# ShahzaibAhmad05/NextSearch-api

Hardware: AMD Instinct MI355X
Metric: queries/sec at k=10 over 1M-doc index; achieved HBM GB/s vs peak (higher is better)
Workload: dtype f32

## Files before the change

### include/nextsearch_hip.h

```cpp
#ifndef NEXTSEARCH_HIP_H
#define NEXTSEARCH_HIP_H

#include <stdint.h>

#ifdef __cplusplus
extern "C" {
#endif

#define NS_OK            0
#define NS_E_INVAL      -1
#define NS_E_NODEVICE   -2
#define NS_E_HIP        -3
#define NS_E_NOMEM      -4
#define NS_E_STATE      -5

#define NS_MAX_K        100u

#define NS_FLAG_OR      0u
#define NS_FLAG_AND     1u
#define NS_INFO_IMPACTS 0x100u
#define NS_INFO_PACKED  0x200u
#define NS_INFO_SHARED  0x800u
#define NS_INFO_PRUNED  0x400u

typedef struct ns_ctx   ns_ctx;
typedef struct ns_seg   ns_seg;
typedef struct ns_batch ns_batch;

typedef struct ns_term_ref {
    uint32_t seg_id;
    uint32_t count;
    uint64_t byte_off;
    float    idf;
    float    qweight;
} ns_term_ref;

typedef struct ns_query_desc {
    uint32_t term_begin;
    uint32_t term_count;
} ns_query_desc;

typedef struct ns_hit {
    float    score;
    uint32_t seg_id;
    uint32_t doc_id;
} ns_hit;

typedef struct ns_batch_info {
    uint64_t postings;
    uint64_t algo_bytes;
    uint32_t n_queries;
    uint32_t n_items;
    uint32_t n_term_refs;
    uint32_t tile_docs;
    uint32_t k;
    uint32_t flags;
    float    last_score_kernel_ms;
    float    last_total_ms;
    uint32_t timed_runs;
    uint32_t shared_lists;
    double   sum_score_kernel_ms;
    double   sum_total_ms;
    uint64_t shared_postings;
} ns_batch_info;

int  ns_ctx_create(int device, ns_ctx** out);
void ns_ctx_destroy(ns_ctx* ctx);
int  ns_ctx_set_stream(ns_ctx* ctx, void* hip_stream);
const char* ns_last_error(ns_ctx* ctx);
const char* ns_device_name(ns_ctx* ctx);

int ns_segment_upload(ns_ctx* ctx, uint32_t seg_id, uint32_t n_docs, float avgdl,
                      const uint32_t* doc_len, const void* postings, uint64_t nbytes, ns_seg** out);
int ns_segment_release(ns_ctx* ctx, ns_seg* seg);
int ns_segment_upload_begin(ns_ctx* ctx, uint32_t seg_id, uint32_t n_docs, float avgdl, const uint32_t* doc_len,
                            uint64_t total_nbytes, ns_seg** out);
int ns_segment_upload_append(ns_ctx* ctx, ns_seg* seg, const void* bytes, uint64_t nbytes);
int ns_segment_upload_end(ns_ctx* ctx, ns_seg* seg);

int ns_segment_build_impacts(ns_ctx* ctx, ns_seg* seg, const uint64_t* byte_off, const uint32_t* counts,
                             const float* idfs, uint32_t n_lists);
int ns_ctx_set_overlap(ns_ctx* ctx, int on);
int ns_ctx_set_host_threads(ns_ctx* ctx, uint32_t n);
int ns_segment_build_packed(ns_ctx* ctx, ns_seg* seg);
int ns_ctx_use_packed(ns_ctx* ctx, int mode);
int ns_ctx_use_impacts(ns_ctx* ctx, int on);
int ns_segment_build_skips(ns_ctx* ctx, ns_seg* seg, const uint64_t* byte_off, const uint32_t* counts, uint32_t n_lists);
int ns_segment_filter(ns_ctx* ctx, ns_seg* src, uint32_t new_seg_id, const uint32_t* keep_bits, const uint64_t* byte_off,
                      const uint32_t* counts, uint32_t n_lists, uint64_t* new_byte_off_out, uint32_t* new_counts_out,
                      void* postings_out, uint64_t* kept_postings_out, float* device_ms_out, ns_seg** out);
int ns_ctx_use_skips(ns_ctx* ctx, int on);
int ns_segment_build_blockmax(ns_ctx* ctx, ns_seg* seg, const uint64_t* byte_off, const uint32_t* counts,
                              const float* idfs, uint32_t n_lists);
int ns_ctx_use_pruning(ns_ctx* ctx, int on);
int ns_ctx_use_merge(ns_ctx* ctx, int on);
int ns_ctx_share_scores(ns_ctx* ctx, int mode);

int ns_search_batch(ns_ctx* ctx, const ns_query_desc* queries, const ns_term_ref* terms,
                    uint32_t n_queries, uint32_t k, ns_hit* hits_out, uint32_t* nhits_out,
                    uint64_t* found_out, uint32_t flags);

int  ns_batch_prepare(ns_ctx* ctx, const ns_query_desc* queries, const ns_term_ref* terms,
                      uint32_t n_queries, uint32_t k, uint32_t flags, ns_batch** out);
int  ns_batch_bind_outputs(ns_batch* b, void* d_hits, void* d_nhits, void* d_found);
#define NS_RUN_TIMED 1
#define NS_RUN_FETCH 2
int  ns_batch_run(ns_batch* b, int run_flags);
void* ns_batch_stream(ns_batch* b);
int  ns_batch_gap_ms(ns_batch* prev, ns_batch* next, float* ms);
int  ns_batch_sync(ns_batch* b);
int  ns_batch_fetch(ns_batch* b, ns_hit* hits_out, uint32_t* nhits_out, uint64_t* found_out);
int  ns_batch_get_info(ns_batch* b, ns_batch_info* info);
void ns_batch_destroy(ns_batch* b);

typedef struct ns_sem ns_sem;
int ns_sem_upload(ns_ctx* ctx, const float* vecs, uint32_t n_rows, uint32_t dim, ns_sem** out);
int ns_sem_release(ns_ctx* ctx, ns_sem* sem);
int ns_sem_topk(ns_ctx* ctx, ns_sem* sem, const float* qvecs, uint32_t n_q, uint32_t topk, float min_sim,
                const uint32_t* ban_off, const uint32_t* ban_rows, uint32_t* rows_out, float* sims_out,
                uint32_t* counts_out, float* device_ms_out);

typedef struct ns_ac ns_ac;
int ns_ac_upload(ns_ctx* ctx, const uint8_t* pool, const uint64_t* offsets, const uint32_t* scores, uint32_t n_terms, ns_ac** out);
int ns_ac_suggest(ns_ctx* ctx, ns_ac* ac, const uint8_t* prefix_bytes, const uint32_t* prefix_offsets, uint32_t n_q, uint32_t L,
                  uint32_t* idx_out, uint32_t* count_out, float* device_ms_out);
int ns_ac_release(ns_ctx* ctx, ns_ac* ac);

#define NS_FUZZY_MAX_LEN   64u
#define NS_FUZZY_MAX_EDITS 2u
int ns_ac_build_fuzzy(ns_ctx* ctx, ns_ac* ac, float* device_ms_out);
int ns_ac_fuzzy(ns_ctx* ctx, ns_ac* ac, const uint8_t* term_bytes, const uint32_t* term_offsets, uint32_t n_q,
                const uint8_t* max_edits, uint32_t prefix_len, uint32_t L, uint32_t* idx_out, uint8_t* dist_out,
                uint32_t* count_out, float* device_ms_out);

int ns_ac_fuzzy_prefix(ns_ctx* ctx, ns_ac* ac, const uint8_t* prefix_bytes, const uint32_t* prefix_offsets, uint32_t n_q,
                       const uint8_t* max_edits, uint32_t prefix_len, uint32_t L, uint32_t* idx_out, uint8_t* dist_out,
                       uint32_t* count_out, float* device_ms_out);

int ns_merge_rank_rows(ns_ctx* ctx, const void* d_hits, const void* d_nhits, const void* d_found, uint32_t n_ranks,
                       uint32_t n_queries, uint32_t k, const uint32_t* d_seg_map, uint32_t seg_map_stride,
                       void* d_out_hits, void* d_out_nhits, void* d_out_found);

int ns_invert_forward(ns_ctx* ctx, const uint32_t* doc_term_counts, uint32_t n_docs, const uint32_t* pairs,
                      uint64_t n_pairs, uint32_t n_terms, uint32_t* df_out, void* postings_out, uint64_t* kept_out,
                      float* device_ms_out);
int ns_segment_upload_inverted(ns_ctx* ctx, ns_seg* seg, const uint32_t* doc_term_counts, const uint32_t* pairs,
                               uint64_t n_pairs, uint32_t n_terms, uint32_t* df_out, void* postings_out,
                               uint64_t* kept_out, float* device_ms_out);

#define NS_E_ARG NS_E_INVAL
typedef struct ns_forward ns_forward;
typedef struct ns_forward_info {
    uint32_t struct_size;
    uint32_t kept_docs;
    uint32_t n_terms;
    uint32_t n_docs;
    uint64_t n_pairs;
    uint64_t term_bytes;
    uint64_t n_tokens;
    uint64_t kept_tokens;
    uint64_t device_bytes;
    float    device_ms;
    uint32_t pad;
} ns_forward_info;
int ns_forward_build(ns_ctx* ctx, const uint8_t* text, uint64_t text_bytes, const uint64_t* offsets, uint32_t n_docs,
                     ns_forward** out);
int ns_forward_get_info(const ns_forward* fwd, ns_forward_info* info);
int ns_forward_fetch(ns_forward* fwd, uint32_t* kept_docs_out, uint32_t* doc_len_out, uint32_t* counts_out,
                     uint32_t* pairs_out, uint8_t* term_bytes_out, uint64_t* term_offsets_out);
void ns_forward_destroy(ns_forward* fwd);

typedef struct ns_forward_src {
    uint32_t n_docs;  const uint32_t* doc_len;  const uint32_t* counts;
    uint64_t n_pairs; const uint32_t* pairs;
    uint32_t n_terms; const uint8_t* term_bytes; const uint64_t* term_offsets;
} ns_forward_src;
int ns_forward_merge(ns_ctx* ctx, const ns_forward_src* src, uint32_t n_src, ns_forward** out);
int ns_forward_invert(ns_forward* fwd, uint32_t* df_out, void* postings_out, uint64_t* kept_out, float* device_ms_out);
uint32_t ns_compact_doc_cut(void);
// ... 47 lines not shown
```

### nextsearch-api_amd/csrc/ns_api.hip

```cpp
#include <hip/hip_runtime.h>

#include <algorithm>
#include <cmath>
#include <cstdarg>
#include <cstdio>
#include <cstdlib>
#include <cstring>
#include <string>
#include <vector>

#include "../../include/nextsearch_hip.h"
#include "ns_internal.h"
#include "ns_plan.hpp"
#include "ns_kernels.hip"
#include "ns_wave_kernel.hip"
#include "ns_driver_kernel.hip"
#include "ns_prune_kernel.hip"
#include "ns_merge_kernel.hip"
#include "ns_tile_kernel.hip"
#include "ns_invert.hip"
#include "ns_ingest.hip"
#include "ns_compact.hip"
#include "ns_delete.hip"
#include "ns_filter.hip"
#include "ns_facet.hip"
#include "ns_similar.hip"
#include "ns_sorted.hip"
#include "ns_boolean.hip"
#include "ns_sem.hip"
#include "ns_suggest.hip"
#include "ns_fuzzy.hip"

using namespace ns;

static_assert(sizeof(ns_hit) == sizeof(Hit), "ns_hit layout");


struct ns_seg {
    ns_ctx* ctx = nullptr;
    uint32_t id = 0;
    uint32_t n_docs = 0;
    uint64_t n_postings = 0;
    uint2* d_postings = nullptr;
    float* d_norm = nullptr;
    float* d_pnorm = nullptr;
    bool norm_safe = false;
    float avgdl = 0.0f;
    bool pending = false;
    uint64_t filled = 0;
    uint32_t* d_len = nullptr;
    void* pin[2] = {nullptr, nullptr};
    hipEvent_t ev[2] = {nullptr, nullptr};
    int stage_k = 0;
    uint32_t* d_packed = nullptr;
    uint2* d_pk_hdr = nullptr;
    float* d_pk_scores = nullptr;
    uint16_t* d_nidx = nullptr;
    float* d_ntab = nullptr;
    uint32_t n_norms = 0;
    uint2* d_impacts = nullptr;
    uint32_t* d_skips = nullptr;
    std::vector<uint32_t*> skip_retired;
    uint64_t skip_cap = 0, skip_used = 0;
    uint32_t skip_entries() const { return (n_docs + kSkipDocs - 1) / kSkipDocs + 2; }
    float* d_blockmax = nullptr;
    std::vector<float*> bmx_retired;
    uint64_t bmx_cap = 0, bmx_used = 0;
    SegLists lists;
};

struct ns_ctx {
    struct Block { void* p; size_t n; };
    std::vector<Block> pool;
    size_t pool_bytes = 0;
    int device = 0;
    hipStream_t own_stream = nullptr;
    hipStream_t stream = nullptr;
    hipStream_t alt_stream = nullptr;
    hipStream_t pull_stream = nullptr;
    bool overlap = false, flip = false;
    std::string err;
    std::string devname;
    std::vector<ns_seg*> segs;
    std::vector<ns_seg*> pending_uploads;
    void* h_up = nullptr;
    size_t h_up_cap = 0;
    hipEvent_t up_done = nullptr;
    bool up_busy = false;
    void* h_down = nullptr;
    size_t h_down_cap = 0;
    struct ns_batch* down_owner = nullptr;
    struct DownSlot { void* p = nullptr; size_t cap = 0; bool busy = false; };
    std::vector<DownSlot> down_slots;
    PlanSettings cfg;
    ShareRegistry share;
    BatchPlan plan;
    std::vector<ns_ac*> acs;
    std::vector<ns_forward*> fwds;
    bool cp_inplace = true;
    std::vector<ns_docterms*> dts;
};

static thread_local std::string g_create_err;
static void ac_free_fwd(ns_ac* ac);
static void forward_orphan_fwd(ns_forward* f);
static void docterms_orphan_fwd(ns_docterms* h);
static void seg_free_device_fwd(ns_seg* s);
static void seg_free_staging_fwd(ns_seg* s);

static int fail(ns_ctx* ctx, int code, const char* fmt, ...) {
    va_list ap;
    va_start(ap, fmt);
    (ctx ? ctx->err : g_create_err) = vformat(fmt, ap);
    va_end(ap);
    return code;
}

#define HIPCHK(ctx, call)                                                                         \
    do {                                                                                          \
        hipError_t e_ = (call);                                                                   \
        if (e_ != hipSuccess)                                                                     \
            return fail((ctx), NS_E_HIP, "%s failed: %s (%s:%d)", #call, hipGetErrorString(e_), __FILE__, __LINE__); \
    } while (0)

template <int CB, int TMAX, bool IMP, int PK>
static void launch_uscore(bool and_mode, uint32_t n_items, hipStream_t st, const DevWItem* items, const DevTerm* terms,
                          const DevSeg* segs, Hit* hits, uint32_t* nhits, uint64_t* found, uint32_t K) {
    dim3 grid((n_items + kUscoreWavesPerBlock - 1) / kUscoreWavesPerBlock), block(64 * kUscoreWavesPerBlock);
    if (and_mode)
        hipLaunchKernelGGL((k_uscore<512, 192, true, CB, TMAX, IMP, PK>), grid, block, 0, st, items, n_items, terms, segs, hits, nhits, found, K);
    else
        hipLaunchKernelGGL((k_uscore<512, 192, false, CB, TMAX, IMP, PK>), grid, block, 0, st, items, n_items, terms, segs, hits, nhits, found, K);
}
template <int CB, int TMAX>
static void launch_uscore(bool and_mode, bool imp, int pk, uint32_t n_items, hipStream_t st, const DevWItem* items,
                          const DevTerm* terms, const DevSeg* segs, Hit* hits, uint32_t* nhits, uint64_t* found, uint32_t K) {
    if (imp && pk) launch_uscore<CB, TMAX, true, 1>(and_mode, n_items, st, items, terms, segs, hits, nhits, found, K);
    else if (imp) launch_uscore<CB, TMAX, true, 0>(and_mode, n_items, st, items, terms, segs, hits, nhits, found, K);
    else if (pk == 2) launch_uscore<CB, TMAX, false, 2>(and_mode, n_items, st, items, terms, segs, hits, nhits, found, K);
    else if (pk == 1) launch_uscore<CB, TMAX, false, 1>(and_mode, n_items, st, items, terms, segs, hits, nhits, found, K);
    else launch_uscore<CB, TMAX, false, 0>(and_mode, n_items, st, items, terms, segs, hits, nhits, found, K);
}

template <int HK, int FB>
static void launch_dscore(bool and_mode, uint32_t n_items, hipStream_t st, const DevWItem* items, const DevTerm* terms,
                          const DevSeg* segs, Hit* hits, uint32_t* nhits, uint64_t* found, uint32_t K) {
    dim3 grid((n_items + 3) / 4), block(256);
    if (and_mode)
        hipLaunchKernelGGL((k_dscore<HK, FB, true>), grid, block, 0, st, items, n_items, terms, segs, hits, nhits, found, K);
    else
        hipLaunchKernelGGL((k_dscore<HK, FB, false>), grid, block, 0, st, items, n_items, terms, segs, hits, nhits, found, K);
}

template <int TD>
static void launch_tscore(bool and_mode, uint32_t n_items, hipStream_t st, const DevWItem* items, const DevTerm* terms,
                          const DevSeg* segs, Hit* hits, uint32_t* nhits, uint64_t* found, uint32_t K) {
    dim3 grid((n_items + 3) / 4), block(256);
    if (and_mode)
        hipLaunchKernelGGL((k_tscore<TD, true>), grid, block, 0, st, items, n_items, terms, segs, hits, nhits, found, K);
    else
        hipLaunchKernelGGL((k_tscore<TD, false>), grid, block, 0, st, items, n_items, terms, segs, hits, nhits, found, K);
}

template <int NT, int SPT, int U>
static void launch_score(bool and_mode, uint32_t n_items, hipStream_t st, const DevItem* items, const DevTerm* terms,
                         const DevSeg* segs, const uint32_t* bounds, Hit* hits, uint32_t* nhits, uint64_t* found,
                         uint32_t K) {
    if (and_mode)
        hipLaunchKernelGGL((k_score<NT, SPT, U, true>), dim3(n_items), dim3(NT), 0, st, items, terms, segs, bounds, hits, nhits, found, K);
    else
        hipLaunchKernelGGL((k_score<NT, SPT, U, false>), dim3(n_items), dim3(NT), 0, st, items, terms, segs, bounds, hits, nhits, found, K);
}

extern "C" int ns_ctx_create(int device, ns_ctx** out) {
    if (!out) return fail(nullptr, NS_E_INVAL, "ns_ctx_create: out is NULL");
    *out = nullptr;
    int ndev = 0;
    hipError_t e = hipGetDeviceCount(&ndev);
    if (e != hipSuccess || ndev <= 0)
        return fail(nullptr, NS_E_NODEVICE, "no HIP device available (%s); this library has no CPU fallback",
                    e == hipSuccess ? "device count 0" : hipGetErrorString(e));
    if (device < 0 || device >= ndev) return fail(nullptr, NS_E_INVAL, "device %d out of range [0,%d)", device, ndev);
    e = hipSetDevice(device);
    if (e != hipSuccess) return fail(nullptr, NS_E_NODEVICE, "hipSetDevice(%d): %s", device, hipGetErrorString(e));
    hipDeviceProp_t prop;
    e = hipGetDeviceProperties(&prop, device);
    if (e != hipSuccess) return fail(nullptr, NS_E_NODEVICE, "hipGetDeviceProperties: %s", hipGetErrorString(e));
    ns_ctx* ctx = new ns_ctx();
    ctx->device = device;
    ctx->devname = std::string(prop.gcnArchName) + " " + prop.name;
    ctx->cfg.n_cus = prop.multiProcessorCount;
    e = hipStreamCreateWithFlags(&ctx->own_stream, hipStreamNonBlocking);
    if (e != hipSuccess) {
        int rc = fail(nullptr, NS_E_HIP, "hipStreamCreate: %s", hipGetErrorString(e));
        delete ctx;
        return rc;
    }
    ctx->stream = ctx->own_stream;
    if (const char* om = std::getenv("NS_ORDER_MODE")) ctx->cfg.order_mode = std::atoi(om);
    if (const char* kp = std::getenv("NS_KEY_PCT")) {
        unsigned a = 100, b = 100, c = 100, d = 100;
        if (std::sscanf(kp, "%u,%u,%u,%u", &a, &b, &c, &d) >= 1) { ctx->cfg.key_pct[0] = a; ctx->cfg.key_pct[1] = b; ctx->cfg.key_pct[2] = c; ctx->cfg.key_pct[3] = d; }
    }
    if (const char* td = std::getenv("NS_TILE_DENS64")) ctx->cfg.tile_dens64 = (uint32_t)std::max(1, std::atoi(td));
    if (const char* um = std::getenv("NS_MERGE")) ctx->cfg.use_merge = std::atoi(um) != 0;
    if (const char* mr = std::getenv("NS_MERGE_RATIO")) ctx->cfg.merge_ratio = (uint32_t)std::max(1, std::atoi(mr));
    if (const char* sm = std::getenv("NS_SHARE")) ctx->cfg.share_mode = std::max(0, std::min(2, std::atoi(sm)));
    if (const char* sr = std::getenv("NS_SHARE_RATIO")) ctx->cfg.share_ratio = (uint32_t)std::max(1, std::atoi(sr));
    if (const char* sp = std::getenv("NS_SHARE_MIN")) ctx->cfg.share_min_postings = (uint64_t)std::max(0ll, std::atoll(sp));
    if (const char* oc = std::getenv("NS_ORDER_COARSE")) { ctx->cfg.order_coarse = std::max(0, std::min(11, std::atoi(oc))); ctx->cfg.order_coarse_forced = true; }
    if (hipStreamCreateWithFlags(&ctx->alt_stream, hipStreamNonBlocking) != hipSuccess) { ctx->alt_stream = nullptr; (void)hipGetLastError(); }
    {
        int lo_pri = 0, hi_pri = 0;
        (void)hipDeviceGetStreamPriorityRange(&lo_pri, &hi_pri);
        if (hipStreamCreateWithPriority(&ctx->pull_stream, hipStreamNonBlocking, hi_pri) != hipSuccess) { ctx->pull_stream = nullptr; (void)hipGetLastError(); }
    }
    *out = ctx;
    return NS_OK;
}

extern "C" void ns_ctx_destroy(ns_ctx* ctx) {
    if (!ctx) return;
    (void)hipSetDevice(ctx->device);
    (void)hipStreamSynchronize(ctx->stream);
    if (ctx->alt_stream) (void)hipStreamSynchronize(ctx->alt_stream);
    if (ctx->pull_stream) (void)hipStreamSynchronize(ctx->pull_stream);
    for (ns_seg* s : ctx->segs) {
        if (!s) continue;
        seg_free_device_fwd(s);
        delete s;
    }
    for (ns_seg* s : ctx->pending_uploads) {
        seg_free_staging_fwd(s);
        seg_free_device_fwd(s);
        delete s;
    }
    for (ns_ac* ac : ctx->acs) ac_free_fwd(ac);
    for (ns_forward* f : ctx->fwds) forward_orphan_fwd(f);
    for (ns_docterms* h : ctx->dts) docterms_orphan_fwd(h);
    for (auto& blk : ctx->pool) (void)hipFree(blk.p);
    if (ctx->h_up) (void)hipHostFree(ctx->h_up);
    if (ctx->h_down) (void)hipHostFree(ctx->h_down);
    for (auto& ds : ctx->down_slots) if (ds.p) (void)hipHostFree(ds.p);
    if (ctx->up_done) (void)hipEventDestroy(ctx->up_done);
    if (ctx->own_stream) (void)hipStreamDestroy(ctx->own_stream);
    if (ctx->alt_stream) (void)hipStreamDestroy(ctx->alt_stream);
    if (ctx->pull_stream) (void)hipStreamDestroy(ctx->pull_stream);
    delete ctx;
}

extern "C" int ns_ctx_set_stream(ns_ctx* ctx, void* hip_stream) {
    if (!ctx) return fail(nullptr, NS_E_INVAL, "ns_ctx_set_stream: ctx is NULL");
    ctx->stream = hip_stream ? (hipStream_t)hip_stream : ctx->own_stream;
    return NS_OK;
}

extern "C" const char* ns_last_error(ns_ctx* ctx) { return ctx ? ctx->err.c_str() : g_create_err.c_str(); }
extern "C" const char* ns_device_name(ns_ctx* ctx) { return ctx ? ctx->devname.c_str() : ""; }

extern "C" int ns_set_tuning(ns_ctx* ctx, uint32_t variant, uint32_t min_items, uint32_t split_postings) {
    if (!ctx) return fail(nullptr, NS_E_INVAL, "ns_set_tuning: ctx is NULL");
    if (variant >= kNumVariants || kVariants[variant].nt == 0) return fail(ctx, NS_E_INVAL, "unknown kernel variant %u", variant);
#ifndef NS_VARIANTS
    if (variant != 0) return fail(ctx, NS_E_INVAL, "kernel variant %u exists only in the variants build (make -C nextsearch-api_amd variants)", variant);
#endif
    ctx->cfg.variant = variant;
    ctx->cfg.min_items = min_items;
    ctx->cfg.split_postings = split_postings;
    return NS_OK;
}

static constexpr size_t kPadPostings = 256;
static constexpr size_t kStageChunk = 32u << 20;

static void seg_free_staging(ns_seg* s) {
    for (int i = 0; i < 2; i++) {
        if (s->pin[i]) (void)hipHostFree(s->pin[i]);
        if (s->ev[i]) (void)hipEventDestroy(s->ev[i]);
        s->pin[i] = nullptr; s->ev[i] = nullptr;
    }
    if (s->d_len) (void)hipFree(s->d_len);
    s->d_len = nullptr;
}
static void seg_free_device(ns_seg* s);
static void seg_free_device_fwd(ns_seg* s) { seg_free_device(s); }
static void seg_free_staging_fwd(ns_seg* s) { seg_free_staging(s); }
static void seg_free_device(ns_seg* s) {
    (void)hipFree(s->d_postings);
    (void)hipFree(s->d_norm);
    (void)hipFree(s->d_pnorm);
    (void)hipFree(s->d_impacts);
    (void)hipFree(s->d_packed);
    (void)hipFree(s->d_pk_hdr);
    (void)hipFree(s->d_pk_scores);
    (void)hipFree(s->d_nidx);
    (void)hipFree(s->d_ntab);
    (void)hipFree(s->d_skips);
    for (uint32_t* p : s->skip_retired) (void)hipFree(p);
    s->skip_retired.clear();
    (void)hipFree(s->d_blockmax);
    for (float* p : s->bmx_retired) (void)hipFree(p);
    s->bmx_retired.clear();
    s->d_blockmax = nullptr; s->bmx_cap = s->bmx_used = 0; s->lists.bmx.clear();
    s->d_skips = nullptr; s->skip_cap = s->skip_used = 0; s->lists.skip.clear();
    s->d_postings = nullptr; s->d_norm = nullptr; s->d_pnorm = nullptr; s->d_impacts = nullptr; s->d_packed = nullptr;
    s->d_pk_hdr = nullptr; s->d_pk_scores = nullptr; s->d_nidx = nullptr; s->d_ntab = nullptr;
}
static hipError_t seg_stage(ns_ctx* ctx, ns_seg* s, void* dst, const void* src, size_t n) {
    size_t off = 0;
    while (off < n) {
        const size_t c = std::min(kStageChunk, n - off);
        const int k = s->stage_k;
        hipError_t r = hipEventSynchronize(s->ev[k]);
        if (r != hipSuccess) return r;
        std::memcpy(s->pin[k], (const char*)src + off, c);
        r = hipMemcpyAsync((char*)dst + off, s->pin[k], c, hipMemcpyHostToDevice, ctx->stream);
        if (r != hipSuccess) return r;
        r = hipEventRecord(s->ev[k], ctx->stream);
        if (r != hipSuccess) return r;
        off += c;
        s->stage_k ^= 1;
    }
    return hipSuccess;
}

extern "C" int ns_segment_upload_begin(ns_ctx* ctx, uint32_t seg_id, uint32_t n_docs, float avgdl, const uint32_t* doc_len,
                                       uint64_t nbytes, ns_seg** out) {
    if (!ctx) return fail(nullptr, NS_E_INVAL, "ns_segment_upload: ctx is NULL");
    if (!out) return fail(ctx, NS_E_INVAL, "ns_segment_upload_begin: out is NULL");
    *out = nullptr;
// ... 203 lines not shown
    if (int rc = check_lists(ctx, seg, byte_off, counts, n_lists)) return rc;
    struct L { uint32_t first, count; float idf; };
    std::vector<L> lists;
    lists.reserve(n_lists);
    for (uint32_t i = 0; i < n_lists; i++)
        if (counts[i]) lists.push_back({(uint32_t)(byte_off[i] / 8), counts[i], idfs[i]});
    std::sort(lists.begin(), lists.end(), [](const L& a, const L& b) { return a.first < b.first; });
    for (size_t i = 1; i < lists.size(); i++)
        if (lists[i - 1].first + (uint64_t)lists[i - 1].count > lists[i].first) return fail(ctx, NS_E_INVAL, "lists overlap at posting %u", lists[i].first);
    if (lists.empty()) return NS_OK;
    hipError_t e = hipSuccess;
    if (!seg->d_impacts) {
        e = hipMalloc((void**)&seg->d_impacts, (seg->n_postings + kPadPostings) * 8);
        if (e != hipSuccess) { seg->d_impacts = nullptr; return fail(ctx, NS_E_NOMEM, "hipMalloc impact stream (%llu B): %s", (unsigned long long)(seg->n_postings * 8), hipGetErrorString(e)); }
        e = hipMemsetAsync(seg->d_impacts, 0xFF, (seg->n_postings + kPadPostings) * 8, ctx->stream);
    }
    const size_t n = lists.size();
    std::vector<uint32_t> h_starts(n), h_counts(n);
    std::vector<float> h_idfs(n);
    for (size_t i = 0; i < n; i++) { h_starts[i] = lists[i].first; h_counts[i] = lists[i].count; h_idfs[i] = lists[i].idf; }
    uint32_t* d_tmp = nullptr;
    if (e == hipSuccess) e = hipMalloc((void**)&d_tmp, n * 12);
    if (e == hipSuccess) e = hipMemcpyAsync(d_tmp, h_starts.data(), n * 4, hipMemcpyHostToDevice, ctx->stream);
    if (e == hipSuccess) e = hipMemcpyAsync(d_tmp + n, h_counts.data(), n * 4, hipMemcpyHostToDevice, ctx->stream);
    if (e == hipSuccess) e = hipMemcpyAsync(d_tmp + 2 * n, h_idfs.data(), n * 4, hipMemcpyHostToDevice, ctx->stream);
    if (e == hipSuccess) {
        const uint32_t blocks = (uint32_t)std::min<uint64_t>((seg->n_postings + 255) / 256, 1u << 16);
        hipLaunchKernelGGL(k_build_impacts, dim3(blocks), dim3(256), 0, ctx->stream, seg->d_postings, seg->d_pnorm, seg->d_impacts,
                           d_tmp, d_tmp + n, (const float*)(d_tmp + 2 * n), (uint32_t)n, seg->n_postings);
        e = hipGetLastError();
    }
    if (e == hipSuccess) e = hipStreamSynchronize(ctx->stream);
    (void)hipFree(d_tmp);
    if (e == hipSuccess) e = seg_fill_pk_scores(ctx, seg);
    if (e != hipSuccess) return fail(ctx, NS_E_HIP, "ns_segment_build_impacts: %s", hipGetErrorString(e));
    for (const auto& l : lists) {
        uint32_t ib; std::memcpy(&ib, &l.idf, 4);
        seg->lists.imp.put(l.first, {l.count, ib});
    }
    return NS_OK;
}

__global__ void __launch_bounds__(256) k_share_scores(const DevShare* __restrict__ sh, uint32_t n_lists, const DevSeg* __restrict__ segs) {
    const uint32_t total = sh[n_lists].before;
    const uint32_t base = blockIdx.x * 1024u;
    if (base >= total) return;
    const uint32_t last = min(base + 1023u, total - 1u);
    __shared__ uint32_t s_lo, s_hi;
    if (threadIdx.x < 2) {
        const uint32_t want = threadIdx.x == 0 ? base : last;
        uint32_t lo = 0, hi = n_lists;
        while (hi - lo > 1) {
            const uint32_t mid = lo + ((hi - lo) >> 1);
            if (sh[mid].before <= want) lo = mid; else hi = mid;
        }
        if (threadIdx.x == 0) s_lo = lo; else s_hi = lo;
    }
    __syncthreads();
    const uint32_t l0 = s_lo, l1 = s_hi;
#pragma unroll
    for (int j = 0; j < 4; j++) {
        const uint32_t p = base + (uint32_t)j * 256u + threadIdx.x;
        if (p > last) continue;
        uint32_t lo = l0, hi = l1 + 1u;
        while (hi - lo > 1) {
            const uint32_t mid = lo + ((hi - lo) >> 1);
            if (sh[mid].before <= p) lo = mid; else hi = mid;
        }
        const DevShare L = sh[lo];
        const DevSeg& sg = segs[L.seg];
        const uint64_t at = (uint64_t)L.first + (p - L.before);
        const uint2 pv = sg.postings[at];
        const float tf = (float)pv.y;
        const float den = tf + sg.pnorm[at];
        const float num = L.idf * (tf * (1.2f + 1.0f));
        const_cast<uint2*>(sg.impacts)[at] = make_uint2(pv.x, __float_as_uint(num / den));
    }
}

extern "C" int ns_ctx_share_scores(ns_ctx* ctx, int mode) {
    if (!ctx) return fail(nullptr, NS_E_INVAL, "ns_ctx_share_scores: ctx is NULL");
    if (mode < 0 || mode > 2) return fail(ctx, NS_E_INVAL, "ns_ctx_share_scores: mode %d outside [0, 2]", mode);
    ctx->cfg.share_mode = mode;
    return NS_OK;
}

extern "C" int ns_segment_build_packed(ns_ctx* ctx, ns_seg* seg) {
    if (!ctx || !seg) return fail(ctx, NS_E_INVAL, "ns_segment_build_packed: null argument");
    if (seg->pending || seg->id >= ctx->segs.size() || ctx->segs[seg->id] != seg) return fail(ctx, NS_E_INVAL, "segment does not belong to this ctx");
    if (seg->d_packed || !seg->n_postings) return NS_OK;
    if (!seg->d_nidx) return fail(ctx, NS_E_INVAL, "ns_segment_build_packed: segment %u has more than 65536 distinct document lengths; its norms do not fit a 16-bit index", seg->id);
    HIPCHK(ctx, hipSetDevice(ctx->device));
    const uint64_t n_blocks = (seg->n_postings + kPkBlock - 1) / kPkBlock;
    hipError_t e = hipMalloc((void**)&seg->d_packed, (n_blocks + 2) * kPkStrideDwords * 4);
    if (e == hipSuccess) e = hipMalloc((void**)&seg->d_pk_hdr, (n_blocks + 2) * sizeof(uint2));
    if (e == hipSuccess) e = hipMemsetAsync(seg->d_packed + n_blocks * kPkStrideDwords, 0, 2 * kPkStrideDwords * 4, ctx->stream);
    if (e == hipSuccess) e = hipMemsetAsync(seg->d_pk_hdr + n_blocks, 0, 2 * sizeof(uint2), ctx->stream);
    if (e == hipSuccess) {
        hipLaunchKernelGGL(k_pack, dim3((uint32_t)n_blocks), dim3(64), 0, ctx->stream, seg->d_postings, seg->d_nidx, seg->d_packed, seg->d_pk_hdr,
                           seg->n_postings, seg->n_docs, (uint32_t)n_blocks);
        e = hipGetLastError();
    }
    if (e == hipSuccess) e = hipStreamSynchronize(ctx->stream);
    if (e == hipSuccess) e = seg_fill_pk_scores(ctx, seg);
    if (e != hipSuccess) {
        (void)hipFree(seg->d_packed); (void)hipFree(seg->d_pk_hdr);
        seg->d_packed = nullptr; seg->d_pk_hdr = nullptr;
        return fail(ctx, e == hipErrorOutOfMemory ? NS_E_NOMEM : NS_E_HIP, "ns_segment_build_packed: %s", hipGetErrorString(e));
    }
    return NS_OK;
}

__global__ void __launch_bounds__(256) k_skip_fill(uint32_t* __restrict__ sk, const uint32_t* __restrict__ starts, const uint32_t* __restrict__ counts,
                                                   uint32_t per_list) {
    const uint32_t l = blockIdx.y;
    const uint32_t endp = starts[l] + counts[l];
    for (uint32_t i = blockIdx.x * 256 + threadIdx.x; i < per_list; i += gridDim.x * 256) sk[(uint64_t)l * per_list + i] = endp;
}
__global__ void __launch_bounds__(256) k_skip_build(const uint2* __restrict__ postings, uint32_t* __restrict__ sk, const uint32_t* __restrict__ starts,
                                                    const uint32_t* __restrict__ counts, uint32_t per_list) {
    const uint32_t l = blockIdx.y;
    const uint32_t first = starts[l], n = counts[l];
    uint32_t* row = sk + (uint64_t)l * per_list;
    const uint32_t cells = per_list - 2;
    for (uint32_t i = blockIdx.x * 256 + threadIdx.x; i < n; i += gridDim.x * 256) {
        const uint32_t d = postings[first + i].x / kSkipDocs;
        uint32_t c0 = 0;
        if (i) {
            const uint32_t dp = postings[first + i - 1].x / kSkipDocs;
            c0 = dp + 1;
        }
        for (uint32_t c = c0; c <= d && c <= cells; c++) row[c] = first + i;
    }
}
__global__ void __launch_bounds__(256) k_skip_check(const uint2* __restrict__ postings, const uint32_t* __restrict__ sk, const uint32_t* __restrict__ starts,
                                                    const uint32_t* __restrict__ counts, uint32_t per_list, uint32_t* __restrict__ bad) {
    const uint32_t l = blockIdx.y;
    const uint32_t first = starts[l], endp = first + counts[l];
    const uint32_t* row = sk + (uint64_t)l * per_list;
    bool b = false;
    for (uint32_t i = blockIdx.x * 256 + threadIdx.x; i + 1 < per_list; i += gridDim.x * 256) {
        const uint32_t a = row[i], z = row[i + 1];
        if (a > z || a < first || z > endp) b = true;
        if (i == 0 && a != first) b = true;
        if (i + 2 == per_list && (z != endp || a != endp)) b = true;
        if (i + 2 < per_list && a < z) {
            if (postings[a].x / kSkipDocs != i || postings[z - 1].x / kSkipDocs != i) b = true;
        }
    }
    if (b) bad[l] = 1u;
}

extern "C" int ns_segment_build_skips(ns_ctx* ctx, ns_seg* seg, const uint64_t* byte_off, const uint32_t* counts, uint32_t n_lists) {
    if (!ctx || !seg) return fail(ctx, NS_E_INVAL, "ns_segment_build_skips: null argument");
    if (seg->pending || seg->id >= ctx->segs.size() || ctx->segs[seg->id] != seg) return fail(ctx, NS_E_INVAL, "segment does not belong to this ctx");
    if (n_lists && (!byte_off || !counts)) return fail(ctx, NS_E_INVAL, "null list arrays");
    if (!n_lists || !seg->n_postings || !seg->n_docs) return NS_OK;
    HIPCHK(ctx, hipSetDevice(ctx->device));
    if (int rc = check_lists(ctx, seg, byte_off, counts, n_lists)) return rc;
    struct L { uint32_t first, count; };
    std::vector<L> lists;
    lists.reserve(n_lists);
    for (uint32_t i = 0; i < n_lists; i++)
        if (counts[i] && !seg->lists.skip_of((uint32_t)(byte_off[i] / 8), counts[i])) lists.push_back({(uint32_t)(byte_off[i] / 8), counts[i]});
    std::sort(lists.begin(), lists.end(), [](const L& a, const L& b) { return a.first < b.first || (a.first == b.first && a.count < b.count); });
    lists.erase(std::unique(lists.begin(), lists.end(), [](const L& a, const L& b) { return a.first == b.first; }), lists.end());
// ... 96 lines not shown
    if (e == hipSuccess) e = hipMemcpyAsync(d_tmp, h.data(), n * 16, hipMemcpyHostToDevice, ctx->stream);
    if (e == hipSuccess) {
        for (size_t l0 = 0; l0 < n; l0 += 32768) {
            const uint32_t ny = (uint32_t)std::min<size_t>(32768, n - l0);
            hipLaunchKernelGGL(k_blockmax, dim3(std::min<uint32_t>(std::max<uint32_t>(bmax_blocks, 1u), 256u), ny), dim3(64), 0, ctx->stream,
                               seg->d_postings, seg->d_pnorm, seg->d_blockmax, d_tmp + l0, d_tmp + n + l0, (const float*)(d_tmp + 2 * n + l0), d_tmp + 3 * n + l0);
        }
        e = hipGetLastError();
    }
    if (e == hipSuccess) e = hipStreamSynchronize(ctx->stream);
    (void)hipFree(d_tmp);
    if (e != hipSuccess) return fail(ctx, NS_E_HIP, "ns_segment_build_blockmax: %s", hipGetErrorString(e));
    seg->bmx_used = need;
    for (const auto& l : lists) {
        uint32_t ib; std::memcpy(&ib, &l.idf, 4);
        seg->lists.bmx.put(l.first, {l.count, ib, l.entry});
    }
    return NS_OK;
}

extern "C" int ns_ctx_use_merge(ns_ctx* ctx, int on) {
    if (!ctx) return NS_E_INVAL;
    ctx->cfg.use_merge = on != 0;
    return NS_OK;
}

extern "C" int ns_ctx_use_pruning(ns_ctx* ctx, int on) {
    if (!ctx) return NS_E_INVAL;
    ctx->cfg.use_pruning = on != 0;
    return NS_OK;
}

extern "C" int ns_ctx_use_skips(ns_ctx* ctx, int on) {
    if (!ctx) return NS_E_INVAL;
    ctx->cfg.use_skips = on != 0;
    return NS_OK;
}

extern "C" int ns_ctx_use_packed(ns_ctx* ctx, int on) {
    if (!ctx) return NS_E_INVAL;
    if (on < 0 || on > 2) return fail(ctx, NS_E_INVAL, "ns_ctx_use_packed: mode %d (0, 1 or 2)", on);
    ctx->cfg.use_packed = on;
    return NS_OK;
}

extern "C" int ns_ctx_set_overlap(ns_ctx* ctx, int on) {
    if (!ctx) return NS_E_INVAL;
    if (on && !ctx->alt_stream) return fail(ctx, NS_E_HIP, "ns_ctx_set_overlap: the second stream could not be created");
    ctx->overlap = on != 0;
    return NS_OK;
}

extern "C" int ns_ctx_set_host_threads(ns_ctx* ctx, uint32_t n) {
    if (!ctx) return NS_E_INVAL;
    if (n > 64) return fail(ctx, NS_E_INVAL, "ns_ctx_set_host_threads: %u threads (at most 64)", n);
    ctx->cfg.prep_threads = n;
    return NS_OK;
}

extern "C" int ns_ctx_use_impacts(ns_ctx* ctx, int on) {
    if (!ctx) return NS_E_INVAL;
    ctx->cfg.use_impacts = on != 0;
    return NS_OK;
}

struct ns_batch {
    ns_ctx* ctx = nullptr;
    uint32_t Q = 0, K = 0, flags = 0;
    uint32_t variant = 0, tile_docs = 0, hb = 0;
    uint32_t n_items = 0;
    uint32_t n_witems = 0;
    uint32_t n_class[3] = {0, 0, 0};
    uint32_t n_bgroups = 0;
    uint32_t n_terms = 0, n_parts = 0;
    uint64_t postings = 0;
    bool direct = false;
    int pk = 0;
    bool pruned = false;
    bool imp = false;
    bool shared = false;
    uint32_t n_share = 0;
    uint64_t share_postings = 0;
    DevShare* d_share = nullptr;
    DevItem* d_items = nullptr;
    DevWItem* d_witems = nullptr;
    DevTerm* d_terms = nullptr;
    DevGroup* d_groups = nullptr;
    DevQuery* d_queries = nullptr;
    DevSeg* d_segs = nullptr;
    uint32_t* d_bounds = nullptr;
    Hit* d_part_hits = nullptr;
    uint32_t* d_part_nhits = nullptr;
    uint64_t* d_part_found = nullptr;
    uint32_t* d_heads = nullptr;
    Hit* d_hits = nullptr;
    uint32_t* d_nhits = nullptr;
    uint64_t* d_found = nullptr;
    Hit* o_hits = nullptr;
    uint32_t* o_nhits = nullptr;
    uint64_t* o_found = nullptr;
    std::vector<hipEvent_t> ev_pool;
    size_t ev_pending = 0;
    bool ran = false;
    float last_score_ms = -1.0f, last_total_ms = -1.0f;
    double sum_score_ms = 0.0, sum_total_ms = 0.0;
    uint32_t timed_runs = 0;
    uint32_t* d_wide_q = nullptr;
    uint32_t n_wide_q = 0;
    size_t out_span = 0, off_nhits = 0, off_found = 0;
    std::vector<std::pair<void*, size_t>> blocks;
    hipStream_t st = nullptr;
    hipEvent_t done = nullptr;
    bool done_recorded = false;
    bool fetch_enqueued = false;
    int down_slot = -1;
};

static constexpr size_t kPoolMaxBytes = 1ull << 30;
static constexpr size_t kStageMaxBytes = 256ull << 20;
static constexpr size_t kPullUploadBytes = 256 << 10;
static constexpr size_t kHostResultBytes = 64 << 10;

static size_t pool_quantise(size_t n) {
    if (n <= (64u << 10)) return 64u << 10;
    if (n <= (64u << 20)) { size_t q = 64u << 10; while (q < n) q <<= 1; return q; }
    return (n + (16u << 20) - 1) & ~(size_t)((16u << 20) - 1);
}
static hipError_t pool_alloc(ns_ctx* ctx, void** out, size_t n) {
    n = pool_quantise(n);
    size_t best = (size_t)-1;
    for (size_t i = 0; i < ctx->pool.size(); i++)
        if (ctx->pool[i].n >= n && ctx->pool[i].n <= 2 * n + 4096 && (best == (size_t)-1 || ctx->pool[i].n < ctx->pool[best].n)) best = i;
    if (best != (size_t)-1) {
        *out = ctx->pool[best].p;
        ctx->pool_bytes -= ctx->pool[best].n;
        ctx->pool[best] = ctx->pool.back();
        ctx->pool.pop_back();
        return hipSuccess;
    }
    hipError_t e = hipMalloc(out, n);
    if (e == hipErrorOutOfMemory && !ctx->pool.empty()) {
        for (auto& b : ctx->pool) (void)hipFree(b.p);
        ctx->pool.clear(); ctx->pool_bytes = 0;
        e = hipMalloc(out, n);
    }
    return e;
}
static void pool_free(ns_ctx* ctx, void* p, size_t n) {
    if (!p) return;
    n = pool_quantise(n);
    if (ctx->pool_bytes + n > kPoolMaxBytes || ctx->pool.size() >= 64) { (void)hipFree(p); return; }
    ctx->pool.push_back({p, n});
    ctx->pool_bytes += n;
}

__global__ void __launch_bounds__(256) k_pull(uint4* __restrict__ dst, const uint4* __restrict__ src, uint32_t n16) {
    const uint32_t i = blockIdx.x * 256 + threadIdx.x;
    if (i < n16) dst[i] = src[i];
}

extern "C" void ns_batch_destroy(ns_batch* b) {
    if (!b) return;
    (void)hipSetDevice(b->ctx->device);
    if (b->done_recorded) (void)hipEventSynchronize(b->done);
    else (void)hipStreamSynchronize(b->st);
    if (b->ctx->down_owner == b) b->ctx->down_owner = nullptr;
    if (b->down_slot >= 0) b->ctx->down_slots[(size_t)b->down_slot].busy = false;
    if (b->shared && b->ctx->share.live) b->ctx->share.live--;
    for (auto& blk : b->blocks) pool_free(b->ctx, blk.first, blk.second);
    for (auto& e : b->ev_pool) if (e) (void)hipEventDestroy(e);
    if (b->done) (void)hipEventDestroy(b->done);
    delete b;
}

static hipError_t batch_alloc(ns_batch* b, void** dptr, size_t n) {
    hipError_t e = pool_alloc(b->ctx, dptr, n);
    if (e == hipSuccess) b->blocks.push_back({*dptr, n});
    return e;
}
extern "C" int ns_batch_prepare(ns_ctx* ctx, const ns_query_desc* queries, const ns_term_ref* terms, uint32_t n_queries,
                                uint32_t k, uint32_t flags, ns_batch** out) {
    if (!ctx) return fail(nullptr, NS_E_INVAL, "ns_batch_prepare: ctx is NULL");
    if (!out) return fail(ctx, NS_E_INVAL, "ns_batch_prepare: out is NULL");
    *out = nullptr;
    if (k < 1 || k > NS_MAX_K) return fail(ctx, NS_E_INVAL, "k=%u outside [1,%u]", k, NS_MAX_K);
    if (n_queries && !queries) return fail(ctx, NS_E_INVAL, "queries is NULL");
    if (flags & ~NS_FLAG_AND) return fail(ctx, NS_E_INVAL, "unknown flags 0x%x", flags);
    HIPCHK(ctx, hipSetDevice(ctx->device));

    const VariantDesc vd = kVariants[ctx->cfg.variant];
    const uint32_t tile_docs = vd.nt * vd.spt;
    std::vector<SegView> views(ctx->segs.size());
    std::vector<DevSeg> segs(ctx->segs.size());
    for (size_t i = 0; i < ctx->segs.size(); i++) {
        DevSeg d{};
        if (ns_seg* s = ctx->segs[i]) {
            d.postings = s->d_postings;
            d.pnorm = s->d_pnorm;
            d.impacts = s->d_impacts;
            d.packed = s->d_packed;
            d.pk_hdr = s->d_pk_hdr;
            d.ntab = s->d_ntab;
            d.pk_scores = s->d_pk_scores;
            d.skips = s->d_skips;
            d.blockmax = s->d_blockmax;
            d.norm = s->d_norm;
            d.n_postings = s->n_postings;
            d.n_docs = s->n_docs;
            d.n_tiles = (s->n_docs + tile_docs - 1) / tile_docs;
            views[i] = SegView{s->n_docs, d.n_tiles, s->n_postings, s->norm_safe, s->d_packed != nullptr, &s->lists};
        }
        segs[i] = d;
    }

    BatchPlan& P = ctx->plan;
    int rc = P.group(ctx->cfg, views, ctx->share, queries, terms, n_queries, k, flags);
    if (rc != NS_OK) return fail(ctx, rc, "%s", P.err.c_str());
    for (size_t i = 0; P.shared && i < P.share_build.size(); i++) {
        ns_seg* sg = ctx->segs[P.share_build[i].seg];
        if (!sg->d_impacts) {
            const size_t nb = (size_t)(sg->n_postings + kPadPostings) * 8;
            hipError_t ea = hipMalloc((void**)&sg->d_impacts, nb);
            if (ea == hipSuccess) ea = hipMemsetAsync(sg->d_impacts, 0xFF, nb, ctx->stream);
            if (ea == hipSuccess) ea = hipStreamSynchronize(ctx->stream);
            if (ea != hipSuccess) {
                if (sg->d_impacts) (void)hipFree(sg->d_impacts);
                sg->d_impacts = nullptr; (void)hipGetLastError();
                P.shared = false;
            }
        }
        if (P.shared) segs[P.share_build[i].seg].impacts = sg->d_impacts;
    }
    rc = P.cut();
    if (rc != NS_OK) return fail(ctx, rc, "%s", P.err.c_str());

    ns_batch* b = new ns_batch();
    b->ctx = ctx;
    b->st = ctx->stream;
    if (ctx->overlap && ctx->stream == ctx->own_stream && ctx->alt_stream) {
        ctx->flip = !ctx->flip;
        if (ctx->flip) b->st = ctx->alt_stream;
    }
    b->Q = n_queries; b->K = k; b->flags = flags;
    b->variant = ctx->cfg.variant; b->tile_docs = tile_docs; b->hb = vd.hb;
    b->n_items = P.n_items; b->n_witems = P.n_witems;
    b->n_bgroups = P.n_bgroups; b->n_terms = P.n_dterms;
    for (int c = 0; c < 3; c++) b->n_class[c] = P.n_class[c];
    b->n_parts = P.direct ? 0 : P.n_rows;
    b->postings = P.postings_total;
    b->direct = P.direct;
    b->imp = P.all_imp && P.postings_total > 0;
    if (P.shared) {
        b->shared = true;
        b->n_share = (uint32_t)P.share_build.size();
        b->share_postings = P.share_postings;
        ctx->share.live++;
    }
    b->pk = (P.all_pk && P.postings_total > 0) ? ctx->cfg.use_packed : 0;
    b->pruned = P.pruned;
    b->n_wide_q = (uint32_t)P.wide_q.size();

    hipError_t e = hipSuccess;
    auto chk = [&](hipError_t r) { if (e == hipSuccess) e = r; };
    const BatchPlan::Layout& L = P.layout;
    const size_t up_bytes = L.bytes;
    size_t off = up_bytes;
    auto place = [&](size_t bytes) { return place_at(off, bytes); };
    const size_t Qn = std::max<uint32_t>(n_queries, 1), Pn = std::max<uint32_t>(b->n_parts, 1);
    const size_t o_bounds = place(P.bounds_total * 4);
    size_t o_phits = 0, o_pnhits = 0, o_pfound = 0, o_heads = 0;
    if (!P.direct) {
        o_phits = place(Pn * k * sizeof(Hit));
        o_pnhits = place(Pn * 4);
        o_pfound = place(Pn * 8);
        o_heads = place(Pn * 4);
    }
    const size_t o_hits = place(Qn * k * sizeof(Hit));
    const size_t o_nhits = place(Qn * 4);
    const size_t o_found = place(Qn * 8);
    char* base = nullptr;
    chk(batch_alloc(b, (void**)&base, off));
    if (e == hipSuccess) {
        b->d_items = (decltype(b->d_items))(base + L.items);
        b->d_witems = (decltype(b->d_witems))(base + L.witems);
        b->d_terms = (decltype(b->d_terms))(base + L.terms);
        b->d_groups = (decltype(b->d_groups))(base + L.groups);
        b->d_queries = (decltype(b->d_queries))(base + L.queries);
        b->d_segs = (decltype(b->d_segs))(base + L.segs);
        b->d_wide_q = (uint32_t*)(base + L.wideq);
        b->d_share = (DevShare*)(base + L.share);
        b->d_bounds = (uint32_t*)(base + o_bounds);
        if (!P.direct) {
            b->d_part_hits = (Hit*)(base + o_phits);
            b->d_part_nhits = (uint32_t*)(base + o_pnhits);
            b->d_part_found = (uint64_t*)(base + o_pfound);
            b->d_heads = (uint32_t*)(base + o_heads);
        }
        b->d_hits = (Hit*)(base + o_hits);
        b->d_nhits = (uint32_t*)(base + o_nhits);
        b->d_found = (uint64_t*)(base + o_found);
        b->out_span = o_found + Qn * 8 - o_hits;
        b->off_nhits = o_nhits - o_hits;
        b->off_found = o_found - o_hits;
        if (b->out_span <= kHostResultBytes && !ctx->down_owner) {
            if (ctx->h_down_cap < b->out_span) {
                if (ctx->h_down) (void)hipHostFree(ctx->h_down);
                ctx->h_down = nullptr; ctx->h_down_cap = 0;
                if (hipHostMalloc(&ctx->h_down, kHostResultBytes, hipHostMallocDefault) == hipSuccess) ctx->h_down_cap = kHostResultBytes;
                else { ctx->h_down = nullptr; (void)hipGetLastError(); }
            }
            if (ctx->h_down_cap >= b->out_span) {
                ctx->down_owner = b;
                b->d_hits = (Hit*)ctx->h_down;
                b->d_nhits = (uint32_t*)((char*)ctx->h_down + b->off_nhits);
                b->d_found = (uint64_t*)((char*)ctx->h_down + b->off_found);
            }
        }
    }
    if (e == hipSuccess && ctx->up_busy) {
        chk(hipEventSynchronize(ctx->up_done));
        ctx->up_busy = false;
    }
    if (e == hipSuccess && up_bytes <= kStageMaxBytes && ctx->h_up_cap < up_bytes) {
        if (ctx->h_up) (void)hipHostFree(ctx->h_up);
        ctx->h_up = nullptr; ctx->h_up_cap = 0;
        const size_t cap = std::max<size_t>(up_bytes + up_bytes / 2, 1 << 16);
        if (hipHostMalloc(&ctx->h_up, cap, hipHostMallocDefault) == hipSuccess) ctx->h_up_cap = cap;
        else { ctx->h_up = nullptr; (void)hipGetLastError(); }
    }
    if (e == hipSuccess && !ctx->up_done) chk(hipEventCreateWithFlags(&ctx->up_done, hipEventDisableTiming));
    if (e == hipSuccess) {
        const bool staged = ctx->h_up_cap >= up_bytes && ctx->up_done;
        std::vector<char> unstaged;
        if (!staged) unstaged.resize(up_bytes);
        char* hb = staged ? (char*)ctx->h_up : unstaged.data();
        P.write(hb);
        if (!segs.empty()) std::memcpy(hb + L.segs, segs.data(), segs.size() * sizeof(segs[0]));
        if (staged) {
            if (up_bytes > kPullUploadBytes && ctx->pull_stream) {
                hipLaunchKernelGGL(k_pull, dim3((uint32_t)((up_bytes / 16 + 255) / 256)), dim3(256), 0, ctx->pull_stream,
                                   (uint4*)base, (const uint4*)hb, (uint32_t)(up_bytes / 16));
                chk(hipEventRecord(ctx->up_done, ctx->pull_stream));
                chk(hipStreamWaitEvent(b->st, ctx->up_done, 0));
            } else {
                if (up_bytes <= kPullUploadBytes || ctx->overlap)
                    hipLaunchKernelGGL(k_pull, dim3((uint32_t)((up_bytes / 16 + 255) / 256)), dim3(256), 0, b->st,
                                       (uint4*)base, (const uint4*)hb, (uint32_t)(up_bytes / 16));
                else
                    chk(hipMemcpyAsync(base, hb, up_bytes, hipMemcpyHostToDevice, b->st));
                chk(hipEventRecord(ctx->up_done, b->st));
            }
            if (e == hipSuccess) ctx->up_busy = true;
        } else {
            chk(hipMemcpyAsync(base, hb, up_bytes, hipMemcpyHostToDevice, b->st));
            chk(hipStreamSynchronize(b->st));
        }
    }
    if (e != hipSuccess) {
        rc = fail(ctx, e == hipErrorOutOfMemory ? NS_E_NOMEM : NS_E_HIP, "ns_batch_prepare: %s", hipGetErrorString(e));
        ns_batch_destroy(b);
        return rc;
    }
    b->o_hits = b->d_hits; b->o_nhits = b->d_nhits; b->o_found = b->d_found;
    *out = b;
    return NS_OK;
}

extern "C" int ns_batch_bind_outputs(ns_batch* b, void* d_hits, void* d_nhits, void* d_found) {
    if (!b) return NS_E_INVAL;
    b->o_hits = d_hits ? (Hit*)d_hits : b->d_hits;
    b->o_nhits = d_nhits ? (uint32_t*)d_nhits : b->d_nhits;
    b->o_found = d_found ? (uint64_t*)d_found : b->d_found;
    return NS_OK;
}

extern "C" int ns_batch_run(ns_batch* b, int run_flags) {
    if (!b) return NS_E_INVAL;
    ns_ctx* ctx = b->ctx;
    const int timed = run_flags & NS_RUN_TIMED;
    if (run_flags & NS_RUN_FETCH) {
        const bool own_outputs = b->o_hits == b->d_hits && b->o_nhits == b->d_nhits && b->o_found == b->d_found;
        if (!own_outputs) return fail(ctx, NS_E_STATE, "NS_RUN_FETCH: the batch writes into caller-bound device buffers (ns_batch_bind_outputs); there is nothing to fetch");
    }
    b->done_recorded = false;
    HIPCHK(ctx, hipSetDevice(ctx->device));
    hipStream_t st = b->st;
    const bool and_mode = (b->flags & NS_FLAG_AND) != 0;
    hipEvent_t* ev = nullptr;
    if (timed) {
        while (b->ev_pool.size() < b->ev_pending + 4) {
            hipEvent_t e = nullptr;
            HIPCHK(ctx, hipEventCreate(&e));
            b->ev_pool.push_back(e);
        }
        ev = b->ev_pool.data() + b->ev_pending;
        b->ev_pending += 4;
    }
    if (timed) HIPCHK(ctx, hipEventRecord(ev[0], st));
    if (b->n_bgroups)
        hipLaunchKernelGGL(k_bounds, dim3(b->n_bgroups), dim3(128), 0, st, b->d_groups, b->d_terms, b->d_segs, b->d_bounds, b->tile_docs);
    if (timed) HIPCHK(ctx, hipEventRecord(ev[1], st));
    if (b->shared && b->n_share)
        hipLaunchKernelGGL(k_share_scores, dim3((uint32_t)((b->share_postings + 1023) / 1024)), dim3(256), 0, st, b->d_share, b->n_share, b->d_segs);
    Hit* sh = b->direct ? b->o_hits : b->d_part_hits;
    uint32_t* sn = b->direct ? b->o_nhits : b->d_part_nhits;
    uint64_t* sf = b->direct ? b->o_found : b->d_part_found;
    if (b->n_witems && b->variant == 0) {
        const uint32_t n_narrow = b->n_class[0], n_wide = b->n_witems - b->n_class[0];
        const DevWItem* wide = b->d_witems + n_narrow;
        if (b->K <= 32) {
            if (n_narrow) launch_uscore<128, 16>(and_mode, b->imp, b->pk, n_narrow, st, b->d_witems, b->d_terms, b->d_segs, sh, sn, sf, b->K);
            if (n_wide) launch_uscore<128, 64>(and_mode, b->imp, b->pk, n_wide, st, wide, b->d_terms, b->d_segs, sh, sn, sf, b->K);
        } else {
            if (n_narrow) launch_uscore<256, 16>(and_mode, b->imp, b->pk, n_narrow, st, b->d_witems, b->d_terms, b->d_segs, sh, sn, sf, b->K);
            if (n_wide) launch_uscore<256, 64>(and_mode, b->imp, b->pk, n_wide, st, wide, b->d_terms, b->d_segs, sh, sn, sf, b->K);
        }
    }
#ifdef NS_VARIANTS
    else if (b->n_witems) {
        const VariantDesc wv = kVariants[b->variant];
#define NS_D(HH, FF) launch_dscore<HH, FF>(and_mode, b->n_witems, st, b->d_witems, b->d_terms, b->d_segs, sh, sn, sf, b->K)
        if (wv.d == 1) {
            if (wv.hb == 512) launch_tscore<512>(and_mode, b->n_witems, st, b->d_witems, b->d_terms, b->d_segs, sh, sn, sf, b->K);
            else if (wv.hb == 2048) launch_tscore<2048>(and_mode, b->n_witems, st, b->d_witems, b->d_terms, b->d_segs, sh, sn, sf, b->K);
            else launch_tscore<1024>(and_mode, b->n_witems, st, b->d_witems, b->d_terms, b->d_segs, sh, sn, sf, b->K);
        } else if (wv.d == 0) {
            switch (b->variant) {
                case 13: NS_D(256, 64); break;
                case 14: NS_D(1024, 256); break;
                case 15: NS_D(512, 64); break;
                case 16: NS_D(512, 256); break;
                case 17: NS_D(1024, 128); break;
                default: NS_D(512, 128); break;
            }
        }
#undef NS_D
    }
#endif
    if (b->n_items) {
#ifdef NS_VARIANTS
        const VariantDesc vd = kVariants[b->variant];
        if (vd.nt == 1024) launch_score<1024, 12, 4>(and_mode, b->n_items, st, b->d_items, b->d_terms, b->d_segs, b->d_bounds, sh, sn, sf, b->K);
        else if (vd.nt == 256) launch_score<256, 16, 4>(and_mode, b->n_items, st, b->d_items, b->d_terms, b->d_segs, b->d_bounds, sh, sn, sf, b->K);
        else if (vd.spt == 16) launch_score<512, 16, 8>(and_mode, b->n_items, st, b->d_items, b->d_terms, b->d_segs, b->d_bounds, sh, sn, sf, b->K);
        else
#endif
        launch_score<512, 12, 4>(and_mode, b->n_items, st, b->d_items, b->d_terms, b->d_segs, b->d_bounds, sh, sn, sf, b->K);
    }
    if (timed) HIPCHK(ctx, hipEventRecord(ev[2], st));
    if (!b->direct && b->Q > b->n_wide_q)
        hipLaunchKernelGGL(k_merge, dim3((b->Q + 3) / 4), dim3(256), 0, st, b->d_queries, b->Q, b->d_part_hits, b->d_part_nhits,
                           b->d_part_found, b->o_hits, b->o_nhits, b->o_found, b->K, b->d_heads);
    if (!b->direct && b->n_wide_q)
        hipLaunchKernelGGL(k_merge_wide, dim3(b->n_wide_q), dim3(256), 0, st, b->d_queries, b->d_wide_q, b->d_part_hits, b->d_part_nhits,
                           b->d_part_found, b->o_hits, b->o_nhits, b->o_found, b->K, b->d_heads);
    if (timed) HIPCHK(ctx, hipEventRecord(ev[3], st));
    HIPCHK(ctx, hipGetLastError());
    b->ran = true;
    if (run_flags & NS_RUN_FETCH) {
        if (b->Q && ctx->down_owner != b) {
            if (b->down_slot < 0) {
                int slot = -1;
                for (size_t i = 0; i < ctx->down_slots.size(); i++)
                    if (!ctx->down_slots[i].busy && ctx->down_slots[i].cap >= b->out_span) { slot = (int)i; break; }
                if (slot < 0) {
                    for (size_t i = 0; i < ctx->down_slots.size() && slot < 0; i++)
                        if (!ctx->down_slots[i].busy) {
                            if (ctx->down_slots[i].p) (void)hipHostFree(ctx->down_slots[i].p);
                            ctx->down_slots[i] = ns_ctx::DownSlot{};
                            slot = (int)i;
                        }
                    if (slot < 0) {
                        if (ctx->down_slots.size() >= 8) return fail(ctx, NS_E_STATE, "NS_RUN_FETCH: more than 8 batches between run and fetch");
                        ctx->down_slots.emplace_back();
                        slot = (int)ctx->down_slots.size() - 1;
                    }
                    const size_t cap = std::max<size_t>(b->out_span + b->out_span / 4, 1 << 16);
                    if (hipHostMalloc(&ctx->down_slots[(size_t)slot].p, cap, hipHostMallocDefault) != hipSuccess) {
                        ctx->down_slots[(size_t)slot].p = nullptr;
                        (void)hipGetLastError();
                        return fail(ctx, NS_E_NOMEM, "NS_RUN_FETCH: pinned result buffer of %zu bytes", cap);
                    }
                    ctx->down_slots[(size_t)slot].cap = cap;
                }
                ctx->down_slots[(size_t)slot].busy = true;
                b->down_slot = slot;
            }
            HIPCHK(ctx, hipMemcpyAsync(ctx->down_slots[(size_t)b->down_slot].p, b->d_hits, b->out_span, hipMemcpyDeviceToHost, st));
        }
    }
    if (!b->done) HIPCHK(ctx, hipEventCreateWithFlags(&b->done, hipEventDisableTiming));
    HIPCHK(ctx, hipEventRecord(b->done, st));
    b->done_recorded = true;
    b->fetch_enqueued = (run_flags & NS_RUN_FETCH) != 0;
    return NS_OK;
}

extern "C" void* ns_batch_stream(ns_batch* b) { return b ? (void*)b->st : nullptr; }

extern "C" int ns_batch_gap_ms(ns_batch* prev, ns_batch* next, float* ms) {
    if (!prev || !next || !ms) return NS_E_INVAL;
    if (prev->ev_pool.size() < 4 || next->ev_pool.size() < 4) return fail(next->ctx, NS_E_STATE, "ns_batch_gap_ms: both batches need a timed run");
    const hipError_t e = hipEventElapsedTime(ms, prev->ev_pool[3], next->ev_pool[0]);
    if (e == hipErrorNotReady) { (void)hipGetLastError(); return NS_E_STATE; }
    if (e != hipSuccess) return fail(next->ctx, NS_E_HIP, "ns_batch_gap_ms: %s", hipGetErrorString(e));
    return NS_OK;
}


static int batch_collect_timings(ns_batch* b) {
    ns_ctx* ctx = b->ctx;
    for (size_t i = 0; i + 4 <= b->ev_pending; i += 4) {
        HIPCHK(ctx, hipEventElapsedTime(&b->last_score_ms, b->ev_pool[i + 1], b->ev_pool[i + 2]));
        HIPCHK(ctx, hipEventElapsedTime(&b->last_total_ms, b->ev_pool[i], b->ev_pool[i + 3]));
        b->sum_score_ms += b->last_score_ms;
        b->sum_total_ms += b->last_total_ms;
        b->timed_runs++;
    }
    b->ev_pending = 0;
    return NS_OK;
}

extern "C" int ns_batch_sync(ns_batch* b) {
    if (!b) return NS_E_INVAL;
    ns_ctx* ctx = b->ctx;
    HIPCHK(ctx, hipSetDevice(ctx->device));
    HIPCHK(ctx, hipStreamSynchronize(b->st));
    return batch_collect_timings(b);
}

extern "C" int ns_batch_fetch(ns_batch* b, ns_hit* hits_out, uint32_t* nhits_out, uint64_t* found_out) {
    if (!b) return NS_E_INVAL;
    ns_ctx* ctx = b->ctx;
    if (!b->ran) return fail(ctx, NS_E_STATE, "ns_batch_fetch before ns_batch_run");
    HIPCHK(ctx, hipSetDevice(ctx->device));
    hipStream_t st = b->st;
    const bool own_outputs = b->o_hits == b->d_hits && b->o_nhits == b->d_nhits && b->o_found == b->d_found;
    if (b->fetch_enqueued && b->done_recorded && own_outputs) {
        HIPCHK(ctx, hipEventSynchronize(b->done));
        int rc = batch_collect_timings(b);
        if (rc != NS_OK) return rc;
        if (b->Q) {
            const char* h = (ctx->down_owner == b) ? (const char*)ctx->h_down : (const char*)ctx->down_slots[(size_t)b->down_slot].p;
            if (hits_out) std::memcpy(hits_out, h, (size_t)b->Q * b->K * sizeof(Hit));
            if (nhits_out) std::memcpy(nhits_out, h + b->off_nhits, (size_t)b->Q * 4);
            if (found_out) std::memcpy(found_out, h + b->off_found, (size_t)b->Q * 8);
        }
        if (b->down_slot >= 0) { ctx->down_slots[(size_t)b->down_slot].busy = false; b->down_slot = -1; }
        b->fetch_enqueued = false;
        return NS_OK;
    }
    if (b->Q && own_outputs && ctx->down_owner == b) {
        int rc = ns_batch_sync(b);
        if (rc != NS_OK) return rc;
        const char* h = (const char*)ctx->h_down;
        if (hits_out) std::memcpy(hits_out, h, (size_t)b->Q * b->K * sizeof(Hit));
        if (nhits_out) std::memcpy(nhits_out, h + b->off_nhits, (size_t)b->Q * 4);
        if (found_out) std::memcpy(found_out, h + b->off_found, (size_t)b->Q * 8);
        return NS_OK;
    }
    if (b->Q && own_outputs && !ctx->down_owner && b->out_span <= kStageMaxBytes) {
        if (ctx->h_down_cap < b->out_span) {
            if (ctx->h_down) (void)hipHostFree(ctx->h_down);
            ctx->h_down = nullptr; ctx->h_down_cap = 0;
            const size_t cap = std::max<size_t>(b->out_span + b->out_span / 2, 1 << 16);
            if (hipHostMalloc(&ctx->h_down, cap, hipHostMallocDefault) == hipSuccess) ctx->h_down_cap = cap;
            else { ctx->h_down = nullptr; (void)hipGetLastError(); }
        }
        if (ctx->h_down_cap >= b->out_span) {
            HIPCHK(ctx, hipMemcpyAsync(ctx->h_down, b->d_hits, b->out_span, hipMemcpyDeviceToHost, st));
            int rc = ns_batch_sync(b);
            if (rc != NS_OK) return rc;
            const char* h = (const char*)ctx->h_down;
            if (hits_out) std::memcpy(hits_out, h, (size_t)b->Q * b->K * sizeof(Hit));
            if (nhits_out) std::memcpy(nhits_out, h + b->off_nhits, (size_t)b->Q * 4);
            if (found_out) std::memcpy(found_out, h + b->off_found, (size_t)b->Q * 8);
            return NS_OK;
        }
    }
    if (b->Q) {
        if (hits_out) HIPCHK(ctx, hipMemcpyAsync(hits_out, b->o_hits, (size_t)b->Q * b->K * sizeof(Hit), hipMemcpyDeviceToHost, st));
        if (nhits_out) HIPCHK(ctx, hipMemcpyAsync(nhits_out, b->o_nhits, (size_t)b->Q * 4, hipMemcpyDeviceToHost, st));
        if (found_out) HIPCHK(ctx, hipMemcpyAsync(found_out, b->o_found, (size_t)b->Q * 8, hipMemcpyDeviceToHost, st));
    }
    return ns_batch_sync(b);
}

extern "C" int ns_batch_get_info(ns_batch* b, ns_batch_info* info) {
    if (!b || !info) return NS_E_INVAL;
    info->postings = b->postings;
    info->algo_bytes = b->postings * 8;
    info->n_queries = b->Q;
    info->n_items = b->n_items + b->n_witems;
    info->n_term_refs = b->n_terms;
    info->tile_docs = b->tile_docs;
    info->k = b->K;
    info->flags = b->flags | (b->imp ? NS_INFO_IMPACTS : 0u) | (b->pk ? NS_INFO_PACKED : 0u) | (b->pruned ? NS_INFO_PRUNED : 0u) |
                  (b->shared ? NS_INFO_SHARED : 0u);
    info->shared_lists = b->n_share;
    info->shared_postings = b->share_postings;
    info->last_score_kernel_ms = b->last_score_ms;
    info->last_total_ms = b->last_total_ms;
    info->timed_runs = b->timed_runs;
    info->sum_score_kernel_ms = b->sum_score_ms;
    info->sum_total_ms = b->sum_total_ms;
    return NS_OK;
}

extern "C" int ns_search_batch(ns_ctx* ctx, const ns_query_desc* queries, const ns_term_ref* terms, uint32_t n_queries,
                               uint32_t k, ns_hit* hits_out, uint32_t* nhits_out, uint64_t* found_out, uint32_t flags) {
    ns_batch* b = nullptr;
    int rc = ns_batch_prepare(ctx, queries, terms, n_queries, k, flags, &b);
    if (rc != NS_OK) return rc;
    rc = ns_batch_run(b, 0);
    if (rc == NS_OK) rc = ns_batch_fetch(b, hits_out, nhits_out, found_out);
    ns_batch_destroy(b);
    return rc;
}


static int invert_run(ns_ctx* ctx, const uint32_t* doc_term_counts, uint32_t n_docs, const uint32_t* pairs,
                      uint64_t n_pairs, uint32_t n_terms, uint32_t* df_out, void* postings_out, uint64_t* kept_out,
                      float* device_ms_out, ns_seg* adopt, const uint2* dev_pairs = nullptr) {
    if (!ctx) return fail(nullptr, NS_E_INVAL, "ns_invert_forward: ctx is NULL");
    if ((n_docs && !doc_term_counts) || (n_pairs && !pairs && !dev_pairs) || (n_terms && !df_out) || !kept_out) return fail(ctx, NS_E_INVAL, "ns_invert_forward: null argument");
    if (n_pairs >= (1ull << 32) - kIvTile) return fail(ctx, NS_E_INVAL, "ns_invert_forward: %llu pairs; this build indexes pairs with 32 bits (split the segment)", (unsigned long long)n_pairs);
    if (n_terms == 0xFFFFFFFFu) return fail(ctx, NS_E_INVAL, "ns_invert_forward: n_terms too large");
    *kept_out = 0;
    if (device_ms_out) *device_ms_out = 0.0f;
    std::vector<uint64_t> prefix((size_t)n_docs + 1, 0);
    for (uint32_t d = 0; d < n_docs; d++) prefix[d + 1] = prefix[d] + doc_term_counts[d];
    if (prefix[n_docs] != n_pairs) return fail(ctx, NS_E_INVAL, "ns_invert_forward: the per-document counts sum to %llu, not to n_pairs = %llu", (unsigned long long)prefix[n_docs], (unsigned long long)n_pairs);
    if (n_terms) std::memset(df_out, 0, (size_t)n_terms * 4);
    if (!n_pairs) return NS_OK;
    if (!postings_out && !adopt) return fail(ctx, NS_E_INVAL, "ns_invert_forward: postings_out is NULL");
    HIPCHK(ctx, hipSetDevice(ctx->device));
    hipStream_t st = ctx->stream;
    const uint32_t n = (uint32_t)n_pairs;
    const uint32_t n_tiles = (n + kIvTile - 1) / kIvTile;
    int bits = 1;
    while (bits < 32 && n_terms > 1 && ((n_terms - 1) >> bits) != 0) bits++;
    const int passes = std::max(1, (bits + 10) / 11);
    int pbits[3] = {8, 8, 8};
    {
        int left = bits;
        for (int p = 0; p < passes; p++) {
            const int share = (left + (passes - p) - 1) / (passes - p);
            pbits[p] = std::min(11, std::max(8, share));
            left = std::max(0, left - pbits[p]);
        }
    }
    size_t m_max = 0;
    for (int p = 0; p < passes; p++) m_max = std::max(m_max, ((size_t)1 << pbits[p]) * n_tiles);
    const uint32_t scan_blocks_max = (uint32_t)((m_max + 1023) / 1024);

    uint2 *d_pairs = nullptr, *d_vals[2] = {nullptr, nullptr};
    uint32_t *d_keys[2] = {nullptr, nullptr}, *d_df = nullptr, *d_first = nullptr, *d_hist = nullptr, *d_sums = nullptr, *d_kept = nullptr;
    uint64_t* d_prefix = nullptr;
    uint2* d_tile_docs = nullptr;
    std::vector<uint32_t> tile_docs((size_t)n_tiles * 2);
    {
        uint32_t d = 0;
        auto doc_of = [&](uint64_t i) { while (d + 1 < n_docs && prefix[d + 1] <= i) d++; return d; };
        for (uint32_t t = 0; t < n_tiles; t++) {
            const uint64_t i0 = (uint64_t)t * kIvTile, i1 = std::min<uint64_t>(i0 + kIvTile, n) - 1;
            tile_docs[2 * (size_t)t] = doc_of(i0);
            tile_docs[2 * (size_t)t + 1] = doc_of(i1);
        }
    }
    hipEvent_t ev0 = nullptr, ev1 = nullptr;
    hipError_t e = hipSuccess;
    auto chk = [&](hipError_t r) { if (e == hipSuccess) e = r; };
    size_t off = 0;
    auto place = [&](size_t bytes) { const size_t o = off; off = (off + std::max<size_t>(bytes, 1) + 255) & ~(size_t)255; return o; };
    const size_t nt1 = (size_t)std::max<uint32_t>(n_terms, 1);
    const size_t o_pairs = place(dev_pairs ? 1 : (size_t)n * 8), o_v0 = place((size_t)n * 8), o_v1 = place(passes > 1 ? (size_t)n * 8 : 1);
    const size_t o_k0 = place((size_t)n * 4), o_k1 = place(passes > 1 ? (size_t)n * 4 : 1);
    const size_t o_df = place(nt1 * 4), o_first = place(nt1 * 4), o_hist = place(m_max * 4), o_sums = place((size_t)scan_blocks_max * 4), o_kept = place(4), o_prefix = place(prefix.size() * 8), o_tdocs = place((size_t)n_tiles * 8);
    const size_t block_bytes = off;
    char* blk = nullptr;
    chk(pool_alloc(ctx, (void**)&blk, block_bytes));
    if (e == hipSuccess) {
        d_pairs = dev_pairs ? const_cast<uint2*>(dev_pairs) : (uint2*)(blk + o_pairs); d_vals[0] = (uint2*)(blk + o_v0); d_vals[1] = (uint2*)(blk + o_v1);
        d_keys[0] = (uint32_t*)(blk + o_k0); d_keys[1] = (uint32_t*)(blk + o_k1);
        d_df = (uint32_t*)(blk + o_df); d_first = (uint32_t*)(blk + o_first); d_hist = (uint32_t*)(blk + o_hist); d_sums = (uint32_t*)(blk + o_sums);
        d_kept = (uint32_t*)(blk + o_kept);
        d_prefix = (uint64_t*)(blk + o_prefix);
        d_tile_docs = (uint2*)(blk + o_tdocs);
// ... 2043 lines not shown
```

### nextsearch-api_amd/csrc/ns_driver_kernel.hip

```cpp
#pragma once
#include <hip/hip_runtime.h>
#include <stdint.h>

#include "ns_internal.h"
#include "ns_wave_kernel.hip"

namespace ns {

#ifdef NS_COUNT
constexpr int kNsCnt = 32;
__device__ unsigned long long g_ns_cnt[kNsCnt];
#define NS_CNT(i, v) cnt_[(i)] += (unsigned long long)(v)
#else
#define NS_CNT(i, v)
#endif

template <bool IMP, int PKM>
__device__ __forceinline__ void pk_decode_round(const DevSeg& seg, const uint32_t blk, const int lane, uint32_t (&doc)[4], float (&tf)[4],
                                                float (&nr)[4], uint32_t (&sbits)[4]) {
    const gp_u32 pb = (gp_u32)seg.packed + (size_t)blk * kPkStrideDwords + (uint32_t)lane;
    const uint32_t d0 = pb[kPkDoc], d1 = pb[kPkDoc + 64];
    uint32_t t = 0, na = 0, nb = 0;
    if (IMP) {
        const gp_f32 sc = (gp_f32)seg.pk_scores + (size_t)blk * kPkBlock + (uint32_t)lane;
#pragma unroll
        for (int c = 0; c < 4; c++) { sbits[c] = __float_as_uint(sc[c * 64]); tf[c] = 0.0f; nr[c] = 0.0f; }
    } else {
        t = pb[kPkTf];
        if (PKM == 2) { na = pb[kPkNormA]; nb = pb[kPkNormB]; }
        else {
            const gp_f32 np = (gp_f32)seg.pnorm + (size_t)blk * kPkBlock + (uint32_t)lane;
#pragma unroll
            for (int c = 0; c < 4; c++) nr[c] = np[c * 64];
        }
    }
    typedef const __attribute__((address_space(4))) uint32_t* cp_u32;
    const cp_u32 hp = (cp_u32)(const void*)(seg.pk_hdr + blk);
    const uint32_t base = hp[0];
    const uint32_t code = hp[1];
    if (code == 0u) {
#pragma unroll
        for (int c = 0; c < 4; c++) doc[c] = base + ((d0 >> (8 * c)) & 255u);
    } else if (code == 1u) {
        doc[0] = base + (d0 & 0xFFFFu); doc[1] = base + (d0 >> 16);
        doc[2] = base + (d1 & 0xFFFFu); doc[3] = base + (d1 >> 16);
    } else {
        doc[0] = d0; doc[1] = d1;
        doc[2] = pb[kPkDoc + 128]; doc[3] = pb[kPkDoc + 192];
    }
    if (!IMP) {
        uint32_t tfi[4];
#pragma unroll
        for (int c = 0; c < 4; c++) tfi[c] = (t >> (8 * c)) & 255u;
        const uint32_t nt_ = ~t;
        if (wballot(((nt_ - 0x01010101u) & t & 0x80808080u) != 0u) != 0ull) {
            const gp_u2 raw = (gp_u2)seg.postings + (size_t)blk * kPkBlock + (uint32_t)lane;
#pragma unroll
            for (int c = 0; c < 4; c++)
                if (tfi[c] == 255u) { const nat_u2 pv = raw[c * 64]; tfi[c] = pv.y; }
        }
        if (PKM == 2) {
            const gp_f32 ntab = (gp_f32)seg.ntab;
            nr[0] = ntab[na & 0xFFFFu]; nr[1] = ntab[na >> 16];
            nr[2] = ntab[nb & 0xFFFFu]; nr[3] = ntab[nb >> 16];
        }
#pragma unroll
        for (int c = 0; c < 4; c++) { tf[c] = (float)tfi[c]; sbits[c] = 0u; }
    }
}

__device__ __forceinline__ uint64_t lane_span(uint32_t lo, uint32_t hi) {
    const uint64_t upto_hi = hi >= 64u ? ~0ull : ((1ull << hi) - 1ull);
    const uint64_t upto_lo = lo >= 64u ? ~0ull : ((1ull << lo) - 1ull);
    return upto_hi & ~upto_lo;
}

template <int NB, int FB, bool AND, int CB = 256, bool IMP = false, int PK = 0>
__device__ __forceinline__ void dscore_body(const DevWItem& it, const DevTerm* __restrict__ terms, const DevSeg* __restrict__ segs,
                                            uint32_t* ent, float* vals, uint8_t* mcnt, uint64_t* cand, uint4* tab, uint32_t* aux,
                                            Hit* __restrict__ out_hits, uint32_t* __restrict__ out_nhits,
                                            uint64_t* __restrict__ out_found, uint32_t K, const int lane) {
    constexpr int FE = FB / 64;
    constexpr int DE = 4;
    constexpr uint32_t EMPTY = 0u;
    constexpr int LOG2NB = (NB == 64) ? 6 : (NB == 128 ? 7 : 8);
    constexpr uint32_t MAXSPAN = (1u << (LOG2NB + 15)) - 1u;
#define NS_BUCKET(doc) ((uint32_t)__builtin_amdgcn_ubfe(__umul24((doc) - lo, bm), 16u, (uint32_t)LOG2NB))
#define NS_TAG(doc) (0x8000u | (((doc) - lo) & 0x7FFFu))
#define NS_IDENT(doc, bkt) ((NS_TAG(doc) << 16) | ((bkt) << 8))
    static_assert(NB == 64 || NB == 128 || NB == 256, "NB must be 64, 128 or 256");
    static_assert(FB % 64 == 0 && FB >= 64 && FB <= 256 && FB <= 2 * NB, "FB must be a multiple of 64, at most 256 and 2*NB");
    uint4* ent4 = reinterpret_cast<uint4*>(ent);

#ifdef NS_COUNT
    const unsigned long long cyc_t0_ = __builtin_readcyclecounter();
#endif
    const DevSeg seg = segs[it.seg];
    const uint32_t T = it.term_count;
    const bool fast_div = (__builtin_amdgcn_readfirstlane((int)it.whole) & 8) != 0;
    const bool signed_in = (__builtin_amdgcn_readfirstlane((int)it.whole) & 16) != 0;
    const gp_u2 postings = (gp_u2)seg.postings;
    const gp_f32 pnorm = (gp_f32)seg.pnorm;
    const gp_u2 stream = IMP ? (gp_u2)seg.impacts : postings;

    {
        const uint4 empty4 = make_uint4(EMPTY, EMPTY, EMPTY, EMPTY);
#pragma unroll
        for (int g = 0; g < NB / 64; g++) ent4[g * 64 + lane] = empty4;
#pragma unroll
        for (int g = 0; g < FB / 64; g++) {
            vals[g * 64 + lane] = 0.0f;
            if (AND) mcnt[g * 64 + lane] = 0;
        }
    }

    uint32_t base = 0, cur = 0, end = 0, idf_bits = 0, wq_bits = 0;
    if ((uint32_t)lane < T) {
        const DevTerm tm = terms[it.term_begin + lane];
        base = (uint32_t)tm.list_off;
        idf_bits = __float_as_uint(tm.idf);
        wq_bits = __float_as_uint(tm.weight);
        const uint2 r = item_list_range(it, seg, tm);
        cur = r.x + base;
        end = r.y + base;
        tab[lane] = make_uint4(idf_bits, wq_bits, 0u, 0u);
    }
    uint32_t dl;
    {
        const uint32_t remv = end - cur;
        const uint32_t mx = wave_max_dpp(remv);
        dl = (uint32_t)__builtin_ctzll(wballot(remv == mx && (uint32_t)lane < T) | (1ull << 63));
        if (dl >= T) dl = 0;
    }
    uint32_t d_cur = rdlane(cur, dl);
    const uint32_t d_end = rdlane(end, dl);
    const float d_idf = __uint_as_float(rdlane(idf_bits, dl));
    const float d_wq = __uint_as_float(rdlane(wq_bits, dl));
    uint32_t Rf = 0;
    {
        const uint32_t r32 = ((uint32_t)lane == dl) ? 0u : (end - cur);
        for (uint32_t t = 0; t < T; t++) {
            const uint32_t v = rdlane(r32, t);
            Rf = (Rf + v < Rf) ? 0xFFFFFFFFu : (Rf + v);
        }
    }
    if ((uint32_t)lane == dl) { cur = end; }

#ifdef NS_COUNT
    unsigned long long cnt_[kNsCnt] = {};
    cnt_[16] = __builtin_readcyclecounter() - cyc_t0_; cnt_[17] = 0;
    NS_CNT(0, 1);
    NS_CNT(10, T);
#endif
    uint32_t lo = it.doc_lo;
    const uint32_t last_doc = it.doc_hi - 1;
    WaveTopK<CB> top(cand, K, lane);
    uint32_t found_s = 0;

    constexpr uint32_t WSLACK = (FB == 64) ? kWinSlackThin : kWinSlackGen;
    uint32_t w_n = 0, e_n = 0xFFFFFFFFu;
#define NS_PLAN_FOREIGN()                                                                          \
    {                                                                                              \
        const uint32_t rem_ = end - cur;               \
        const uint32_t nact_ = (uint32_t)__popcll(wballot(rem_ > 0));                             \
        const uint32_t c_ = foreign_slack(WSLACK, (uint32_t)FB, nact_, Rf);            \
        const float scale_ = foreign_scale(c_, (uint32_t)FB, nact_, __builtin_amdgcn_rcpf((float)max(Rf, 1u))); \
        const uint32_t w_ = foreign_window(rem_, c_, scale_);                                      \
        const bool probe_ = w_ < rem_;                                                             \
        const uint32_t pi_ = probe_ ? (cur + w_ - 1u) : 0u;                                        \
        const nat_u2 pv_ = postings[pi_];      \
        w_n = (rem_ > 0) ? w_ : 0u;                                                                \
        e_n = probe_ ? pv_.x : 0xFFFFFFFFu;                                                        \
    }
    NS_PLAN_FOREIGN();
    wave_sync();
    for (;;) {
        top.begin_step();
        NS_CNT(1, 1);
        const uint32_t w = w_n;
        const uint32_t e = e_n;
        const uint32_t incl = wave_incl_scan_dpp(w);
        const uint32_t total = rdlane(incl, 63);
        uint32_t hi = wave_min_dpp(e);
        const uint32_t span_hi = (last_doc - lo > MAXSPAN) ? (lo + MAXSPAN) : last_doc;
        const bool span_clamped = hi > span_hi && span_hi != last_doc;
        hi = min(hi, span_hi);
        NS_CNT(27, span_clamped ? 1 : 0);
        uint32_t bm;
        {
            const uint32_t spn1 = (hi >= lo ? hi - lo : 0u) + 1u;
            bm = (uint32_t)((float)((uint32_t)NB << 16) * __builtin_amdgcn_rcpf((float)spn1));
            bm = (uint32_t)__builtin_amdgcn_readfirstlane((int)bm);
            while ((uint64_t)bm * spn1 > (uint64_t)((uint32_t)NB << 16)) bm--;
            while ((uint64_t)(bm + 1u) * spn1 <= (uint64_t)((uint32_t)NB << 16)) bm++;
            bm = min(bm, 0xFFFFFFu);
        }

        uint32_t ftj[FE];
        float fx[FE];
        bool fok[FE], fmine[FE];
        uint32_t fdoc[FE];
        uint32_t tb_min = 0, tb_max = 0;
#pragma unroll
        for (int j = 0; j < FE; j++) { ftj[j] = 0; fx[j] = 0.0f; fok[j] = false; fmine[j] = false; fdoc[j] = 0; }
        if (total > 0) {
            if ((uint32_t)lane < T) reinterpret_cast<uint2*>(tab + lane)[1] = make_uint2(cur - (incl - w), cur);
            if (T > 8 && (uint32_t)lane < T) aux[lane] = incl;
            wave_sync();
            NS_CNT(26, T > 8 ? 1 : 0);
            if (T <= 8) {
                for (uint32_t t = 0; t + 1 < T; t++) {
                    const uint32_t sp = rdlane(incl, t);
#pragma unroll
                    for (int j = 0; j < FE; j++) ftj[j] += ((uint32_t)(j * 64 + lane) >= sp) ? 1u : 0u;
                }
            } else {
#pragma unroll
                for (int j = 0; j < FE; j++) {
                    const uint32_t p = min((uint32_t)(j * 64 + lane), total - 1u);
                    uint32_t a = 0, b = T - 1;
                    while (a < b) {
                        const uint32_t m = (a + b) >> 1;
                        if (aux[m] > p) b = m; else a = m + 1;
                    }
                    ftj[j] = a;
                }
                wave_sync();
            }
            nat_u2 pst[FE];
            float nrm[FE];
            uint32_t pidx[FE];
#pragma unroll
            for (int j = 0; j < FE; j++) {
                const uint32_t p = (uint32_t)(j * 64 + lane);
                const bool inb = p < total;
                ftj[j] = inb ? ftj[j] : 0u;
                pidx[j] = tab[ftj[j]].z + (inb ? p : 0u);
                pst[j] = stream[pidx[j]];
                nrm[j] = IMP ? 0.0f : pnorm[pidx[j]];
                pst[j].x = inb ? pst[j].x : 0xFFFFFFFFu;
// ... 112 lines not shown
                            NS_CNT(15, (uint32_t)__popcll(wballot(isp && pos < 4u)));
                            NS_CNT(20, (uint32_t)__popcll(wballot(isp && pos >= 4u)));
                            NS_CNT(21, (wballot(isp && bkt == carry_b_in_ && (uint32_t)lane == hl) != 0ull) ? 1 : 0);
                        }
                    }
                }
                wave_sync();
            }
#pragma unroll
            for (int j = 0; j < FE; j++) {
                if ((uint32_t)(j * 64) >= total) continue;
                bool pending = fok[j] && !fmine[j];
                if (wballot(pending) == 0ull) continue;
                const uint32_t me = (uint32_t)(j * 64 + lane);
                uint32_t b = NS_BUCKET(fdoc[j]);
                const uint32_t mine = NS_IDENT(fdoc[j], b) | me;
                const bool todo = pending;
                uint32_t slot = 0, own = 0;
                bool scan = pending;
                uint32_t pos = 0;
                for (int round = 0; round < 8 * NB; round++) {
                    if (wballot(pending) == 0ull) break;
                    NS_CNT(6, 1);
                    if (wballot(scan) != 0ull) {
#ifdef NS_COUNT
                        bool owner_found_ = false;
#endif
                        if (scan) {
                            const uint4 q = ent4[b];
                            const uint32_t tmin = min(min(q.x ^ mine, q.y ^ mine), min(q.z ^ mine, q.w ^ mine));
                            pos = (q.x >> 31) + (q.y >> 31) + (q.z >> 31) + (q.w >> 31);
                            if (tmin < 256u) { own = tmin ^ me; pending = false; }
#ifdef NS_COUNT
                            owner_found_ = tmin < 256u;
#endif
                            scan = false;
                        }
                        NS_CNT(24, (uint32_t)__popcll(wballot(owner_found_)));
                    }
                    const bool try_store = pending && pos < 4;
                    if (try_store) ent[b * 4 + pos] = mine;
                    wave_sync();
                    if (try_store) {
                        const uint32_t back = ent[b * 4 + pos];
                        if ((back ^ mine) < 256u) { slot = b * 4 + pos; own = back & 255u; pending = false; }
                        else pos++;
                    } else if (pending) {
                        b = (b + 1) & (uint32_t)(NB - 1);
                        scan = true;
                    }
                    NS_CNT(22, (uint32_t)__popcll(wballot(pending && scan)));
                    NS_CNT(23, (uint32_t)__popcll(wballot(pending && scan && b == 0u)));
                    wave_sync();
                }
                if (todo) {
                    fmine[j] = own == me;
                    ftj[j] |= (own << 6) | (slot << 14);
                }
            }
        }

#define NS_FOREIGN_RMW(ta, tb)                                                                     \
        for (uint32_t tt = (ta); tt <= (tb); tt++) {                                               \
            if (tt == dl) continue;                                                                \
            NS_CNT(7, 1);                                                                          \
            float old_[FE];                                                                        \
             \
                                    \
            _Pragma("unroll") for (int j = 0; j < FE; j++) {                                       \
                const bool c_ = fok[j] && (ftj[j] & 63u) == tt;                                    \
                old_[j] = vals[c_ ? ((ftj[j] >> 6) & 255u) : (uint32_t)(j * 64 + lane)];           \
            }                                                                                      \
            _Pragma("unroll") for (int j = 0; j < FE; j++) {                                       \
                if (fok[j] && (ftj[j] & 63u) == tt) {                                              \
                    const uint32_t o_ = (ftj[j] >> 6) & 255u;                                      \
                    vals[o_] = old_[j] + fx[j];                                                    \
                    if (AND) mcnt[o_] = (uint8_t)(mcnt[o_] + 1);                                   \
                }                                                                                  \
            }                                                                                      \
            wave_sync();                                                                           \
        }
        if (total > 0 && tb_min < dl) { NS_FOREIGN_RMW(tb_min, min(tb_max, dl - 1)); }

        bool driver_progress = false;
        for (;;) {
            const uint32_t remd = d_end - d_cur;
            if (remd == 0) break;
            uint32_t n;
            nat_u2 ps[DE];
            float nr[DE];
            float tfv[DE];
            uint32_t sbits[DE];
            uint32_t cnt = 0, r_hits = 0;
            NS_CNT(8, 1);
            float dx[DE];
            uint64_t dokm[DE];
            uint32_t first_pos, last_pos;
            if (PK) {
                static_assert(DE == 4, "a packed round is one block of 4 chunks");
                const uint32_t blk = d_cur >> 8;
                const uint32_t a = d_cur & 255u;
                const uint32_t e = min(256u, d_end - (blk << 8));
                n = e - a;
                first_pos = a; last_pos = e - 1u;
                uint32_t docs_[4];
                pk_decode_round<IMP, PK>(seg, blk, lane, docs_, tfv, nr, sbits);
#pragma unroll
                for (int j = 0; j < DE; j++) { ps[j].x = docs_[j]; ps[j].y = sbits[j]; }
                if (n == (uint32_t)(DE * 64)) {
#pragma unroll
                    for (int j = 0; j < DE; j++) {
                        dokm[j] = wballot(ps[j].x <= hi);
                        cnt += (uint32_t)__popcll(dokm[j]);
                    }
                } else {
#pragma unroll
                    for (int j = 0; j < DE; j++) {
                        const uint32_t c0 = (uint32_t)(j * 64);
                        const uint64_t vm = lane_span(a > c0 ? a - c0 : 0u, e > c0 ? min(e - c0, 64u) : 0u);
                        dokm[j] = wballot(ps[j].x <= hi) & vm;
                        cnt += (uint32_t)__popcll(dokm[j]);
                    }
                }
            } else {
                n = min(remd, (uint32_t)(DE * 64));
                first_pos = 0u; last_pos = n - 1u;
                const gp_u2 sp = stream + d_cur;
                const gp_f32 np = pnorm + d_cur;
#pragma unroll
                for (int j = 0; j < DE; j++) {
                    ps[j] = sp[j * 64 + lane];
                    nr[j] = IMP ? 0.0f : np[j * 64 + lane];
                    tfv[j] = (float)ps[j].y;
                }
                if (n == (uint32_t)(DE * 64)) {
#pragma unroll
                    for (int j = 0; j < DE; j++) {
                        dokm[j] = wballot(ps[j].x <= hi);
                        cnt += (uint32_t)__popcll(dokm[j]);
                    }
                } else {
#pragma unroll
                    for (int j = 0; j < DE; j++) {
                        const uint32_t left = (n > (uint32_t)(j * 64)) ? (n - (uint32_t)(j * 64)) : 0u;
                        const uint64_t nmask = (left >= 64u) ? ~0ull : ((1ull << left) - 1ull);
                        dokm[j] = wballot(ps[j].x <= hi) & nmask;
                        cnt += (uint32_t)__popcll(dokm[j]);
                    }
                }
            }
            NS_CNT(12, (n + 63) / 64);
            {
                float num[DE], den[DE];
#pragma unroll
                for (int j = 0; j < DE; j++) {
                    const float tf = tfv[j];
                    den[j] = tf + nr[j];
                    num[j] = d_idf * (tf * (1.2f + 1.0f));
                }
                if (IMP) {
#pragma unroll
                    for (int j = 0; j < DE; j++) dx[j] = __uint_as_float(ps[j].y);
                } else {
                    ns_div_n<DE>(dx, num, den, fast_div);
                }
#pragma unroll
                for (int j = 0; j < DE; j++) dx[j] = d_wq * dx[j];
                if (signed_in) {
// ... 19 lines not shown
#pragma unroll
                for (int j = 0; j < FE; j++) here = here || (fok[j] && fdoc[j] >= rfirst && fdoc[j] <= rlast);
                any_foreign_here = wballot(here) != 0ull;
            }
            if (any_foreign_here) {
#pragma unroll
                for (int j = 0; j < DE; j++) {
                    if (dokm[j] == 0ull) continue;
                    const uint32_t tag = NS_TAG(ps[j].x);
                    const uint32_t hb = NS_BUCKET(ps[j].x);
                    uint32_t b = hb;
                    uint4 q = ent4[b];
                    const uint64_t cm = wballot((q.x >> 16) == tag) | wballot((q.y >> 16) == tag) |
                                        wballot((q.z >> 16) == tag) | wballot((q.w >> 16) == tag);
                    const uint64_t go = dokm[j] & (cm | wballot(q.w != EMPTY));
                    if (go != 0ull) {
                        const uint32_t ident = NS_IDENT(ps[j].x, hb);
                        uint32_t m = 0;
                        bool more = __builtin_amdgcn_inverse_ballot_w64(go);
                        while (wballot(more) != 0ull) {
                            if (more) {
                                m = ((q.x ^ ident) < 256u) ? q.x : m;
                                m = ((q.y ^ ident) < 256u) ? q.y : m;
                                m = ((q.z ^ ident) < 256u) ? q.z : m;
                                m = ((q.w ^ ident) < 256u) ? q.w : m;
                                more = m == 0 && q.w != EMPTY;
                                if (more) { b = (b + 1) & (uint32_t)(NB - 1); q = ent4[b]; }
                            }
                        }
                        const uint64_t hitm = wballot(m != 0);
                        if (hitm != 0ull) {
                            if (m != 0) {
                                const uint32_t o = m & 255u;
                                vals[o] = vals[o] + dx[j];
                                if (AND) mcnt[o] = (uint8_t)(mcnt[o] + 1);
                            }
                            dokm[j] &= ~hitm;
                            r_hits += (uint32_t)__popcll(hitm);
                        }
                    }
                }
            }
            if (!AND || T == 1) {
                found_s += cnt - r_hits;
#pragma unroll
                for (int j = 0; j < DE; j++) {
                    top.offer_mask_stream(dokm[j], dx[j], ps[j].x);
                }
            }
            NS_CNT(9, cnt);
            NS_CNT(13, any_foreign_here ? (n + 63) / 64 : 0);
            NS_CNT(14, r_hits);
            d_cur += cnt;
            driver_progress = driver_progress || (cnt > 0);
            if (cnt < n) break;
        }

        if (total > 0) {
            if (tb_max > dl) { NS_FOREIGN_RMW(max(tb_min, dl + 1), tb_max); }
            float fin[FE];
            bool scored[FE];
#pragma unroll
            for (int j = 0; j < FE; j++) {
                fin[j] = vals[j * 64 + lane];
                scored[j] = fmine[j];
                if (AND && fmine[j]) scored[j] = (mcnt[j * 64 + lane] == (uint8_t)T);
            }
            wave_sync();
#pragma unroll
            for (int j = 0; j < FE; j++) {
                vals[j * 64 + lane] = 0.0f;
                if (fmine[j]) {
                    ent[ftj[j] >> 14] = EMPTY;
                    if (AND) mcnt[j * 64 + lane] = 0;
                }
                found_s += (uint32_t)__popcll(wballot(scored[j]));
                top.offer(scored[j], fin[j], fdoc[j]);
            }
            wave_sync();
        }
        top.keep_room();

        if (hi >= last_doc) break;
        if (Rf == 0 && d_cur >= d_end) break;
        if (total == 0 && !driver_progress) break;
        lo = hi + 1;
    }
#undef NS_FOREIGN_RMW
#undef NS_PLAN_FOREIGN
#undef NS_TAG
#undef NS_IDENT
#undef NS_BUCKET

#ifdef NS_COUNT
    const unsigned long long cyc_t1_ = __builtin_readcyclecounter();
#endif
    top.write_out(it.seg, it.out_slot, found_s, out_hits, out_nhits, out_found);
#ifdef NS_COUNT
    cnt_[17] = __builtin_readcyclecounter() - cyc_t0_;
    cnt_[18] = __builtin_readcyclecounter() - cyc_t1_;
    if (lane == 0)
        for (int i = 0; i < kNsCnt; i++) if (cnt_[i]) atomicAdd(&g_ns_cnt[i], cnt_[i]);
#endif
}

template <int HK, int FB, bool AND>
__global__ void __launch_bounds__(256) k_dscore(const DevWItem* __restrict__ items, uint32_t n_items,
                                                const DevTerm* __restrict__ terms, const DevSeg* __restrict__ segs,
                                                Hit* __restrict__ out_hits, uint32_t* __restrict__ out_nhits,
                                                uint64_t* __restrict__ out_found, uint32_t K) {
    constexpr int WPB = 4;
    __shared__ __attribute__((aligned(16))) uint32_t s_ent[WPB][HK];
    __shared__ __attribute__((aligned(16))) float s_vals[WPB][FB];
    __shared__ __attribute__((aligned(16))) uint8_t s_mcnt[WPB][AND ? FB : 16];
    __shared__ uint64_t s_cand[WPB][256];
    __shared__ __attribute__((aligned(16))) uint4 s_tab[WPB][64];
    __shared__ uint32_t s_aux[WPB][64];
    const int wave = __builtin_amdgcn_readfirstlane((int)(threadIdx.x >> 6));
    const int lane = threadIdx.x & 63;
    const uint32_t item_idx = blockIdx.x * WPB + wave;
    if (item_idx >= n_items) return;
    const DevWItem it = items[item_idx];
    dscore_body<HK / 4, FB, AND>(it, terms, segs, s_ent[wave], s_vals[wave], s_mcnt[wave], s_cand[wave], s_tab[wave], s_aux[wave],
                                 out_hits, out_nhits, out_found, K, lane);
}

}
```

### nextsearch-api_amd/csrc/ns_internal.h

```cpp
#pragma once
#include <stdint.h>

namespace ns {

static constexpr uint32_t kTileEmptyBits = 0xFFFFFFFFu;
static constexpr uint32_t kPkBlock = 256;
static constexpr uint32_t kPkStrideDwords = 512;
static constexpr uint32_t kPkTf = 0, kPkNormA = 64, kPkNormB = 128, kPkDoc = 192;
static constexpr uint32_t kSkipDocs = 1024;
static constexpr uint32_t kBmxBlock = 256;

struct DevSeg {
    const uint2* postings;
    const float* pnorm;
    const float* norm;
    const uint2* impacts;
    const uint32_t* packed;
    const uint2* pk_hdr;
    const float* ntab;
    const float* pk_scores;
    const uint32_t* skips;
    const float* blockmax;
    uint64_t     n_postings;
    uint32_t     n_docs;
    uint32_t     n_tiles;
};

struct DevTerm {
    uint64_t list_off;
    uint32_t count;
    float    idf;
    float    weight;
    uint32_t seg;
    uint32_t skip;
    uint32_t bmx;
};

struct DevShare {
    uint32_t first;
    uint32_t count;
    float    idf;
    uint32_t seg;
    uint32_t before;
};

struct DevItem {
    uint64_t bounds_off;
    uint32_t query;
    uint32_t seg;
    uint32_t term_begin;
    uint32_t term_count;
    uint32_t tile_begin;
    uint32_t tile_end;
    uint32_t out_slot;
    uint32_t pad;
};

struct DevWItem {
    uint32_t query;
    uint32_t seg;
    uint32_t term_begin;
    uint32_t term_count;
    uint32_t doc_lo;
    uint32_t doc_hi;
    uint32_t out_slot;
    uint32_t whole;
};

struct DevGroup {
    uint64_t bounds_off;
    uint32_t term_begin;
    uint32_t term_count;
    uint32_t seg;
    uint32_t pad;
};

struct DevQuery {
    uint32_t part_begin;
    uint32_t part_count;
};
constexpr bool merge_is_wide(uint32_t part_count, uint32_t K) { return part_count > 64 && part_count >= K; }

#ifndef NS_WIN_SLACK_THIN
#define NS_WIN_SLACK_THIN 1
#endif
#ifndef NS_WIN_SLACK_GEN
#define NS_WIN_SLACK_GEN 3
#endif
static constexpr uint32_t kWinSlackThin = NS_WIN_SLACK_THIN, kWinSlackGen = NS_WIN_SLACK_GEN;
#if defined(__HIPCC__) || defined(__CUDACC__)
#define NS_HD __host__ __device__
#else
#define NS_HD
#endif
NS_HD inline uint32_t foreign_slack(uint32_t c, uint32_t FB, uint32_t nact, uint32_t Rf) {
    if (Rf <= FB - nact) return 1u;
    if (2u * c * nact > FB) return 1u;
    return c;
}
NS_HD inline float foreign_scale(uint32_t c_eff, uint32_t FB, uint32_t nact, float rcp_Rf) {
    return (float)((int)FB - (int)(c_eff * nact)) * rcp_Rf;
}
NS_HD inline uint32_t foreign_window(uint32_t rem, uint32_t c_eff, float scale) {
    const uint32_t w = c_eff + (uint32_t)((float)rem * scale);
    return (w < rem) ? w : rem;
}

struct Hit {
    float    score;
    uint32_t seg;
    uint32_t doc;
};

}
```

### nextsearch-api_amd/csrc/ns_plan.hpp

```cpp
#pragma once
#include <algorithm>
#include <cmath>
#include <cstdarg>
#include <cstdio>
#include <cstring>
#include <functional>
#include <map>
#include <memory>
#include <string>
#include <thread>
#include <vector>

#include "../../include/nextsearch_hip.h"
#include "ns_forkjoin.hpp"
#include "ns_internal.h"

namespace ns {

struct VariantDesc { uint32_t hb; uint32_t nt, spt, u; uint32_t d; };
static const VariantDesc kVariants[] = {
    {512, 512, 12, 4, 0},
    {0, 1024, 12, 4, 0},
    {0, 512, 12, 4, 0},
    {0, 256, 16, 4, 0},
    {0, 512, 16, 8, 0},
    {0, 0, 0, 0, 0},
    {0, 0, 0, 0, 0}, {0, 0, 0, 0, 0}, {0, 0, 0, 0, 0}, {0, 0, 0, 0, 0}, {0, 0, 0, 0, 0}, {0, 0, 0, 0, 0},
    {512, 512, 12, 4, 0},
    {256, 512, 12, 4, 0},
    {1024, 512, 12, 4, 0},
    {512, 512, 12, 4, 0},
    {512, 512, 12, 4, 0},
    {1024, 512, 12, 4, 0},
    {512, 512, 12, 4, 1},
    {1024, 512, 12, 4, 1},
    {2048, 512, 12, 4, 1},
};
static constexpr uint32_t kNumVariants = sizeof(kVariants) / sizeof(kVariants[0]);
static constexpr uint32_t kWaveMaxTerms = 64;
static constexpr uint32_t kDefaultSplitPostings = 32768;
static constexpr uint32_t kSplitWorkSmallK = 98304, kSplitWorkLargeK = 131072;
static constexpr uint64_t kWorkForeign = 8, kWorkTile = 2, kWorkMerge = 4;
static constexpr uint32_t kSkipMinCount = 64;
static constexpr uint64_t kItemTermGeneral = 4000, kItemTermThin = 3000, kItemTermTile = 8000;

inline std::string vformat(const char* fmt, va_list ap) {
    char buf[512];
    std::vsnprintf(buf, sizeof(buf), fmt, ap);
    return buf;
}

template <class V>
class ListTable {
public:
    bool empty() const { return n_ == 0; }
    size_t slot_of(uint64_t key) const { return (size_t)((key * 0x9E3779B97F4A7C15ull) >> 20) & (slots_.size() - 1); }
    void prefetch(uint64_t key) const { if (!slots_.empty()) __builtin_prefetch(&slots_[slot_of(key)]); }
    const V* find(uint64_t key) const {
        if (slots_.empty()) return nullptr;
        for (size_t h = slot_of(key);; h = (h + 1) & (slots_.size() - 1)) {
            if (slots_[h].key == key) return &slots_[h].v;
            if (slots_[h].key == kFree) return nullptr;
        }
    }
    V& insert(uint64_t key, bool* fresh) {
        if (2 * n_ >= slots_.size()) rebuild(std::max<size_t>(16, slots_.size() * 2));
        for (size_t h = slot_of(key);; h = (h + 1) & (slots_.size() - 1)) {
            Slot& s = slots_[h];
            if (s.key == key) { *fresh = false; return s.v; }
            if (s.key == kFree) { s.key = key; n_++; *fresh = true; return s.v; }
        }
    }
    void put(uint64_t key, const V& v) { bool fresh; insert(key, &fresh) = v; }
    template <class F> void for_each(F fn) { for (Slot& s : slots_) if (s.key != kFree) fn(s.key, s.v); }
    template <class F> void erase_if(F pred) { refill(slots_.size(), pred); }
    void clear() { slots_.clear(); n_ = 0; }

private:
    static constexpr uint64_t kFree = ~0ull;
    struct Slot { uint64_t key = kFree; V v{}; };
    void rebuild(size_t cap) { refill(cap, [](uint64_t, const V&) { return false; }); }
    template <class F> void refill(size_t cap, F drop) {
        std::vector<Slot> old(cap);
        old.swap(slots_);
        n_ = 0;
        for (const Slot& s : old) if (s.key != kFree && !drop(s.key, s.v)) put(s.key, s.v);
    }
    std::vector<Slot> slots_;
    size_t n_ = 0;
};

struct SegLists {
    struct Imp { uint32_t count, idf_bits; };
    struct Skip { uint32_t count, entry; };
    struct Bmx { uint32_t count, idf_bits, entry; };
    ListTable<Imp> imp;
    ListTable<Skip> skip;
    ListTable<Bmx> bmx;
    std::map<uint32_t, uint32_t> share_lists;
    bool share_admit(uint32_t first, uint32_t count) {
        auto it = share_lists.lower_bound(first);
        if (it != share_lists.end() && (it->first == first ? it->second != count : (uint64_t)first + count > it->first)) return false;
        if (it != share_lists.begin() && (it == share_lists.end() || it->first != first)) {
            auto pv = std::prev(it);
            if ((uint64_t)pv->first + pv->second > first) return false;
        }
        share_lists.emplace(first, count);
        return true;
    }
    bool imp_has(uint32_t first, uint32_t count, uint32_t idf_bits) const {
        const Imp* e = imp.find(first);
        return e && e->count == count && e->idf_bits == idf_bits;
    }
    uint32_t skip_of(uint32_t first, uint32_t count) const {
        const Skip* e = skip.find(first);
        return e && e->count == count ? e->entry + 1u : 0u;
    }
    uint32_t bmx_of(uint32_t first, uint32_t count, uint32_t idf_bits) const {
        const Bmx* e = bmx.find(first);
        return e && e->count == count && e->idf_bits == idf_bits ? e->entry + 1u : 0u;
    }
};

struct SegView {
    uint32_t n_docs = 0, n_tiles = 0;
    uint64_t n_postings = 0;
    bool norm_safe = false;
    bool packed = false;
    SegLists* lists = nullptr;
};

struct ShareRegistry {
    struct Ent { uint32_t count, idf_bits, epoch; bool bad; };
    ListTable<Ent> tab;
    uint32_t epoch = 0;
    uint32_t live = 0;
};

struct PlanSettings {
    uint32_t variant = 0;
    uint32_t min_items = 0;
    uint32_t split_postings = 0;
    int n_cus = 0;
    bool use_impacts = true;
    int use_packed = 1;
    bool use_skips = true;
    bool use_merge = true;
    uint32_t merge_ratio = 8;
    bool use_pruning = false;
    int share_mode = 1;
    uint32_t share_ratio = 48;
    uint64_t share_min_postings = 4u << 20;
    unsigned prep_threads = 0;
    int order_mode = 1, order_coarse = 3;
    bool order_coarse_forced = false;
    uint32_t key_pct[4] = {100, 100, 100, 100};
    uint32_t tile_dens64 = 16;
};

inline size_t place_at(size_t& off, size_t bytes) {
    const size_t o = off;
    off = (off + std::max<size_t>(bytes, 1) + 255) & ~(size_t)255;
    return o;
}


struct HostGroup { DevGroup g; uint32_t query; uint64_t cost; uint64_t cmax; uint64_t work; bool wave; uint8_t cls; bool fast_div; bool signed_in; bool grid; bool merge2; };

constexpr uint32_t kOrderBuckets = 2048;
inline uint32_t order_bucket(uint64_t c) {
    if (c < 32) return kOrderBuckets - 1 - (uint32_t)c;
    const int b = 63 - __builtin_clzll(c);
    const uint32_t key = (uint32_t)b * 32u + (uint32_t)((c >> (b - 5)) & 31u);
    return kOrderBuckets - 1 - std::min(key, kOrderBuckets - 1);
}

struct PrepSlice {
    uint32_t q0 = 0, q1 = 0;
    std::vector<DevTerm> dterms;
    std::vector<HostGroup> groups;
    std::vector<uint32_t> qgroup_begin;
    std::vector<uint32_t> seg_ids;
    uint64_t bounds_total = 0, postings_total = 0, total_work = 0;
    bool all_imp = true, all_pk = true, any_pruned = false;
    int err_code = NS_OK;
    uint32_t err_query = 0xFFFFFFFFu;
    std::string err_msg;
    std::vector<DevWItem> witems;
    std::vector<uint16_t> wbucket;
    std::vector<uint32_t> wshare;
    std::vector<DevItem> items;
    std::vector<uint64_t> item_cost;
    std::vector<DevGroup> bgroups;
    uint32_t n_rows = 0;
    bool direct = true;
    std::vector<uint32_t> hist;
    uint32_t term_off = 0, row_off = 0, bgroup_off = 0;
    uint64_t bounds_off = 0;
    std::vector<uint32_t> start;
    void reset(uint32_t a, uint32_t b) {
        q0 = a; q1 = b;
        dterms.clear(); groups.clear(); qgroup_begin.clear(); seg_ids.clear();
        bounds_total = postings_total = total_work = 0; all_imp = true; all_pk = true; any_pruned = false;
        err_code = NS_OK; err_query = 0xFFFFFFFFu; err_msg.clear();
        witems.clear(); wbucket.clear(); wshare.clear(); items.clear(); item_cost.clear(); bgroups.clear();
        n_rows = 0; direct = true;
        hist.assign(2 * kOrderBuckets, 0u);
        start.assign(2 * kOrderBuckets, 0u);
        term_off = row_off = bgroup_off = 0; bounds_off = 0;
    }
    void fail_at(uint32_t q, int code, const char* fmt, ...) {
        if (err_code != NS_OK) return;
        va_list ap;
        va_start(ap, fmt);
        err_msg = vformat(fmt, ap);
        va_end(ap);
        err_code = code; err_query = q;
    }
};

struct BatchPlan {
    std::string err;
    uint32_t n_dterms = 0, n_rows = 0, n_witems = 0, n_items = 0, n_bgroups = 0;
    uint32_t n_class[3] = {0, 0, 0};
    uint64_t bounds_total = 0, postings_total = 0;
    bool direct = false;
    bool all_imp = false, all_pk = false, pruned = false;
    bool shared = false;
    std::vector<DevShare> share_build;
    uint64_t share_postings = 0;
    std::vector<uint32_t> wide_q;
    struct Layout { size_t items, witems, terms, groups, queries, segs, wideq, share, bytes; } layout{};
    bool deal = false;
    uint32_t deal_shift = 0;
    std::vector<uint32_t> bucket_pos;

    const PlanSettings* cfg = nullptr;
    const std::vector<SegView>* segs = nullptr;
    const ns_query_desc* queries = nullptr;
    const ns_term_ref* terms = nullptr;
    uint32_t n_queries = 0, k = 0, flags = 0;
    bool auto_mode = false, want_imp = false;
    unsigned width = 1;
    uint32_t G = 0;
    uint64_t total_work = 0;
    std::vector<PrepSlice> slices;
    std::vector<DevQuery> dq;
    std::vector<DevItem> sorted_items;
    std::vector<uint32_t> share_at;
    std::vector<std::vector<DevWItem>> deal_tmp;
    std::vector<std::vector<uint64_t>> deal_key, deal_alt;
    std::vector<std::vector<uint32_t>> deal_bins;
    std::unique_ptr<ForkJoin> pool;

    int failed(int code, const char* fmt, ...) {
        va_list ap;
        va_start(ap, fmt);
        err = vformat(fmt, ap);
        va_end(ap);
        return code;
    }
    void fork(const std::function<void(unsigned)>& fn) {
        if (width == 1) fn(0); else pool->run(width, fn);
    }

    int group(const PlanSettings& C, const std::vector<SegView>& SV, ShareRegistry& reg, const ns_query_desc* queries_,
              const ns_term_ref* terms_, uint32_t n_queries_, uint32_t k_, uint32_t flags_) {
        cfg = &C; segs = &SV; queries = queries_; terms = terms_; n_queries = n_queries_; k = k_; flags = flags_;
        const bool wave_path = kVariants[C.variant].hb != 0;
        auto_mode = C.variant == 0;

        width = 1;
        if (n_queries >= 3000 && C.prep_threads != 1) {
            unsigned want = C.prep_threads ? C.prep_threads : std::min<unsigned>(std::max(1u, std::thread::hardware_concurrency()), 8u);
            uint64_t n_refs = 0;
            for (uint32_t q = 0; q < n_queries; q++) n_refs += queries[q].term_count;
            width = std::max(1u, std::min<unsigned>(want, std::max<unsigned>(n_queries / 1500, (unsigned)std::min<uint64_t>(n_refs / 6000, 64))));
        }
        if (width > 1 && (!pool || pool->width() < width)) pool.reset(new ForkJoin(width));
        if (slices.size() < width) slices.resize(width);
        for (unsigned s = 0; s < width; s++) slices[s].reset((uint32_t)((uint64_t)n_queries * s / width), (uint32_t)((uint64_t)n_queries * (s + 1) / width));
        want_imp = C.use_impacts && auto_mode;

        fork([&](unsigned si) {
            PrepSlice& S = slices[si];
            S.all_imp = want_imp;
            S.qgroup_begin.reserve(S.q1 - S.q0 + 1);
            for (uint32_t q = S.q0; q < S.q1; q++) {
                S.qgroup_begin.push_back((uint32_t)S.groups.size());
                const ns_query_desc qd = queries[q];
                if (qd.term_count && !terms) { S.fail_at(q, NS_E_INVAL, "terms is NULL"); break; }
                S.seg_ids.clear();
                bool bad = false;
                for (uint32_t i = 0; i < qd.term_count && !bad; i++) {
                    const ns_term_ref& r = terms[qd.term_begin + i];
                    if (r.seg_id >= SV.size() || !SV[r.seg_id].lists) { S.fail_at(q, NS_E_INVAL, "query %u term %u: unknown segment %u", q, i, r.seg_id); bad = true; break; }
                    const SegView& s = SV[r.seg_id];
                    if (r.byte_off % 8 != 0) { S.fail_at(q, NS_E_INVAL, "query %u term %u: byte_off %llu not a multiple of 8", q, i, (unsigned long long)r.byte_off); bad = true; break; }
                    if (r.byte_off / 8 + r.count > s.n_postings) { S.fail_at(q, NS_E_INVAL, "query %u term %u: list [%llu,+%u) outside segment %u (%llu postings)", q, i, (unsigned long long)(r.byte_off / 8), r.count, r.seg_id, (unsigned long long)s.n_postings); bad = true; break; }
                    if (std::find(S.seg_ids.begin(), S.seg_ids.end(), r.seg_id) == S.seg_ids.end()) S.seg_ids.push_back(r.seg_id);
                }
                if (bad) break;
                std::sort(S.seg_ids.begin(), S.seg_ids.end());
                for (uint32_t sid : S.seg_ids) {
                    const SegView& sv = SV[sid];
                    HostGroup hg{};
                    hg.fast_div = sv.norm_safe;
                    if (!sv.packed) S.all_pk = false;
                    hg.g.term_begin = (uint32_t)S.dterms.size();
                    hg.g.seg = sid;
                    hg.query = q;
                    for (uint32_t i = 0; i < qd.term_count; i++) {
                        const ns_term_ref& r = terms[qd.term_begin + i];
                        if (r.seg_id != sid) continue;
                        DevTerm t{};
                        t.list_off = r.byte_off / 8;
                        t.count = r.count;
                        t.idf = r.idf;
                        t.weight = r.qweight;
                        t.seg = sid;
                        S.dterms.push_back(t);
                        hg.cost += r.count;
                        hg.cmax = std::max<uint64_t>(hg.cmax, r.count);
                        if (S.all_imp) {
                            uint32_t ib; std::memcpy(&ib, &r.idf, 4);
                            S.all_imp = sv.lists->imp_has((uint32_t)(r.byte_off / 8), r.count, ib);
                        }
                        if (!(r.idf >= 9.313225746154785e-10f && r.idf <= 1073741824.0f)) hg.fast_div = false;
                        if (std::signbit(r.idf) || std::signbit(r.qweight)) hg.signed_in = true;
                    }
                    hg.g.term_count = (uint32_t)S.dterms.size() - hg.g.term_begin;
                    if ((flags & NS_FLAG_AND) && hg.g.term_count > 255) { S.fail_at(q, NS_E_INVAL, "AND mode supports at most 255 term refs per (query, segment)"); bad = true; break; }
                    hg.wave = wave_path && hg.g.term_count <= kWaveMaxTerms;
                    {
                        const uint64_t rest = hg.cost - hg.cmax;
                        const uint32_t nd = std::max<uint32_t>(sv.n_docs, 1);
                        if (rest * 32 <= hg.cmax) hg.cls = 1;
                        else if (hg.g.term_count >= 2 && hg.cost * 64 >= (uint64_t)nd * C.tile_dens64) hg.cls = 2;
                        else hg.cls = 0;
                        hg.work = !auto_mode ? hg.cost : (hg.cls == 2 ? hg.cost * kWorkTile : hg.cmax + rest * kWorkForeign);
                        hg.merge2 = auto_mode && C.use_merge && hg.cls == 0 && hg.g.term_count == 2 && rest * C.merge_ratio >= hg.cmax;
                        if (hg.merge2) hg.work = hg.cmax + rest * kWorkMerge;
                    }
                    if (!hg.wave) {
                        hg.g.bounds_off = S.bounds_total;
                        S.bounds_total += (uint64_t)(sv.n_tiles + 1) * hg.g.term_count;
                    }
                    S.postings_total += hg.cost;
                    S.total_work += hg.work;
                    S.groups.push_back(hg);
                }
                if (bad) break;
            }
            S.qgroup_begin.resize(S.q1 - S.q0 + 1, (uint32_t)S.groups.size());
        });
        {
            const PrepSlice* first = nullptr;
            for (unsigned s = 0; s < width; s++)
                if (slices[s].err_code != NS_OK && (!first || slices[s].err_query < first->err_query)) first = &slices[s];
            if (first) return failed(first->err_code, "%s", first->err_msg.c_str());
        }
        bounds_total = postings_total = total_work = 0;
        n_dterms = G = 0;
        all_imp = want_imp; all_pk = C.use_packed != 0 && auto_mode;
        for (unsigned s = 0; s < width; s++) {
            PrepSlice& S = slices[s];
            S.term_off = n_dterms; S.bounds_off = bounds_total;
            n_dterms += (uint32_t)S.dterms.size(); G += (uint32_t)S.groups.size();
            bounds_total += S.bounds_total; postings_total += S.postings_total; total_work += S.total_work;
            all_imp = all_imp && S.all_imp;
            all_pk = all_pk && S.all_pk;
        }
        if (bounds_total >= (1ull << 32)) return failed(NS_E_INVAL, "batch too large: %llu boundary entries; split the batch", (unsigned long long)bounds_total);

        share_build.clear();
        share_postings = 0;
        shared = false;
        if (!all_imp && want_imp && C.share_mode != 0 && !all_pk && postings_total > 0 &&
            (C.share_mode == 2 || postings_total >= C.share_min_postings)) {
            shared = true;
            if (++reg.epoch == 0) {
                reg.tab.for_each([](uint64_t, ShareRegistry::Ent& en) { en.epoch = 0; });
                reg.epoch = 1;
            }
            const uint32_t epoch = reg.epoch;
            for (unsigned sl = 0; sl < width && shared; sl++) {
                const std::vector<DevTerm>& dts = slices[sl].dterms;
                for (size_t ti = 0; ti < dts.size(); ti++) {
                    if (ti + 8 < dts.size()) reg.tab.prefetch(((uint64_t)dts[ti + 8].seg << 32) | (uint32_t)dts[ti + 8].list_off);
                    const DevTerm& t = dts[ti];
                    if (!t.count) continue;
                    SegLists* sg = SV[t.seg].lists;
                    uint32_t ib; std::memcpy(&ib, &t.idf, 4);
                    const uint32_t first = (uint32_t)t.list_off;
                    if (!sg->imp.empty()) {
                        if (sg->imp_has(first, t.count, ib)) continue;
                        shared = false; break;
                    }
                    bool fresh = false;
                    ShareRegistry::Ent& en = reg.tab.insert(((uint64_t)t.seg << 32) | first, &fresh);
                    if (fresh) { en.count = t.count; en.idf_bits = ib; en.epoch = 0; en.bad = !sg->share_admit(first, t.count); }
                    if (en.bad || en.count != t.count) { shared = false; break; }
                    if (en.idf_bits != ib) {
                        if (reg.live || en.epoch == epoch) { shared = false; break; }
                        en.idf_bits = ib;
                    }
                    if (en.epoch != epoch) {
                        en.epoch = epoch;
                        if (share_postings + t.count >= (1ull << 32)) { shared = false; break; }
                        share_build.push_back(DevShare{first, t.count, t.idf, t.seg, (uint32_t)share_postings});
                        share_postings += t.count;
                        if (C.share_mode == 1 && share_postings * C.share_ratio > postings_total) { shared = false; break; }
                    }
                }
            }
            if (shared && C.share_mode == 1 && postings_total < (uint64_t)C.share_ratio * share_postings) shared = false;
        }
        return NS_OK;
    }

    int cut() {
        const PlanSettings& C = *cfg;
        const std::vector<SegView>& SV = *segs;
        if (shared) all_imp = true;
        else { share_build.clear(); share_postings = 0; }

        const uint32_t min_items = C.min_items ? C.min_items : (uint32_t)std::max(C.n_cus, 1) * 24u;
        int small_mode = 0;
        uint64_t split_postings = C.split_postings ? C.split_postings
                                  : (!auto_mode ? kDefaultSplitPostings : (k <= 32 ? kSplitWorkSmallK : kSplitWorkLargeK));
        bool fine_cut = false;
        if (!C.split_postings && auto_mode) {
            const uint64_t fine = total_work / ((uint64_t)std::max(C.n_cus, 1) * 96u);
            fine_cut = fine < split_postings;
            split_postings = std::min<uint64_t>(split_postings, std::max<uint64_t>(fine, 16384));
            const uint64_t per_slot = total_work / ((uint64_t)std::max(C.n_cus, 1) * 24u);
            small_mode = per_slot >= 2 * split_postings ? 0 : (per_slot >= split_postings ? 1 : 2);
        }
        uint32_t chunks_per_group = 1;
        if (G > 0 && G < min_items) chunks_per_group = std::min<uint32_t>((min_items + G - 1) / G, 1024u);
        dq.assign(n_queries, DevQuery{});

        fork([&](unsigned si) {
            PrepSlice& S = slices[si];
            for (uint32_t q = S.q0; q < S.q1; q++) {
                dq[q].part_begin = S.n_rows;
                for (uint32_t gi = S.qgroup_begin[q - S.q0]; gi < S.qgroup_begin[q - S.q0 + 1]; gi++) {
                    HostGroup& hg = S.groups[gi];
                    hg.g.term_begin += S.term_off;
                    const SegView& sg = SV[hg.g.seg];
                    if (sg.n_docs == 0) continue;
                    if (hg.wave) {
                        DevTerm* dt = S.dterms.data() + (hg.g.term_begin - S.term_off);
                        uint64_t sp_ = (auto_mode && hg.cls != 0) ? split_postings * 2 : split_postings;
                        if (auto_mode && hg.cls != 0 && small_mode) sp_ = small_mode == 2 ? split_postings / 2 : split_postings;
                        const uint64_t want = std::max<uint64_t>((hg.work + sp_ - 1) / sp_, chunks_per_group);
                        uint32_t ns = (uint32_t)std::min<uint64_t>(std::max<uint64_t>(want, 1), std::min<uint32_t>(sg.n_docs, 4096));
                        if (auto_mode && ns > 1) {
                            uint32_t p2 = 1;
                            while (p2 < ns) p2 <<= 1;
                            if (!small_mode && (uint64_t)ns * ns * 2 < (uint64_t)p2 * p2) p2 >>= 1;
                            if (k > 32 && p2 < 8) p2 = 8;
                            ns = std::min<uint32_t>(p2, std::min<uint32_t>(sg.n_docs, 4096));
                        }
                        if (auto_mode && C.use_skips && (hg.cls == 2 || ns > 1) && !sg.lists->skip.empty()) {
                            for (uint32_t ti = 0; ti < hg.g.term_count; ti++) {
                                if (dt[ti].count < kSkipMinCount) continue;
                                dt[ti].skip = sg.lists->skip_of((uint32_t)dt[ti].list_off, dt[ti].count);
                                if (dt[ti].skip) hg.grid = true;
                            }
                        }
                        bool pruned_ = false;
                        if (auto_mode && C.use_pruning && hg.g.term_count == 1 && !sg.lists->bmx.empty()) {
                            uint32_t ib; std::memcpy(&ib, &dt[0].idf, 4);
                            if (dt[0].idf > 0.0f && std::isfinite(dt[0].idf) && dt[0].weight > 0.0f && std::isfinite(dt[0].weight)) {
                                dt[0].bmx = sg.lists->bmx_of((uint32_t)dt[0].list_off, dt[0].count, ib);
                                pruned_ = dt[0].bmx != 0;
                            }
                            if (pruned_) S.any_pruned = true;
                        }
                        const uint64_t per_term = hg.cls == 2 ? kItemTermTile : (hg.cls == 1 ? kItemTermThin : kItemTermGeneral);
                        uint64_t key = hg.work / ns + 1 + (auto_mode ? per_term * hg.g.term_count : 0);
                        if (fine_cut && hg.cls == 0) key = key * 5 / 8;
                        else if (auto_mode && k > 32 && hg.cls == 0) key = key * 3 / 4;
                        if (auto_mode) key = key * C.key_pct[hg.merge2 ? 3 : hg.cls] / 100;
                        const bool wide = auto_mode && hg.g.term_count > 16;
                        const uint32_t bucket = order_bucket(key);
                        uint64_t big_off = 0;
                        for (uint32_t ti = 0, cm = 0; ti < hg.g.term_count; ti++)
                            if (dt[ti].count >= cm) { cm = dt[ti].count; big_off = dt[ti].list_off; }
                        for (uint32_t i = 0; i < ns; i++) {
                            DevWItem it{};
                            it.query = q;
                            it.seg = hg.g.seg;
                            it.term_begin = hg.g.term_begin;
                            it.term_count = hg.g.term_count;
                            it.doc_lo = (uint32_t)((uint64_t)sg.n_docs * i / ns);
                            it.doc_hi = (uint32_t)((uint64_t)sg.n_docs * (i + 1) / ns);
                            if (hg.grid) {
                                it.doc_lo -= it.doc_lo % kSkipDocs;
                                if (i + 1 < ns) it.doc_hi -= it.doc_hi % kSkipDocs;
                            }
                            if (it.doc_hi <= it.doc_lo) continue;
                            it.out_slot = S.n_rows++;
                            it.whole = (ns == 1 ? 1u : 0u) | (hg.fast_div ? 8u : 0u) | (hg.signed_in ? 16u : 0u) | (hg.grid ? (hg.cls == 2 ? 32u : 64u) : 0u);
                            if (auto_mode) it.whole |= (hg.cls == 2 ? 2u : 0u) | (hg.cls == 1 ? 4u : 0u) | (pruned_ ? 128u : 0u) | (hg.merge2 && hg.wave ? 256u : 0u);
                            S.witems.push_back(it);
                            S.wbucket.push_back((uint16_t)(bucket | (wide ? 0x8000u : 0u)));
                            {
                                uint64_t h = big_off * 0x9E3779B97F4A7C15ull;
                                h ^= h >> 29;
                                const uint32_t r12 = (uint32_t)(((uint64_t)it.doc_lo << 12) / std::max<uint32_t>(sg.n_docs, 1u)) & 4095u;
                                S.wshare.push_back(((it.seg & 63u) << 26) | (r12 << 14) | (uint32_t)((h >> 40) & 0x3FFFu));
                            }
                            S.hist[(wide ? kOrderBuckets : 0) + bucket]++;
                        }
                    } else {
                        DevGroup g = hg.g;
                        g.bounds_off += S.bounds_off;
                        S.bgroups.push_back(g);
                        const uint32_t nt = sg.n_tiles;
                        const uint32_t chunks = std::min(chunks_per_group, nt);
                        const uint32_t per = (nt + chunks - 1) / chunks;
                        for (uint32_t tb = 0; tb < nt; tb += per) {
                            DevItem it{};
                            it.bounds_off = g.bounds_off;
                            it.query = q;
                            it.seg = g.seg;
                            it.term_begin = g.term_begin;
                            it.term_count = g.term_count;
                            it.tile_begin = tb;
                            it.tile_end = std::min(nt, tb + per);
                            it.out_slot = S.n_rows++;
                            S.item_cost.push_back(hg.cost * (it.tile_end - it.tile_begin) / nt + 1);
                            S.items.push_back(it);
                        }
                    }
                }
                dq[q].part_count = S.n_rows - dq[q].part_begin;
                if (dq[q].part_count != 1) S.direct = false;
            }
        });
        n_rows = n_witems = n_items = n_bgroups = 0;
        direct = n_queries > 0;
        pruned = false;
        for (unsigned s = 0; s < width; s++) {
            PrepSlice& S = slices[s];
            S.row_off = n_rows; S.bgroup_off = n_bgroups;
            n_rows += S.n_rows; n_witems += (uint32_t)S.witems.size(); n_items += (uint32_t)S.items.size(); n_bgroups += (uint32_t)S.bgroups.size();
            direct = direct && S.direct;
            pruned = pruned || S.any_pruned;
        }
        n_class[0] = n_class[1] = n_class[2] = 0;
        {
            uint32_t pos = 0;
            bucket_pos.assign(kOrderBuckets + 1, 0u);
            for (uint32_t half = 0; half < 2; half++) {
                for (uint32_t bkt = 0; bkt < kOrderBuckets; bkt++) {
                    if (half == 0) bucket_pos[bkt] = pos;
                    for (unsigned s = 0; s < width; s++) {
                        slices[s].start[half * kOrderBuckets + bkt] = pos;
                        pos += slices[s].hist[half * kOrderBuckets + bkt];
                    }
                }
                if (half == 0) { n_class[0] = pos; bucket_pos[kOrderBuckets] = pos; }
            }
            n_class[1] = pos - n_class[0];
            if (pos != n_witems) return failed(NS_E_STATE, "internal: launch order holds %u of %u work items", pos, n_witems);
            if (!auto_mode) { n_class[0] = n_class[1] = 0; }
        }
        sorted_items.clear();
        if (n_items) {
            struct Cost { uint64_t c; uint32_t slice, idx; };
            std::vector<Cost> ic;
            ic.reserve(n_items);
            for (unsigned s = 0; s < width; s++)
                for (uint32_t i = 0; i < slices[s].items.size(); i++) ic.push_back({slices[s].item_cost[i], s, i});
            std::stable_sort(ic.begin(), ic.end(), [](const Cost& a, const Cost& b) { return a.c > b.c; });
            sorted_items.resize(n_items);
            for (uint32_t i = 0; i < n_items; i++) {
                DevItem it = slices[ic[i].slice].items[ic[i].idx];
                it.out_slot = direct ? it.query : it.out_slot + slices[ic[i].slice].row_off;
                sorted_items[i] = it;
            }
        }
        wide_q.clear();
        if (!direct)
            for (uint32_t q = 0; q < n_queries; q++)
                if (merge_is_wide(dq[q].part_count, k)) wide_q.push_back(q);

        size_t off = 0;
        layout.items = place_at(off, (size_t)n_items * sizeof(DevItem));
        layout.witems = place_at(off, (size_t)n_witems * sizeof(DevWItem));
        layout.terms = place_at(off, (size_t)n_dterms * sizeof(DevTerm));
        layout.groups = place_at(off, (size_t)n_bgroups * sizeof(DevGroup));
        layout.queries = place_at(off, dq.size() * sizeof(DevQuery));
        layout.segs = place_at(off, SV.size() * sizeof(DevSeg));
        layout.wideq = place_at(off, wide_q.size() * 4);
        layout.share = place_at(off, shared ? (share_build.size() + 1) * sizeof(DevShare) : 0);
        layout.bytes = off;

        uint64_t resident_bytes = 0;
        for (const SegView& sv : SV) resident_bytes += sv.n_postings * 12ull;
        deal = C.order_mode >= 1 && auto_mode && n_class[0] >= 64 && (width >= 4 || resident_bytes > (256ull << 20) || C.order_mode >= 2);
        deal_shift = C.order_coarse_forced ? (uint32_t)C.order_coarse : (resident_bytes > (256ull << 20) ? 4u : 3u);
        return NS_OK;
    }

    void write(char* hb) {
        if (deal && share_at.size() < n_witems) share_at.resize(n_witems);
        fork([&](unsigned si) {
            PrepSlice& S = slices[si];
            DevWItem* wdst = (DevWItem*)(hb + layout.witems);
            for (size_t i = 0; i < S.witems.size(); i++) {
                DevWItem it = S.witems[i];
                it.out_slot = direct ? it.query : it.out_slot + S.row_off;
                const uint32_t bk = S.wbucket[i];
                const uint32_t at = S.start[((bk & 0x8000u) ? kOrderBuckets : 0) + (bk & 0x7FFFu)]++;
                wdst[at] = it;
                if (deal) share_at[at] = S.wshare[i];
            }
            if (!S.dterms.empty()) std::memcpy(hb + layout.terms + (size_t)S.term_off * sizeof(DevTerm), S.dterms.data(), S.dterms.size() * sizeof(DevTerm));
            if (!S.bgroups.empty()) std::memcpy(hb + layout.groups + (size_t)S.bgroup_off * sizeof(DevGroup), S.bgroups.data(), S.bgroups.size() * sizeof(DevGroup));
            for (uint32_t q = S.q0; q < S.q1; q++) dq[q].part_begin += S.row_off;
            if (S.q1 > S.q0) std::memcpy(hb + layout.queries + (size_t)S.q0 * sizeof(DevQuery), dq.data() + S.q0, (size_t)(S.q1 - S.q0) * sizeof(DevQuery));
        });
        if (deal) {
            DevWItem* wd = (DevWItem*)(hb + layout.witems);
            const uint32_t shift = deal_shift, n_cls = kOrderBuckets >> shift;
            if (deal_tmp.size() < width) { deal_tmp.resize(width); deal_key.resize(width); deal_alt.resize(width); deal_bins.resize(width); }
            fork([&](unsigned si) {
                std::vector<DevWItem>& tmp = deal_tmp[si];
                std::vector<uint64_t>& ord = deal_key[si];
                for (uint32_t c = si; c < n_cls; c += width) {
                    const uint32_t p0 = bucket_pos[c << shift], p1 = bucket_pos[(c + 1) << shift];
                    const uint32_t n = p1 - p0;
                    if (n < 16) continue;
                    ord.resize(n);
                    for (uint32_t i = 0; i < n; i++) ord[i] = ((uint64_t)share_at[p0 + i] << 32) | i;
                    if (n <= 4096) {
                        std::sort(ord.begin(), ord.end());
                    } else {
                        std::vector<uint64_t>& alt = deal_alt[si];
                        std::vector<uint32_t>& bins = deal_bins[si];
                        alt.resize(n);
                        bins.resize(65537);
                        for (int pass = 0; pass < 2; pass++) {
                            const int sh = 32 + 16 * pass;
                            std::fill(bins.begin(), bins.end(), 0u);
                            const uint64_t* src = pass ? alt.data() : ord.data();
                            uint64_t* dst = pass ? ord.data() : alt.data();
                            for (uint32_t i = 0; i < n; i++) bins[((src[i] >> sh) & 0xFFFFu) + 1u]++;
                            for (uint32_t b2 = 0; b2 < 65536; b2++) bins[b2 + 1] += bins[b2];
                            for (uint32_t i = 0; i < n; i++) dst[bins[(src[i] >> sh) & 0xFFFFu]++] = src[i];
                        }
                    }
                    tmp.assign(wd + p0, wd + p1);
                    uint32_t cur[8], end[8];
                    for (uint32_t x = 0; x < 8; x++) { cur[x] = (uint32_t)((uint64_t)n * x / 8); end[x] = (uint32_t)((uint64_t)n * (x + 1) / 8); }
                    for (uint32_t p = 0; p < n; p++) {
                        uint32_t x = (p0 + p) & 7u;
                        for (uint32_t tr = 0; tr < 8 && cur[x] >= end[x]; tr++) x = (x + 1) & 7u;
                        wd[p0 + p] = tmp[(uint32_t)ord[cur[x]++]];
                    }
                }
            });
        }
        if (n_items) std::memcpy(hb + layout.items, sorted_items.data(), (size_t)n_items * sizeof(DevItem));
        if (!wide_q.empty()) std::memcpy(hb + layout.wideq, wide_q.data(), wide_q.size() * 4);
        if (shared) {
            std::memcpy(hb + layout.share, share_build.data(), share_build.size() * sizeof(DevShare));
            const DevShare sentinel{0u, 0u, 0.0f, 0u, (uint32_t)share_postings};
            std::memcpy(hb + layout.share + share_build.size() * sizeof(DevShare), &sentinel, sizeof(DevShare));
        }
    }
};

}
```

### nextsearch-api_amd/nsbind.py

```python
import ctypes as C
import os

import numpy as np

HERE = os.path.dirname(os.path.abspath(__file__))
HIP_LIB_PATH = os.environ.get("NS_HIP_LIB") or os.path.join(HERE, "libnextsearch_hip.so")
HOST_LIB_PATH = os.path.join(HERE, "libnextsearch_host.so")

NS_OK = 0
NS_FLAG_OR = 0
NS_FLAG_AND = 1
NS_SORT_DESC, NS_SORT_ASC = 0, 0x1000
NS_ROLE_SHOULD, NS_ROLE_MUST, NS_ROLE_NOT = 0, 1, 2
NS_INFO_IMPACTS = 0x100
NS_INFO_PACKED = 0x200
NS_INFO_PRUNED = 0x400
NS_INFO_SHARED = 0x800
NS_MAX_K = 100


class NsTermRef(C.Structure):
    _fields_ = [("seg_id", C.c_uint32), ("count", C.c_uint32), ("byte_off", C.c_uint64),
                ("idf", C.c_float), ("qweight", C.c_float)]


class NsQueryDesc(C.Structure):
    _fields_ = [("term_begin", C.c_uint32), ("term_count", C.c_uint32)]


class NsHit(C.Structure):
    _fields_ = [("score", C.c_float), ("seg_id", C.c_uint32), ("doc_id", C.c_uint32)]


class NsBatchInfo(C.Structure):
    _fields_ = [("postings", C.c_uint64), ("algo_bytes", C.c_uint64), ("n_queries", C.c_uint32),
                ("n_items", C.c_uint32), ("n_term_refs", C.c_uint32), ("tile_docs", C.c_uint32),
                ("k", C.c_uint32), ("flags", C.c_uint32), ("last_score_kernel_ms", C.c_float),
                ("last_total_ms", C.c_float), ("timed_runs", C.c_uint32), ("shared_lists", C.c_uint32),
                ("sum_score_kernel_ms", C.c_double), ("sum_total_ms", C.c_double), ("shared_postings", C.c_uint64)]


HIT_DTYPE = np.dtype([("score", "<f4"), ("seg", "<u4"), ("doc", "<u4")])
TERM_DTYPE = np.dtype([("seg_id", "<u4"), ("count", "<u4"), ("byte_off", "<u8"), ("idf", "<f4"), ("qweight", "<f4")])
QDESC_DTYPE = np.dtype([("term_begin", "<u4"), ("term_count", "<u4")])
assert HIT_DTYPE.itemsize == C.sizeof(NsHit) == 12
assert TERM_DTYPE.itemsize == C.sizeof(NsTermRef) == 24
assert QDESC_DTYPE.itemsize == C.sizeof(NsQueryDesc) == 8

HIP_SYMBOLS = [
    "ns_facet_upload", "ns_facet_release", "ns_facet_count", "ns_facet_tile_docs",
    "ns_dockeys_upload", "ns_dockeys_release", "ns_search_sorted", "ns_sorted_kernel_ms",
    "ns_search_boolean", "ns_boolean_kernel_ms",
    "ns_segment_filter",
    "ns_ctx_create", "ns_ctx_destroy", "ns_ctx_set_stream", "ns_last_error", "ns_device_name",
    "ns_segment_upload", "ns_segment_release", "ns_segment_upload_begin", "ns_segment_upload_append", "ns_segment_upload_end", "ns_search_batch", "ns_batch_prepare",
    "ns_batch_bind_outputs", "ns_batch_run", "ns_batch_stream", "ns_batch_gap_ms", "ns_batch_sync", "ns_batch_fetch", "ns_batch_get_info",
    "ns_batch_destroy", "ns_set_tuning", "ns_segment_build_impacts", "ns_ctx_use_impacts", "ns_ctx_set_host_threads", "ns_ctx_set_overlap", "ns_segment_build_packed", "ns_ctx_use_packed", "ns_segment_build_skips", "ns_ctx_use_skips", "ns_segment_build_blockmax", "ns_ctx_use_pruning", "ns_ctx_use_merge", "ns_ctx_share_scores",
    "ns_invert_forward", "ns_segment_upload_inverted", "ns_merge_rank_rows", "ns_sem_upload", "ns_sem_release", "ns_sem_topk",
    "ns_ac_upload", "ns_ac_suggest", "ns_ac_release", "ns_ac_build_fuzzy", "ns_ac_fuzzy", "ns_ac_fuzzy_prefix",
    "ns_forward_build", "ns_forward_get_info", "ns_forward_fetch", "ns_forward_destroy",
    "ns_forward_merge", "ns_forward_invert", "ns_compact_doc_cut", "ns_ctx_use_docsort",
    "ns_forward_merge_keep",
    "ns_docterms_upload", "ns_docterms_select", "ns_docterms_destroy", "ns_docterms_doc_cut",
]
HOST_SYMBOLS = [
    "nsh_parse_boolean", "nsh_engine_search_boolean_batch", "nsh_engine_search_boolean_json",
    "nsh_engine_sort_keys", "nsh_engine_search_sorted_batch", "nsh_engine_search_sorted_json", "nsh_engine_release_sorted", "nsh_engine_sort_tables_on_device",
    "nsh_engine_facet_buckets", "nsh_engine_facet_batch", "nsh_engine_search_faceted_json", "nsh_engine_release_facets", "nsh_engine_facet_tables_on_device",
    "nsh_date_key", "nsh_engine_filter_bits", "nsh_engine_open_filter", "nsh_engine_open_filter_bits", "nsh_engine_close_filter", "nsh_engine_open_filters",
    "nsh_engine_search_filtered_batch", "nsh_engine_search_filtered_json",
    "nsh_gen_index", "nsh_engine_open", "nsh_engine_open_multi", "nsh_engine_num_devices", "nsh_shard_bounds", "nsh_engine_close", "nsh_engine_reload", "nsh_engine_error", "nsh_engine_ctx",
    "nsh_engine_num_segments", "nsh_engine_segment_name", "nsh_engine_segment_info",
    "nsh_engine_segment_doc_len", "nsh_engine_segment_postings", "nsh_engine_lookup", "nsh_bm25_idf",
    "nsh_base_terms", "nsh_engine_build_refs", "nsh_engine_search_json", "nsh_free",
    "nsh_engine_search_batch", "nsh_engine_prepare", "nsh_engine_doc_metadata", "nsh_engine_hits_to_json", "nsh_engine_search_batch_json",
    "nsh_engine_build_impacts", "nsh_engine_use_impacts", "nsh_engine_build_packed", "nsh_engine_use_packed", "nsh_engine_build_blockmax", "nsh_engine_use_pruning", "nsh_engine_use_merge", "nsh_engine_share_scores", "nsh_engine_use_skips", "nsh_invert_segment", "nsh_invert_error",
    "nsh_engine_semantic_info", "nsh_engine_expand", "nsh_engine_semantic_row", "nsh_engine_set_cache", "nsh_engine_cache_size",
    "nsh_engine_suggest_json", "nsh_engine_suggest_batch", "nsh_engine_suggest_table", "nsh_suggest_split", "nsh_suggest_clamp_limit",
    "nsh_engine_correct_batch", "nsh_engine_did_you_mean_json", "nsh_correct_auto_edits", "nsh_engine_correct_build_ms",
    "nsh_engine_complete_batch", "nsh_engine_complete_json",
    "nsh_index_documents", "nsh_index_error", "nsh_engine_open_noload", "nsh_engine_add_documents",
    "nsh_merge_segments", "nsh_compact_error", "nsh_engine_compact",
    "nsh_engine_find_documents", "nsh_engine_delete_documents", "nsh_engine_delete_by_id",
    "nsh_similar_select_host", "nsh_similar_clamp_terms", "nsh_similar_clamp_k", "nsh_similar_qweight", "nsh_similar_defaults",
    "nsh_engine_similar_term_stats", "nsh_engine_similar_batch", "nsh_engine_more_like_this_json", "nsh_engine_release_similar",
    "nsh_engine_similar_segments_on_device",
]

class NsForwardInfo(C.Structure):
    _fields_ = [("struct_size", C.c_uint32), ("kept_docs", C.c_uint32), ("n_terms", C.c_uint32), ("n_docs", C.c_uint32),
                ("n_pairs", C.c_uint64), ("term_bytes", C.c_uint64), ("n_tokens", C.c_uint64), ("kept_tokens", C.c_uint64),
                ("device_bytes", C.c_uint64), ("device_ms", C.c_float), ("pad", C.c_uint32)]


class NshIndexStats(C.Structure):
    _fields_ = [("struct_size", C.c_uint32), ("n_docs_in", C.c_uint32), ("n_docs", C.c_uint32), ("n_terms", C.c_uint32),
                ("text_bytes", C.c_uint64), ("tokens", C.c_uint64), ("kept_tokens", C.c_uint64), ("pairs", C.c_uint64),
                ("device_bytes", C.c_uint64), ("avgdl", C.c_float), ("device_ms", C.c_float), ("call_s", C.c_double), ("total_s", C.c_double)]

    def as_dict(self):
        return {k: getattr(self, k) for k, _ in self._fields_ if k != "struct_size"}


class NsForwardSrc(C.Structure):
    _fields_ = [("n_docs", C.c_uint32), ("doc_len", C.c_void_p), ("counts", C.c_void_p), ("n_pairs", C.c_uint64), ("pairs", C.c_void_p),
                ("n_terms", C.c_uint32), ("term_bytes", C.c_void_p), ("term_offsets", C.c_void_p)]


class NshCompactStats(C.Structure):
    _fields_ = [("struct_size", C.c_uint32), ("sources", C.c_uint32), ("n_docs", C.c_uint32), ("n_terms", C.c_uint32),
                ("terms_in", C.c_uint64), ("pairs", C.c_uint64), ("device_bytes", C.c_uint64),
                ("merge_ms", C.c_float), ("invert_ms", C.c_float), ("call_s", C.c_double), ("total_s", C.c_double)]

    def as_dict(self):
        return {k: getattr(self, k) for k, _ in self._fields_ if k != "struct_size"}


class NshDeleteStats(C.Structure):
    _fields_ = [("struct_size", C.c_uint32), ("segments_rewritten", C.c_uint32), ("segments_dropped", C.c_uint32), ("docs_deleted", C.c_uint32),
                ("uids_not_found", C.c_uint32), ("terms_dropped", C.c_uint32),
                ("pairs_in", C.c_uint64), ("pairs_out", C.c_uint64), ("device_bytes", C.c_uint64),
                ("merge_ms", C.c_float), ("invert_ms", C.c_float), ("call_s", C.c_double), ("total_s", C.c_double)]

    def as_dict(self):
        return {k: getattr(self, k) for k, _ in self._fields_ if k != "struct_size"}


class NshFacetSpec(C.Structure):
    _fields_ = [("kind", C.c_uint32), ("n_custom_labels", C.c_uint32), ("custom_buckets", C.c_void_p), ("n_custom", C.c_uint64),
                ("custom_labels", C.POINTER(C.c_char_p))]


FACET_KINDS = {"year": 0, "month": 1, "custom": 2}


class NshSortSpec(C.Structure):
    _fields_ = [("kind", C.c_uint32), ("ascending", C.c_uint32), ("custom_keys", C.c_void_p), ("n_custom", C.c_uint64)]


SORT_ORDERS = {"newest": (0, 0), "oldest": (0, 1)}

_hip = None
_host = None


def hip_lib():
    global _hip
    if _hip is None:
        if not os.path.exists(HIP_LIB_PATH):
            raise RuntimeError(f"{HIP_LIB_PATH} is missing: build it with `make -C nextsearch-api_amd` "
                               "(there is no fallback path)")
        L = C.CDLL(HIP_LIB_PATH, mode=C.RTLD_GLOBAL)
        vp, u32, u64, i32 = C.c_void_p, C.c_uint32, C.c_uint64, C.c_int
        L.ns_ctx_create.argtypes = [i32, C.POINTER(vp)]
        L.ns_ctx_destroy.argtypes = [vp]
        L.ns_ctx_destroy.restype = None
        L.ns_ctx_set_stream.argtypes = [vp, vp]
        L.ns_ac_upload.argtypes = [vp, vp, vp, vp, u32, C.POINTER(vp)]
        L.ns_ac_suggest.argtypes = [vp, vp, vp, vp, u32, u32, vp, vp, C.POINTER(C.c_float)]
        L.ns_ac_release.argtypes = [vp, vp]
        L.ns_ac_build_fuzzy.argtypes = [vp, vp, C.POINTER(C.c_float)]
        L.ns_ac_fuzzy.argtypes = [vp, vp, vp, vp, u32, vp, u32, u32, vp, vp, vp, C.POINTER(C.c_float)]
        L.ns_ac_fuzzy_prefix.argtypes = [vp, vp, vp, vp, u32, vp, u32, u32, vp, vp, vp, C.POINTER(C.c_float)]
        L.ns_last_error.argtypes = [vp]
        L.ns_last_error.restype = C.c_char_p
        L.ns_device_name.argtypes = [vp]
        L.ns_device_name.restype = C.c_char_p
        L.ns_segment_upload.argtypes = [vp, u32, u32, C.c_float, vp, vp, u64, C.POINTER(vp)]
        L.ns_segment_release.argtypes = [vp, vp]
        L.ns_segment_upload_begin.argtypes = [vp, u32, u32, C.c_float, vp, u64, C.POINTER(vp)]
        L.ns_segment_upload_append.argtypes = [vp, vp, vp, u64]
        L.ns_segment_upload_end.argtypes = [vp, vp]
        L.ns_segment_build_impacts.argtypes = [vp, vp, vp, vp, vp, u32]
        L.ns_ctx_use_impacts.argtypes = [vp, i32]
        L.ns_segment_build_skips.argtypes = [vp, vp, vp, vp, u32]
        L.ns_ctx_use_skips.argtypes = [vp, i32]
        L.ns_segment_filter.argtypes = [vp, vp, u32, vp, vp, vp, u32, vp, vp, vp, C.POINTER(u64), C.POINTER(C.c_float), C.POINTER(vp)]
        L.ns_ctx_set_host_threads.argtypes = [vp, u32]
        L.ns_ctx_set_overlap.argtypes = [vp, i32]
        L.ns_segment_build_packed.argtypes = [vp, vp]
        L.ns_ctx_use_packed.argtypes = [vp, i32]
        L.ns_segment_build_blockmax.argtypes = [vp, vp, vp, vp, vp, u32]
        L.ns_ctx_use_pruning.argtypes = [vp, i32]
        L.ns_ctx_use_merge.argtypes = [vp, i32]
        L.ns_ctx_share_scores.argtypes = [vp, i32]
        L.ns_sem_upload.argtypes = [vp, vp, u32, u32, C.POINTER(vp)]
        L.ns_sem_release.argtypes = [vp, vp]
        L.ns_sem_topk.argtypes = [vp, vp, vp, u32, u32, C.c_float, vp, vp, vp, vp, vp, vp]
        L.ns_merge_rank_rows.argtypes = [vp, vp, vp, vp, u32, u32, u32, vp, u32, vp, vp, vp]
        L.ns_invert_forward.argtypes = [vp, vp, u32, vp, u64, u32, vp, vp, C.POINTER(u64), vp]
        L.ns_segment_upload_inverted.argtypes = [vp, vp, vp, vp, u64, u32, vp, vp, C.POINTER(u64), vp]
        L.ns_search_batch.argtypes = [vp, vp, vp, u32, u32, vp, vp, vp, u32]
        L.ns_batch_prepare.argtypes = [vp, vp, vp, u32, u32, u32, C.POINTER(vp)]
        L.ns_batch_bind_outputs.argtypes = [vp, vp, vp, vp]
        L.ns_batch_run.argtypes = [vp, i32]
        L.ns_batch_gap_ms.argtypes = [vp, vp, C.POINTER(C.c_float)]
        L.ns_batch_stream.argtypes = [vp]
        L.ns_batch_stream.restype = vp
        L.ns_batch_sync.argtypes = [vp]
        L.ns_batch_fetch.argtypes = [vp, vp, vp, vp]
        L.ns_batch_get_info.argtypes = [vp, C.POINTER(NsBatchInfo)]
        L.ns_batch_destroy.argtypes = [vp]
        L.ns_batch_destroy.restype = None
        L.ns_set_tuning.argtypes = [vp, u32, u32, u32]
        L.ns_forward_build.argtypes = [vp, vp, u64, vp, u32, C.POINTER(vp)]
        L.ns_forward_get_info.argtypes = [vp, C.POINTER(NsForwardInfo)]
        L.ns_forward_fetch.argtypes = [vp, vp, vp, vp, vp, vp, vp]
        L.ns_forward_destroy.argtypes = [vp]
        L.ns_forward_destroy.restype = None
        L.ns_forward_merge.argtypes = [vp, vp, u32, C.POINTER(vp)]
        L.ns_forward_invert.argtypes = [vp, vp, vp, C.POINTER(u64), vp]
        L.ns_compact_doc_cut.argtypes = []
        L.ns_compact_doc_cut.restype = u32
        L.ns_ctx_use_docsort.argtypes = [vp, i32]
        L.ns_forward_merge_keep.argtypes = [vp, vp, vp, u32, C.POINTER(vp)]
        L.ns_docterms_upload.argtypes = [vp, vp, vp, vp, C.POINTER(vp)]
        L.ns_docterms_select.argtypes = [vp, vp, u32, u32, u32, u32, u32, vp, vp, vp, C.POINTER(C.c_float)]
        L.ns_docterms_destroy.argtypes = [vp]
        L.ns_docterms_destroy.restype = None
        L.ns_docterms_doc_cut.argtypes = []
        L.ns_docterms_doc_cut.restype = u32
        L.ns_facet_upload.argtypes = [vp, u32, vp, u32, C.POINTER(vp)]
        L.ns_facet_release.argtypes = [vp, vp]
        L.ns_facet_count.argtypes = [vp, vp, u32, vp, u32, u32, vp, vp, vp, u32, vp, vp, C.POINTER(C.c_float)]
        L.ns_facet_tile_docs.argtypes = []
        L.ns_facet_tile_docs.restype = u32
        L.ns_dockeys_upload.argtypes = [vp, u32, vp, C.POINTER(vp)]
        L.ns_dockeys_release.argtypes = [vp, vp]
        L.ns_search_sorted.argtypes = [vp, vp, u32, vp, u32, u32, u32, vp, vp, vp, u32, vp, vp, vp, vp, C.POINTER(C.c_float)]
        L.ns_sorted_kernel_ms.argtypes = [C.POINTER(C.c_float), i32]
        L.ns_search_boolean.argtypes = [vp, vp, u32, vp, vp, u32, u32, vp, vp, u32, vp, vp, vp, C.POINTER(C.c_float)]
        L.ns_boolean_kernel_ms.argtypes = [C.POINTER(C.c_float), i32]
        for name in DEBUG_COUNTERS:
            if hasattr(L, name):
                getattr(L, name).argtypes = [C.POINTER(u64), i32]
        _hip = L
    return _hip


DEBUG_COUNTERS = {"ns_debug_counters": 32, "ns_debug_tile_counters": 12, "ns_debug_merge_counters": 16, "ns_debug_topk_counters": 4,
                  "ns_debug_join_counters": 16, "ns_debug_facet_counters": 8, "ns_debug_sorted_counters": 9,
                  "ns_debug_boolean_counters": 8}


def debug_counters(reset=False):
    L = hip_lib()
    out = {}
    for name, n in DEBUG_COUNTERS.items():
        if hasattr(L, name):
            buf = (C.c_uint64 * n)()
            if getattr(L, name)(buf, int(bool(reset))) != 0:
                raise RuntimeError(name + " failed")
            out[name] = [int(v) for v in buf]
    return out


def host_lib():
    global _host
    if _host is None:
        hip_lib()
        if not os.path.exists(HOST_LIB_PATH):
            raise RuntimeError(f"{HOST_LIB_PATH} is missing: build it with `make -C nextsearch-api_amd`")
        L = C.CDLL(HOST_LIB_PATH, mode=C.RTLD_GLOBAL)
        vp, u32, u64, i32 = C.c_void_p, C.c_uint32, C.c_uint64, C.c_int
        L.nsh_gen_index.argtypes = [C.c_char_p, u32, u32, u32, u64, i32, C.POINTER(u64)]
        L.nsh_engine_open.argtypes = [C.c_char_p, i32, C.POINTER(vp)]
        L.nsh_engine_open_multi.argtypes = [C.c_char_p, C.POINTER(i32), u32, C.POINTER(vp)]
        L.nsh_engine_num_devices.argtypes = [vp]
# ... 118 lines not shown
        L.nsh_engine_release_facets.argtypes = [vp]
        L.nsh_engine_release_facets.restype = None
        L.nsh_engine_facet_tables_on_device.argtypes = [vp]
        L.nsh_engine_facet_tables_on_device.restype = u64
        L.nsh_engine_sort_keys.argtypes = [vp, C.POINTER(NshSortSpec), vp, u64]
        L.nsh_engine_sort_keys.restype = C.c_int64
        L.nsh_engine_search_sorted_batch.argtypes = [vp, C.POINTER(NshSortSpec), u32, C.POINTER(C.c_char_p), u32, i32, u32, vp, vp, vp, vp, vp, C.POINTER(C.c_float)]
        L.nsh_engine_search_sorted_json.argtypes = [vp, C.c_char_p, i32, C.POINTER(NshSortSpec), i32, C.c_char_p, C.c_char_p, i32, C.POINTER(vp)]
        L.nsh_engine_release_sorted.argtypes = [vp]
        L.nsh_engine_release_sorted.restype = None
        L.nsh_engine_sort_tables_on_device.argtypes = [vp]
        L.nsh_engine_sort_tables_on_device.restype = u64
        L.nsh_parse_boolean.argtypes = [C.c_char_p, C.c_char_p, u32, vp, u32]
        L.nsh_parse_boolean.restype = u32
        L.nsh_engine_search_boolean_batch.argtypes = [vp, u32, C.POINTER(C.c_char_p), u32, i32, vp, vp, vp, vp, C.POINTER(C.c_float)]
        L.nsh_engine_search_boolean_json.argtypes = [vp, C.c_char_p, i32, i32, C.c_char_p, C.c_char_p, i32, C.POINTER(vp)]
        _host = L
    return _host


def _cstr_array(strings):
    arr = (C.c_char_p * len(strings))()
    arr[:] = [s.encode("utf-8") if isinstance(s, str) else s for s in strings]
    return arr


def clamp_k(k):
    return max(1, min(int(k), NS_MAX_K))


def gen_index(index_dir, n_segments, docs_per_segment, vocab=65536, seed=1337, legacy=False):
    total = C.c_uint64(0)
    rc = host_lib().nsh_gen_index(index_dir.encode(), n_segments, docs_per_segment, vocab, seed, int(legacy), C.byref(total))
    if rc != 0:
        raise RuntimeError(f"nsh_gen_index({index_dir}) failed")
    return total.value


class Batch:

    def __init__(self, handle, n_queries, k):
        self.h = handle
        self.Q = n_queries
        self.K = k

    def bind_outputs(self, d_hits, d_nhits, d_found):
        rc = hip_lib().ns_batch_bind_outputs(self.h, d_hits, d_nhits, d_found)
        if rc != NS_OK:
            raise RuntimeError("ns_batch_bind_outputs failed")

    def run(self, timed=False, fetch=False):
        rc = hip_lib().ns_batch_run(self.h, int(bool(timed)) | (2 if fetch else 0))
        if rc != NS_OK:
            raise RuntimeError(f"ns_batch_run failed rc={rc}")

    @property
    def stream(self):
        return hip_lib().ns_batch_stream(self.h)

    def sync(self):
        rc = hip_lib().ns_batch_sync(self.h)
        if rc != NS_OK:
            raise RuntimeError(f"ns_batch_sync failed rc={rc}")

    def fetch(self):
        hits = np.empty((self.Q, self.K), dtype=HIT_DTYPE)
        nhits = np.empty(self.Q, dtype=np.uint32)
        found = np.empty(self.Q, dtype=np.uint64)
        rc = hip_lib().ns_batch_fetch(self.h, hits.ctypes.data, nhits.ctypes.data, found.ctypes.data)
        if rc != NS_OK:
            raise RuntimeError(f"ns_batch_fetch failed rc={rc}")
        return hits, nhits, found

    def fetch_into(self, hits, nhits, found):
        rc = hip_lib().ns_batch_fetch(self.h, hits.ctypes.data, nhits.ctypes.data, found.ctypes.data)
        if rc != NS_OK:
            raise RuntimeError(f"ns_batch_fetch failed rc={rc}")

    def info(self):
        inf = NsBatchInfo()
        hip_lib().ns_batch_get_info(self.h, C.byref(inf))
        return inf

    def close(self):
        if self.h:
            hip_lib().ns_batch_destroy(self.h)
            self.h = None

    def __del__(self):
        self.close()


class Engine:

    def __init__(self, index_dir, device=0):
        self._L = host_lib()
        h = C.c_void_p()
        if isinstance(device, (list, tuple)):
            arr = (C.c_int32 * len(device))(*device)
            rc = self._L.nsh_engine_open_multi(index_dir.encode(), arr, len(device), C.byref(h))
        else:
            rc = self._L.nsh_engine_open(index_dir.encode(), device, C.byref(h))
        self.h = h
        if rc != 0:
            msg = self._L.nsh_engine_error(h).decode()
            self._L.nsh_engine_close(h)
            self.h = None
            raise RuntimeError(f"Engine.reload failed: {msg}")
        self.device = device

    @classmethod
    def create(cls, index_dir, device=0):
        self = cls.__new__(cls)
        self._L = host_lib()
        h = C.c_void_p()
        if self._L.nsh_engine_open_noload(str(index_dir).encode(), device, C.byref(h)) != 0:
            raise RuntimeError("nsh_engine_open_noload failed")
        self.h = h
        self.device = device
        return self

    def add_documents(self, docs):
        blob, offs = pack_documents(docs)
        st = NshIndexStats(struct_size=C.sizeof(NshIndexStats))
        old_ctx = self.ctx
        rc = self._L.nsh_engine_add_documents(self.h, blob, offs.ctypes.data, (len(offs) - 1) // 4, C.byref(st))
        if _ctx_key(self.ctx) != _ctx_key(old_ctx):
            _LIVE_BATCHES.pop(_ctx_key(old_ctx), None)
        if rc != 0:
            raise RuntimeError(f"Engine.add_documents failed: {self.error()}")
        return st.as_dict()

    def compact(self, first=0, count=None, remove_sources=True):
        st = NshCompactStats(struct_size=C.sizeof(NshCompactStats))
        old_ctx = self.ctx
        rc = self._L.nsh_engine_compact(self.h, int(first), 0xFFFFFFFFFFFFFFFF if count is None else int(count), 1 if remove_sources else 0, C.byref(st))
        if _ctx_key(self.ctx) != _ctx_key(old_ctx):
            _LIVE_BATCHES.pop(_ctx_key(old_ctx), None)
        if rc != 0:
            raise RuntimeError(f"Engine.compact failed: {self.error()}")
        return st.as_dict()

    def find_documents(self, uids):
        blob, offs = _flat_bytes(uids)
        cap = 64
        while True:
            out = np.zeros((cap, 2), dtype=np.uint32)
            n = self._L.nsh_engine_find_documents(self.h, blob, offs.ctypes.data, len(offs) - 1, out.ctypes.data, cap)
            if n < 0:
                raise RuntimeError(f"Engine.find_documents failed: {self.error()}")
            if n <= cap:
                return [(int(s), int(d)) for s, d in out[:n]]
            cap = int(n)

    def _deleted(self, rc, st, old_ctx, what):
        if _ctx_key(self.ctx) != _ctx_key(old_ctx):
            _LIVE_BATCHES.pop(_ctx_key(old_ctx), None)
        if rc != 0:
            raise RuntimeError(f"Engine.{what} failed: {self.error()}")
        return st.as_dict()

    def delete_documents(self, uids):
        blob, offs = _flat_bytes(uids)
        st = NshDeleteStats(struct_size=C.sizeof(NshDeleteStats))
        old_ctx = self.ctx
        rc = self._L.nsh_engine_delete_documents(self.h, blob, offs.ctypes.data, len(offs) - 1, C.byref(st))
# ... 1077 lines not shown
```

Measured before the change: 8.143 million.

## Share precomputed top rows of common driver terms across queries via row consumers

Adds a row-sharing mode, on by default. Producer items score a common driver term once into a top-kRowLen row. Consumer items then merge that shared row with their other terms instead of streaming the driver term's postings, finding matches through skip-table binary search. If the shared row turns out insufficient, the consumer falls back to the full scoring body. Producer and consumer kernels run on a forked stream so they overlap with the regular wide-item kernels. The cost is extra planning complexity, extra kernels and events, and a full recompute whenever the fallback triggers.

```diff
diff --git a/include/nextsearch_hip.h b/include/nextsearch_hip.h
--- a/include/nextsearch_hip.h
+++ b/include/nextsearch_hip.h
@@ -95,6 +95,9 @@
 int ns_ctx_use_pruning(ns_ctx* ctx, int on);
 int ns_ctx_use_merge(ns_ctx* ctx, int on);
 int ns_ctx_share_scores(ns_ctx* ctx, int mode);
+
+int ns_ctx_share_rows(ns_ctx* ctx, int mode);
+int ns_batch_row_stats(ns_batch* b, uint32_t out[4]);
 
 int ns_search_batch(ns_ctx* ctx, const ns_query_desc* queries, const ns_term_ref* terms,
                     uint32_t n_queries, uint32_t k, ns_hit* hits_out, uint32_t* nhits_out,
diff --git a/nextsearch-api_amd/csrc/ns_api.hip b/nextsearch-api_amd/csrc/ns_api.hip
--- a/nextsearch-api_amd/csrc/ns_api.hip
+++ b/nextsearch-api_amd/csrc/ns_api.hip
@@ -18,6 +18,7 @@
 #include "ns_prune_kernel.hip"
 #include "ns_merge_kernel.hip"
 #include "ns_tile_kernel.hip"
+#include "ns_row_kernel.hip"
 #include "ns_invert.hip"
 #include "ns_ingest.hip"
 #include "ns_compact.hip"
@@ -79,6 +80,7 @@
     hipStream_t alt_stream = nullptr;
     hipStream_t pull_stream = nullptr;
     bool overlap = false, flip = false;
+    hipStream_t row_stream = nullptr;
     std::string err;
     std::string devname;
     std::vector<ns_seg*> segs;
@@ -208,6 +210,14 @@
     if (const char* sm = std::getenv("NS_SHARE")) ctx->cfg.share_mode = std::max(0, std::min(2, std::atoi(sm)));
     if (const char* sr = std::getenv("NS_SHARE_RATIO")) ctx->cfg.share_ratio = (uint32_t)std::max(1, std::atoi(sr));
     if (const char* sp = std::getenv("NS_SHARE_MIN")) ctx->cfg.share_min_postings = (uint64_t)std::max(0ll, std::atoll(sp));
+    ctx->cfg.row_mode = 1;
+    if (const char* rm = std::getenv("NS_SHARE_ROWS")) ctx->cfg.row_mode = std::max(0, std::min(2, std::atoi(rm)));
+    if (const char* ru = std::getenv("NS_ROW_MIN_USERS")) ctx->cfg.row_min_users = (uint32_t)std::max(1, std::atoi(ru));
+    if (const char* rc = std::getenv("NS_ROW_CELL")) ctx->cfg.row_cell_postings = (uint32_t)std::max(1, std::atoi(rc));
+    {
+        const char* rf = std::getenv("NS_ROW_FORK");
+        if ((!rf || std::atoi(rf) != 0) && hipStreamCreateWithFlags(&ctx->row_stream, hipStreamNonBlocking) != hipSuccess) { ctx->row_stream = nullptr; (void)hipGetLastError(); }
+    }
     if (const char* oc = std::getenv("NS_ORDER_COARSE")) { ctx->cfg.order_coarse = std::max(0, std::min(11, std::atoi(oc))); ctx->cfg.order_coarse_forced = true; }
     if (hipStreamCreateWithFlags(&ctx->alt_stream, hipStreamNonBlocking) != hipSuccess) { ctx->alt_stream = nullptr; (void)hipGetLastError(); }
     {
@@ -225,6 +235,7 @@
     (void)hipStreamSynchronize(ctx->stream);
     if (ctx->alt_stream) (void)hipStreamSynchronize(ctx->alt_stream);
     if (ctx->pull_stream) (void)hipStreamSynchronize(ctx->pull_stream);
+    if (ctx->row_stream) (void)hipStreamSynchronize(ctx->row_stream);
     for (ns_seg* s : ctx->segs) {
         if (!s) continue;
         seg_free_device_fwd(s);
@@ -246,6 +257,7 @@
     if (ctx->own_stream) (void)hipStreamDestroy(ctx->own_stream);
     if (ctx->alt_stream) (void)hipStreamDestroy(ctx->alt_stream);
     if (ctx->pull_stream) (void)hipStreamDestroy(ctx->pull_stream);
+    if (ctx->row_stream) (void)hipStreamDestroy(ctx->row_stream);
     delete ctx;
 }
 
@@ -615,6 +627,13 @@
     if (!ctx) return fail(nullptr, NS_E_INVAL, "ns_ctx_share_scores: ctx is NULL");
     if (mode < 0 || mode > 2) return fail(ctx, NS_E_INVAL, "ns_ctx_share_scores: mode %d outside [0, 2]", mode);
     ctx->cfg.share_mode = mode;
+    return NS_OK;
+}
+
+extern "C" int ns_ctx_share_rows(ns_ctx* ctx, int mode) {
+    if (!ctx) return fail(nullptr, NS_E_INVAL, "ns_ctx_share_rows: ctx is NULL");
+    if (mode < 0 || mode > 2) return fail(ctx, NS_E_INVAL, "ns_ctx_share_rows: mode %d outside [0, 2]", mode);
+    ctx->cfg.row_mode = mode;
     return NS_OK;
 }
 
@@ -877,6 +896,14 @@
     uint32_t n_share = 0;
     uint64_t share_postings = 0;
     DevShare* d_share = nullptr;
+    uint32_t n_pitems = 0, n_ritems = 0;
+    DevWItem* d_pitems = nullptr;
+    DevRItem* d_ritems = nullptr;
+    Hit* d_row_hits = nullptr;
+    uint32_t* d_row_nhits = nullptr;
+    uint64_t* d_row_found = nullptr;
+    uint32_t* d_row_stats = nullptr;
+    hipEvent_t row_fork = nullptr, row_join = nullptr;
     DevItem* d_items = nullptr;
     DevWItem* d_witems = nullptr;
     DevTerm* d_terms = nullptr;
@@ -965,6 +992,8 @@
     for (auto& blk : b->blocks) pool_free(b->ctx, blk.first, blk.second);
     for (auto& e : b->ev_pool) if (e) (void)hipEventDestroy(e);
     if (b->done) (void)hipEventDestroy(b->done);
+    if (b->row_fork) (void)hipEventDestroy(b->row_fork);
+    if (b->row_join) (void)hipEventDestroy(b->row_join);
     delete b;
 }
 
@@ -1054,6 +1083,7 @@
     b->pk = (P.all_pk && P.postings_total > 0) ? ctx->cfg.use_packed : 0;
     b->pruned = P.pruned;
     b->n_wide_q = (uint32_t)P.wide_q.size();
+    b->n_pitems = P.n_pitems; b->n_ritems = P.n_ritems;
 
     hipError_t e = hipSuccess;
     auto chk = [&](hipError_t r) { if (e == hipSuccess) e = r; };
@@ -1069,6 +1099,12 @@
         o_pnhits = place(Pn * 4);
         o_pfound = place(Pn * 8);
         o_heads = place(Pn * 4);
+    }
+    size_t o_rhits = 0, o_rnhits = 0, o_rfound = 0;
+    if (b->n_pitems) {
+        o_rhits = place((size_t)b->n_pitems * kRowLen * sizeof(Hit));
+        o_rnhits = place((size_t)b->n_pitems * 4);
+        o_rfound = place((size_t)b->n_pitems * 8);
     }
     const size_t o_hits = place(Qn * k * sizeof(Hit));
     const size_t o_nhits = place(Qn * 4);
@@ -1085,6 +1121,14 @@
         b->d_wide_q = (uint32_t*)(base + L.wideq);
         b->d_share = (DevShare*)(base + L.share);
         b->d_bounds = (uint32_t*)(base + o_bounds);
+        if (b->n_pitems) {
+            b->d_pitems = (DevWItem*)(base + L.pitems);
+            b->d_ritems = (DevRItem*)(base + L.ritems);
+            b->d_row_hits = (Hit*)(base + o_rhits);
+            b->d_row_nhits = (uint32_t*)(base + o_rnhits);
+            b->d_row_found = (uint64_t*)(base + o_rfound);
+            b->d_row_stats = (uint32_t*)(base + L.rstats);
+        }
         if (!P.direct) {
             b->d_part_hits = (Hit*)(base + o_phits);
             b->d_part_nhits = (uint32_t*)(base + o_pnhits);
@@ -1200,6 +1244,25 @@
     Hit* sh = b->direct ? b->o_hits : b->d_part_hits;
     uint32_t* sn = b->direct ? b->o_nhits : b->d_part_nhits;
     uint64_t* sf = b->direct ? b->o_found : b->d_part_found;
+    const bool rows = b->n_pitems && b->n_ritems && b->variant == 0;
+    bool row_forked = false;
+    if (rows) {
+        hipStream_t ps = st;
+        if (ctx->row_stream) {
+            if (!b->row_fork) HIPCHK(ctx, hipEventCreateWithFlags(&b->row_fork, hipEventDisableTiming));
+            if (!b->row_join) HIPCHK(ctx, hipEventCreateWithFlags(&b->row_join, hipEventDisableTiming));
+            HIPCHK(ctx, hipEventRecord(b->row_fork, st));
+            HIPCHK(ctx, hipStreamWaitEvent(ctx->row_stream, b->row_fork, 0));
+            ps = ctx->row_stream;
+            row_forked = true;
+        }
+        launch_uscore<128, 16>(false, true, 0, b->n_pitems, ps, b->d_pitems, b->d_terms, b->d_segs, b->d_row_hits, b->d_row_nhits, b->d_row_found, kRowLen);
+        if (row_forked) {
+            hipLaunchKernelGGL((k_rscore<512, 128, 16>), dim3(b->n_ritems), dim3(64), 0, ps, b->d_ritems, b->n_ritems, b->d_terms, b->d_segs,
+                               b->d_row_hits, b->d_row_nhits, sh, sn, sf, b->K, b->d_row_stats);
+            HIPCHK(ctx, hipEventRecord(b->row_join, ps));
+        }
+    }
     if (b->n_witems && b->variant == 0) {
         const uint32_t n_narrow = b->n_class[0], n_wide = b->n_witems - b->n_class[0];
         const DevWItem* wide = b->d_witems + n_narrow;
@@ -1232,6 +1295,11 @@
 #undef NS_D
     }
 #endif
+    if (rows) {
+        if (row_forked) HIPCHK(ctx, hipStreamWaitEvent(st, b->row_join, 0));
+        else hipLaunchKernelGGL((k_rscore<512, 128, 16>), dim3(b->n_ritems), dim3(64), 0, st, b->d_ritems, b->n_ritems, b->d_terms, b->d_segs,
+                                b->d_row_hits, b->d_row_nhits, sh, sn, sf, b->K, b->d_row_stats);
+    }
     if (b->n_items) {
 #ifdef NS_VARIANTS
         const VariantDesc vd = kVariants[b->variant];
@@ -1386,7 +1454,7 @@
     info->postings = b->postings;
     info->algo_bytes = b->postings * 8;
     info->n_queries = b->Q;
-    info->n_items = b->n_items + b->n_witems;
+    info->n_items = b->n_items + b->n_witems + b->n_ritems + b->n_pitems;
     info->n_term_refs = b->n_terms;
     info->tile_docs = b->tile_docs;
     info->k = b->K;
@@ -1399,6 +1467,19 @@
     info->timed_runs = b->timed_runs;
     info->sum_score_kernel_ms = b->sum_score_ms;
     info->sum_total_ms = b->sum_total_ms;
+    return NS_OK;
+}
+
+extern "C" int ns_batch_row_stats(ns_batch* b, uint32_t out[4]) {
+    if (!b || !out) return NS_E_INVAL;
+    ns_ctx* ctx = b->ctx;
+    const bool rows = b->n_pitems && b->n_ritems && b->variant == 0;
+    out[0] = rows ? b->n_pitems : 0u; out[1] = rows ? b->n_ritems : 0u; out[2] = 0u; out[3] = 0u;
+    if (rows && b->ran) {
+        HIPCHK(ctx, hipSetDevice(ctx->device));
+        HIPCHK(ctx, hipMemcpyAsync(out + 2, b->d_row_stats, 8, hipMemcpyDeviceToHost, b->st));
+        HIPCHK(ctx, hipStreamSynchronize(b->st));
+    }
     return NS_OK;
 }
 
diff --git a/nextsearch-api_amd/csrc/ns_driver_kernel.hip b/nextsearch-api_amd/csrc/ns_driver_kernel.hip
--- a/nextsearch-api_amd/csrc/ns_driver_kernel.hip
+++ b/nextsearch-api_amd/csrc/ns_driver_kernel.hip
@@ -75,11 +75,14 @@
     return upto_hi & ~upto_lo;
 }
 
-template <int NB, int FB, bool AND, int CB = 256, bool IMP = false, int PK = 0>
-__device__ __forceinline__ void dscore_body(const DevWItem& it, const DevTerm* __restrict__ terms, const DevSeg* __restrict__ segs,
+struct RowArgs { const Hit* hits; uint32_t nhits; uint32_t dterm; uint32_t* stats; };
+
+template <int NB, int FB, bool AND, int CB = 256, bool IMP = false, int PK = 0, bool ROW = false>
+__device__ __forceinline__ bool dscore_body(const DevWItem& it, const DevTerm* __restrict__ terms, const DevSeg* __restrict__ segs,
                                             uint32_t* ent, float* vals, uint8_t* mcnt, uint64_t* cand, uint4* tab, uint32_t* aux,
                                             Hit* __restrict__ out_hits, uint32_t* __restrict__ out_nhits,
-                                            uint64_t* __restrict__ out_found, uint32_t K, const int lane) {
+                                            uint64_t* __restrict__ out_found, uint32_t K, const int lane, const RowArgs ra = RowArgs{}) {
+    static_assert(!ROW || (FB == 64 && !AND && IMP && PK == 0), "the row consumer is the thin OR body over shared term scores");
     constexpr int FE = FB / 64;
     constexpr int DE = 4;
     constexpr uint32_t EMPTY = 0u;
@@ -132,6 +135,7 @@
         dl = (uint32_t)__builtin_ctzll(wballot(remv == mx && (uint32_t)lane < T) | (1ull << 63));
         if (dl >= T) dl = 0;
     }
+    if constexpr (ROW) dl = ra.dterm;
     uint32_t d_cur = rdlane(cur, dl);
     const uint32_t d_end = rdlane(end, dl);
     const float d_idf = __uint_as_float(rdlane(idf_bits, dl));
@@ -156,6 +160,21 @@
     const uint32_t last_doc = it.doc_hi - 1;
     WaveTopK<CB> top(cand, K, lane);
     uint32_t found_s = 0;
+    float r_sc = 0.0f;
+    uint32_t r_doc = 0xFFFFFFFFu, row_hits = 0;
+    uint64_t r_left = 0ull;
+    bool row_complete = false;
+    gp_u32 d_skips = nullptr;
+    if constexpr (ROW) {
+        const uint32_t nrow = min(ra.nhits, kRowLen);
+        const Hit rh = ra.hits[lane];
+        r_sc = rh.score; r_doc = rh.doc;
+        r_left = lane_span(0u, nrow);
+        found_s = d_end - d_cur;
+        row_complete = nrow == d_end - d_cur;
+        d_skips = (gp_u32)seg.skips + (terms[it.term_begin + dl].skip - 1u);
+        NS_CNT(19, 1);
+    }
 
     constexpr uint32_t WSLACK = (FB == 64) ? kWinSlackThin : kWinSlackGen;
     uint32_t w_n = 0, e_n = 0xFFFFFFFFu;
@@ -434,8 +453,84 @@
         }
         if (total > 0 && tb_min < dl) { NS_FOREIGN_RMW(tb_min, min(tb_max, dl - 1)); }
 
+        if constexpr (ROW) {
+            if (total > 0) {
+                static_assert(FE == 1, "one foreign posting per lane");
+                const bool own = fmine[0];
+                const uint32_t doc = own ? fdoc[0] : lo;
+                const uint32_t cell = doc / kSkipDocs;
+                uint32_t a = d_skips[cell];
+                uint32_t n = d_skips[cell + 1u] - a;
+                bool hit = false;
+                uint32_t hbits = 0u;
+#pragma unroll
+                for (int step = 0; step < 4; step++) {
+                    const uint32_t s8 = (n + 7u) >> 3;
+                    nat_u2 pv[7];
+#pragma unroll
+                    for (int i = 0; i < 7; i++) {
+                        const uint32_t e = (uint32_t)(i + 1) * s8;
+                        pv[i] = stream[a + ((e <= n && e != 0u) ? e - 1u : 0u)];
+                    }
+                    uint32_t c = 0u;
+#pragma unroll
+                    for (int i = 0; i < 7; i++) {
+                        const uint32_t e = (uint32_t)(i + 1) * s8;
+                        const bool valid = e <= n && e != 0u;
+                        c += (valid && pv[i].x < doc) ? 1u : 0u;
+                        if (valid && pv[i].x == doc) { hit = true; hbits = pv[i].y; }
+                    }
+                    const bool closed = c < 7u && (c + 1u) * s8 <= n;
+                    a += c * s8;
+                    n = (n == 0u) ? 0u : (closed ? s8 - 1u : n - c * s8);
+                }
+                hit = hit && own;
+                if (hit) vals[lane] = vals[lane] + d_wq * __uint_as_float(hbits);
+                found_s -= (uint32_t)__popcll(wballot(hit));
+                NS_CNT(28, (uint32_t)__popcll(wballot(own)));
+                NS_CNT(29, (uint32_t)__popcll(wballot(hit)));
+                wave_sync();
+            }
+            const uint64_t inr = r_left & wballot(r_doc <= hi);
+            if (inr != 0ull) {
+                uint64_t offm = inr;
+                if (total > 0) {
+                    const uint32_t tag = NS_TAG(r_doc);
+                    const uint32_t hb = NS_BUCKET(r_doc);
+                    uint32_t b = hb;
+                    uint4 q = ent4[b];
+                    const uint64_t cm = wballot((q.x >> 16) == tag) | wballot((q.y >> 16) == tag) |
+                                        wballot((q.z >> 16) == tag) | wballot((q.w >> 16) == tag);
+                    const uint64_t go = inr & (cm | wballot(q.w != EMPTY));
+                    NS_CNT(30, (uint32_t)__popcll(inr));
+                    if (go != 0ull) {
+                        const uint32_t ident = NS_IDENT(r_doc, hb);
+                        uint32_t m = 0;
+                        bool more = __builtin_amdgcn_inverse_ballot_w64(go);
+                        for (int round = 0; round < NB; round++) {
+                            if (wballot(more) == 0ull) break;
+                            if (more) {
+                                m = ((q.x ^ ident) < 256u) ? q.x : m;
+                                m = ((q.y ^ ident) < 256u) ? q.y : m;
+                                m = ((q.z ^ ident) < 256u) ? q.z : m;
+                                m = ((q.w ^ ident) < 256u) ? q.w : m;
+                                more = m == 0 && q.w != EMPTY;
+                                if (more) { b = (b + 1) & (uint32_t)(NB - 1); q = ent4[b]; }
+                            }
+                        }
+                        const uint64_t hitm = wballot(m != 0) & go;
+                        offm &= ~hitm;
+                        row_hits += (uint32_t)__popcll(hitm);
+                        NS_CNT(31, (uint32_t)__popcll(hitm));
+                    }
+                }
+                top.offer_mask_stream(offm, r_sc, r_doc);
+                r_left &= ~inr;
+            }
+        }
+
         bool driver_progress = false;
-        for (;;) {
+        if constexpr (!ROW) for (;;) {
             const uint32_t remd = d_end - d_cur;
             if (remd == 0) break;
             uint32_t n;
@@ -621,8 +716,10 @@
         top.keep_room();
 
         if (hi >= last_doc) break;
-        if (Rf == 0 && d_cur >= d_end) break;
-        if (total == 0 && !driver_progress) break;
+        if constexpr (!ROW) {
+            if (Rf == 0 && d_cur >= d_end) break;
+            if (total == 0 && !driver_progress) break;
+        }
         lo = hi + 1;
     }
 #undef NS_FOREIGN_RMW
@@ -634,6 +731,16 @@
 #ifdef NS_COUNT
     const unsigned long long cyc_t1_ = __builtin_readcyclecounter();
 #endif
+    if constexpr (ROW) {
+        if (lane == 0 && row_hits != 0u) atomicAdd(ra.stats + 1, row_hits);
+        if (!row_complete && row_hits > kRowLen - K) {
+#ifdef NS_COUNT
+            if (lane == 0)
+                for (int i = 0; i < kNsCnt; i++) if (cnt_[i]) atomicAdd(&g_ns_cnt[i], cnt_[i]);
+#endif
+            return false;
+        }
+    }
     top.write_out(it.seg, it.out_slot, found_s, out_hits, out_nhits, out_found);
 #ifdef NS_COUNT
     cnt_[17] = __builtin_readcyclecounter() - cyc_t0_;
@@ -641,6 +748,7 @@
     if (lane == 0)
         for (int i = 0; i < kNsCnt; i++) if (cnt_[i]) atomicAdd(&g_ns_cnt[i], cnt_[i]);
 #endif
+    return true;
 }
 
 template <int HK, int FB, bool AND>
diff --git a/nextsearch-api_amd/csrc/ns_internal.h b/nextsearch-api_amd/csrc/ns_internal.h
--- a/nextsearch-api_amd/csrc/ns_internal.h
+++ b/nextsearch-api_amd/csrc/ns_internal.h
@@ -67,6 +67,13 @@
     uint32_t whole;
 };
 
+struct DevRItem {
+    DevWItem it;
+    uint32_t row;
+    uint32_t dterm;
+};
+static constexpr uint32_t kRowLen = 64;
+
 struct DevGroup {
     uint64_t bounds_off;
     uint32_t term_begin;
diff --git a/nextsearch-api_amd/csrc/ns_plan.hpp b/nextsearch-api_amd/csrc/ns_plan.hpp
--- a/nextsearch-api_amd/csrc/ns_plan.hpp
+++ b/nextsearch-api_amd/csrc/ns_plan.hpp
@@ -9,6 +9,7 @@
 #include <memory>
 #include <string>
 #include <thread>
+#include <unordered_map>
 #include <vector>
 
 #include "../../include/nextsearch_hip.h"
@@ -43,6 +44,8 @@
 static constexpr uint64_t kWorkForeign = 8, kWorkTile = 2, kWorkMerge = 4;
 static constexpr uint32_t kSkipMinCount = 64;
 static constexpr uint64_t kItemTermGeneral = 4000, kItemTermThin = 3000, kItemTermTile = 8000;
+static constexpr uint32_t kRowMinUsers = 4, kRowCellPostings = 65536;
+static constexpr uint32_t kRowMaxTerms = 16;
 
 inline std::string vformat(const char* fmt, va_list ap) {
     char buf[512];
@@ -156,6 +159,9 @@
     bool order_coarse_forced = false;
     uint32_t key_pct[4] = {100, 100, 100, 100};
     uint32_t tile_dens64 = 16;
+    int row_mode = 0;
+    uint32_t row_min_users = kRowMinUsers;
+    uint32_t row_cell_postings = kRowCellPostings;
 };
 
 inline size_t place_at(size_t& off, size_t bytes) {
@@ -165,7 +171,22 @@
 }
 
 
-struct HostGroup { DevGroup g; uint32_t query; uint64_t cost; uint64_t cmax; uint64_t work; bool wave; uint8_t cls; bool fast_div; bool signed_in; bool grid; bool merge2; };
+struct HostGroup { DevGroup g; uint32_t query; uint64_t cost; uint64_t cmax; uint64_t work; bool wave; uint8_t cls; bool fast_div; bool signed_in; bool grid; bool merge2;
+                   uint32_t rkey1; };
+
+struct RowKey {
+    uint32_t seg, first, count, idf_bits, w_bits;
+    bool operator==(const RowKey& o) const { return seg == o.seg && first == o.first && count == o.count && idf_bits == o.idf_bits && w_bits == o.w_bits; }
+};
+struct RowKeyHash {
+    size_t operator()(const RowKey& k) const {
+        uint64_t h = ((uint64_t)k.seg << 32 | k.first) * 0x9E3779B97F4A7C15ull;
+        h ^= ((uint64_t)k.idf_bits << 32 | k.w_bits) * 0xC2B2AE3D27D4EB4Full;
+        return (size_t)(h ^ (h >> 29));
+    }
+};
+struct RowKeyEnt { RowKey key; uint32_t users, skip, cells, prod_begin, rank; bool on; };
+struct RowCand { uint32_t group, dterm, skip, key; };
 
 constexpr uint32_t kOrderBuckets = 2048;
 inline uint32_t order_bucket(uint64_t c) {
@@ -181,6 +202,7 @@
     std::vector<HostGroup> groups;
     std::vector<uint32_t> qgroup_begin;
     std::vector<uint32_t> seg_ids;
+    std::vector<RowCand> rcand;
     uint64_t bounds_total = 0, postings_total = 0, total_work = 0;
     bool all_imp = true, all_pk = true, any_pruned = false;
     int err_code = NS_OK;
@@ -189,6 +211,8 @@
     std::vector<DevWItem> witems;
     std::vector<uint16_t> wbucket;
     std::vector<uint32_t> wshare;
+    std::vector<DevRItem> ritems;
+    std::vector<uint16_t> rbucket;
     std::vector<DevItem> items;
     std::vector<uint64_t> item_cost;
     std::vector<DevGroup> bgroups;
@@ -200,13 +224,13 @@
     std::vector<uint32_t> start;
     void reset(uint32_t a, uint32_t b) {
         q0 = a; q1 = b;
-        dterms.clear(); groups.clear(); qgroup_begin.clear(); seg_ids.clear();
+        dterms.clear(); groups.clear(); qgroup_begin.clear(); seg_ids.clear(); rcand.clear();
         bounds_total = postings_total = total_work = 0; all_imp = true; all_pk = true; any_pruned = false;
         err_code = NS_OK; err_query = 0xFFFFFFFFu; err_msg.clear();
-        witems.clear(); wbucket.clear(); wshare.clear(); items.clear(); item_cost.clear(); bgroups.clear();
+        witems.clear(); wbucket.clear(); wshare.clear(); ritems.clear(); rbucket.clear(); items.clear(); item_cost.clear(); bgroups.clear();
         n_rows = 0; direct = true;
-        hist.assign(2 * kOrderBuckets, 0u);
-        start.assign(2 * kOrderBuckets, 0u);
+        hist.assign(3 * kOrderBuckets, 0u);
+        start.assign(3 * kOrderBuckets, 0u);
         term_off = row_off = bgroup_off = 0; bounds_off = 0;
     }
     void fail_at(uint32_t q, int code, const char* fmt, ...) {
@@ -230,7 +254,11 @@
     std::vector<DevShare> share_build;
     uint64_t share_postings = 0;
     std::vector<uint32_t> wide_q;
-    struct Layout { size_t items, witems, terms, groups, queries, segs, wideq, share, bytes; } layout{};
+    uint32_t n_ritems = 0, n_pitems = 0, n_pterms = 0;
+    std::vector<RowKeyEnt> rkeys;
+    std::vector<DevWItem> pitems;
+    std::vector<DevTerm> pterms;
+    struct Layout { size_t items, witems, terms, groups, queries, segs, wideq, share, ritems, pitems, rstats, bytes; } layout{};
     bool deal = false;
     uint32_t deal_shift = 0;
     std::vector<uint32_t> bucket_pos;
@@ -240,7 +268,7 @@
     const ns_query_desc* queries = nullptr;
     const ns_term_ref* terms = nullptr;
     uint32_t n_queries = 0, k = 0, flags = 0;
-    bool auto_mode = false, want_imp = false;
+    bool auto_mode = false, want_imp = false, row_try = false;
     unsigned width = 1;
     uint32_t G = 0;
     uint64_t total_work = 0;
@@ -281,6 +309,7 @@
         if (slices.size() < width) slices.resize(width);
         for (unsigned s = 0; s < width; s++) slices[s].reset((uint32_t)((uint64_t)n_queries * s / width), (uint32_t)((uint64_t)n_queries * (s + 1) / width));
         want_imp = C.use_impacts && auto_mode;
+        row_try = want_imp && C.row_mode != 0 && C.share_mode != 0 && C.use_skips && !(flags & NS_FLAG_AND) && k <= 32;
 
         fork([&](unsigned si) {
             PrepSlice& S = slices[si];
@@ -342,6 +371,14 @@
                         hg.merge2 = auto_mode && C.use_merge && hg.cls == 0 && hg.g.term_count == 2 && rest * C.merge_ratio >= hg.cmax;
                         if (hg.merge2) hg.work = hg.cmax + rest * kWorkMerge;
                     }
+                    if (row_try && hg.wave && hg.cls == 1 && !hg.signed_in && hg.g.term_count <= kRowMaxTerms && hg.cmax >= kSkipMinCount &&
+                        sv.n_docs > 0 && !sv.lists->skip.empty() && !(C.use_pruning && hg.g.term_count == 1)) {
+                        const DevTerm* dt = S.dterms.data() + hg.g.term_begin;
+                        uint32_t d = 0;
+                        while (dt[d].count != hg.cmax) d++;
+                        const uint32_t sk = sv.lists->skip_of((uint32_t)dt[d].list_off, dt[d].count);
+                        if (sk) S.rcand.push_back(RowCand{(uint32_t)S.groups.size(), d, sk, 0u});
+                    }
                     if (!hg.wave) {
                         hg.g.bounds_off = S.bounds_total;
                         S.bounds_total += (uint64_t)(sv.n_tiles + 1) * hg.g.term_count;
@@ -419,6 +456,13 @@
         return NS_OK;
     }
 
+    static void row_cell(uint32_t n_docs, uint32_t cells, uint32_t i, uint32_t& lo, uint32_t& hi) {
+        lo = (uint32_t)((uint64_t)n_docs * i / cells);
+        hi = (uint32_t)((uint64_t)n_docs * (i + 1) / cells);
+        lo -= lo % kSkipDocs;
+        if (i + 1 < cells) hi -= hi % kSkipDocs;
+    }
+
     int cut() {
         const PlanSettings& C = *cfg;
         const std::vector<SegView>& SV = *segs;
@@ -440,6 +484,50 @@
         uint32_t chunks_per_group = 1;
         if (G > 0 && G < min_items) chunks_per_group = std::min<uint32_t>((min_items + G - 1) / G, 1024u);
         dq.assign(n_queries, DevQuery{});
+
+        rkeys.clear(); pitems.clear(); pterms.clear();
+        n_ritems = n_pitems = n_pterms = 0;
+        if (shared && row_try) {
+            std::unordered_map<RowKey, uint32_t, RowKeyHash> index;
+            for (unsigned s = 0; s < width; s++) {
+                PrepSlice& S = slices[s];
+                for (RowCand& c : S.rcand) {
+                    const DevTerm& t = S.dterms[S.groups[c.group].g.term_begin + c.dterm];
+                    RowKey key{t.seg, (uint32_t)t.list_off, t.count, 0u, 0u};
+                    std::memcpy(&key.idf_bits, &t.idf, 4); std::memcpy(&key.w_bits, &t.weight, 4);
+                    auto ins = index.emplace(key, (uint32_t)rkeys.size());
+                    if (ins.second) rkeys.push_back(RowKeyEnt{key, 0u, c.skip, 0u, 0u, 0u, false});
+                    c.key = ins.first->second;
+                    rkeys[c.key].users++;
+                }
+            }
+            for (RowKeyEnt& e : rkeys) {
+                if (C.row_mode != 2 && e.users < C.row_min_users) continue;
+                const SegView& sg = SV[e.key.seg];
+                uint32_t cells = 1;
+                while ((uint64_t)cells * std::max<uint32_t>(C.row_cell_postings, 1u) < e.key.count && cells * 2 <= sg.n_docs / kSkipDocs && cells < 4096) cells <<= 1;
+                e.on = true; e.cells = cells; e.prod_begin = n_pitems; e.rank = n_pterms++;
+                DevTerm t{};
+                t.list_off = e.key.first; t.count = e.key.count; t.seg = e.key.seg; t.skip = e.skip;
+                std::memcpy(&t.idf, &e.key.idf_bits, 4); std::memcpy(&t.weight, &e.key.w_bits, 4);
+                pterms.push_back(t);
+                for (uint32_t i = 0; i < cells; i++) {
+                    DevWItem it{};
+                    it.seg = e.key.seg;
+                    it.term_begin = n_dterms + e.rank;
+                    it.term_count = 1;
+                    row_cell(sg.n_docs, cells, i, it.doc_lo, it.doc_hi);
+                    it.out_slot = n_pitems++;
+                    it.whole = (cells == 1 ? 1u : 0u) | 4u | 64u;
+                    pitems.push_back(it);
+                }
+            }
+            for (unsigned s = 0; s < width; s++) {
+                PrepSlice& S = slices[s];
+                for (const RowCand& c : S.rcand)
+                    if (rkeys[c.key].on) S.groups[c.group].rkey1 = c.key + 1u;
+            }
+        }
 
         fork([&](unsigned si) {
             PrepSlice& S = slices[si];
@@ -463,7 +551,9 @@
                             if (k > 32 && p2 < 8) p2 = 8;
                             ns = std::min<uint32_t>(p2, std::min<uint32_t>(sg.n_docs, 4096));
                         }
-                        if (auto_mode && C.use_skips && (hg.cls == 2 || ns > 1) && !sg.lists->skip.empty()) {
+                        const RowKeyEnt* rk = hg.rkey1 ? &rkeys[hg.rkey1 - 1u] : nullptr;
+                        if (rk) ns = rk->cells;
+                        if (auto_mode && C.use_skips && (hg.cls == 2 || ns > 1 || rk) && !sg.lists->skip.empty()) {
                             for (uint32_t ti = 0; ti < hg.g.term_count; ti++) {
                                 if (dt[ti].count < kSkipMinCount) continue;
                                 dt[ti].skip = sg.lists->skip_of((uint32_t)dt[ti].list_off, dt[ti].count);
@@ -484,6 +574,7 @@
                         if (fine_cut && hg.cls == 0) key = key * 5 / 8;
                         else if (auto_mode && k > 32 && hg.cls == 0) key = key * 3 / 4;
                         if (auto_mode) key = key * C.key_pct[hg.merge2 ? 3 : hg.cls] / 100;
+                        if (rk) key = (hg.cost - hg.cmax) * kWorkForeign / ns + 1 + kItemTermThin * hg.g.term_count;
                         const bool wide = auto_mode && hg.g.term_count > 16;
                         const uint32_t bucket = order_bucket(key);
                         uint64_t big_off = 0;
@@ -501,10 +592,19 @@
                                 it.doc_lo -= it.doc_lo % kSkipDocs;
                                 if (i + 1 < ns) it.doc_hi -= it.doc_hi % kSkipDocs;
                             }
+                            if (rk) row_cell(sg.n_docs, ns, i, it.doc_lo, it.doc_hi);
                             if (it.doc_hi <= it.doc_lo) continue;
                             it.out_slot = S.n_rows++;
                             it.whole = (ns == 1 ? 1u : 0u) | (hg.fast_div ? 8u : 0u) | (hg.signed_in ? 16u : 0u) | (hg.grid ? (hg.cls == 2 ? 32u : 64u) : 0u);
                             if (auto_mode) it.whole |= (hg.cls == 2 ? 2u : 0u) | (hg.cls == 1 ? 4u : 0u) | (pruned_ ? 128u : 0u) | (hg.merge2 && hg.wave ? 256u : 0u);
+                            if (rk) {
+                                uint32_t d = 0;
+                                while (dt[d].count != hg.cmax) d++;
+                                S.ritems.push_back(DevRItem{it, rk->prod_begin + i, d});
+                                S.rbucket.push_back((uint16_t)bucket);
+                                S.hist[2 * kOrderBuckets + bucket]++;
+                                continue;
+                            }
                             S.witems.push_back(it);
                             S.wbucket.push_back((uint16_t)(bucket | (wide ? 0x8000u : 0u)));
                             {
@@ -547,7 +647,7 @@
         for (unsigned s = 0; s < width; s++) {
             PrepSlice& S = slices[s];
             S.row_off = n_rows; S.bgroup_off = n_bgroups;
-            n_rows += S.n_rows; n_witems += (uint32_t)S.witems.size(); n_items += (uint32_t)S.items.size(); n_bgroups += (uint32_t)S.bgroups.size();
+            n_rows += S.n_rows; n_witems += (uint32_t)S.witems.size(); n_ritems += (uint32_t)S.ritems.size(); n_items += (uint32_t)S.items.size(); n_bgroups += (uint32_t)S.bgroups.size();
             direct = direct && S.direct;
             pruned = pruned || S.any_pruned;
         }
@@ -568,6 +668,13 @@
             n_class[1] = pos - n_class[0];
             if (pos != n_witems) return failed(NS_E_STATE, "internal: launch order holds %u of %u work items", pos, n_witems);
             if (!auto_mode) { n_class[0] = n_class[1] = 0; }
+            uint32_t rpos = 0;
+            for (uint32_t bkt = 0; bkt < kOrderBuckets; bkt++)
+                for (unsigned s = 0; s < width; s++) {
+                    slices[s].start[2 * kOrderBuckets + bkt] = rpos;
+                    rpos += slices[s].hist[2 * kOrderBuckets + bkt];
+                }
+            if (rpos != n_ritems) return failed(NS_E_STATE, "internal: launch order holds %u of %u row consumers", rpos, n_ritems);
         }
         sorted_items.clear();
         if (n_items) {
@@ -592,12 +699,15 @@
         size_t off = 0;
         layout.items = place_at(off, (size_t)n_items * sizeof(DevItem));
         layout.witems = place_at(off, (size_t)n_witems * sizeof(DevWItem));
-        layout.terms = place_at(off, (size_t)n_dterms * sizeof(DevTerm));
+        layout.terms = place_at(off, (size_t)(n_dterms + n_pterms) * sizeof(DevTerm));
         layout.groups = place_at(off, (size_t)n_bgroups * sizeof(DevGroup));
         layout.queries = place_at(off, dq.size() * sizeof(DevQuery));
         layout.segs = place_at(off, SV.size() * sizeof(DevSeg));
         layout.wideq = place_at(off, wide_q.size() * 4);
         layout.share = place_at(off, shared ? (share_build.size() + 1) * sizeof(DevShare) : 0);
+        layout.ritems = n_ritems ? place_at(off, (size_t)n_ritems * sizeof(DevRItem)) : off;
+        layout.pitems = n_pitems ? place_at(off, (size_t)n_pitems * sizeof(DevWItem)) : off;
+        layout.rstats = n_pitems ? place_at(off, 8) : off;
         layout.bytes = off;
 
         uint64_t resident_bytes = 0;
@@ -619,6 +729,12 @@
                 const uint32_t at = S.start[((bk & 0x8000u) ? kOrderBuckets : 0) + (bk & 0x7FFFu)]++;
                 wdst[at] = it;
                 if (deal) share_at[at] = S.wshare[i];
+            }
+            DevRItem* rdst = (DevRItem*)(hb + layout.ritems);
+            for (size_t i = 0; i < S.ritems.size(); i++) {
+                DevRItem ri = S.ritems[i];
+                ri.it.out_slot = direct ? ri.it.query : ri.it.out_slot + S.row_off;
+                rdst[S.start[2 * kOrderBuckets + S.rbucket[i]]++] = ri;
             }
             if (!S.dterms.empty()) std::memcpy(hb + layout.terms + (size_t)S.term_off * sizeof(DevTerm), S.dterms.data(), S.dterms.size() * sizeof(DevTerm));
             if (!S.bgroups.empty()) std::memcpy(hb + layout.groups + (size_t)S.bgroup_off * sizeof(DevGroup), S.bgroups.data(), S.bgroups.size() * sizeof(DevGroup));
@@ -666,6 +782,9 @@
                 }
             });
         }
+        if (n_pterms) std::memcpy(hb + layout.terms + (size_t)n_dterms * sizeof(DevTerm), pterms.data(), (size_t)n_pterms * sizeof(DevTerm));
+        if (n_pitems) std::memcpy(hb + layout.pitems, pitems.data(), (size_t)n_pitems * sizeof(DevWItem));
+        if (n_pitems) std::memset(hb + layout.rstats, 0, 8);
         if (n_items) std::memcpy(hb + layout.items, sorted_items.data(), (size_t)n_items * sizeof(DevItem));
         if (!wide_q.empty()) std::memcpy(hb + layout.wideq, wide_q.data(), wide_q.size() * 4);
         if (shared) {
diff --git a/nextsearch-api_amd/csrc/ns_row_kernel.hip b/nextsearch-api_amd/csrc/ns_row_kernel.hip
--- /dev/null
+++ b/nextsearch-api_amd/csrc/ns_row_kernel.hip
@@ -0,0 +1,41 @@
+#pragma once
+#include <hip/hip_runtime.h>
+#include <stdint.h>
+
+#include "ns_driver_kernel.hip"
+
+namespace ns {
+
+template <int HK, int CB, int TMAX>
+__global__ void __launch_bounds__(64) __attribute__((amdgpu_waves_per_eu(6, 8))) k_rscore(const DevRItem* __restrict__ items, uint32_t n_items,
+                                                const DevTerm* __restrict__ terms, const DevSeg* __restrict__ segs,
+                                                const Hit* __restrict__ row_hits, const uint32_t* __restrict__ row_nhits,
+                                                Hit* __restrict__ out_hits, uint32_t* __restrict__ out_nhits,
+                                                uint64_t* __restrict__ out_found, uint32_t K, uint32_t* __restrict__ stats) {
+    __shared__ __attribute__((aligned(16))) uint32_t s_tbl[2 * HK];
+    __shared__ __attribute__((aligned(16))) float s_vals[64];
+    __shared__ __attribute__((aligned(16))) uint8_t s_mcnt[16];
+    __shared__ uint64_t s_cand[CB];
+    __shared__ __attribute__((aligned(16))) uint4 s_tab[TMAX];
+    __shared__ uint32_t s_aux[TMAX];
+    const int lane = threadIdx.x & 63;
+    const uint32_t item_idx = blockIdx.x;
+    if (item_idx >= n_items) return;
+    const DevRItem ri = items[item_idx];
+    DevWItem it = ri.it;
+    it.whole &= 121u;
+    RowArgs ra;
+    ra.hits = row_hits + (size_t)ri.row * kRowLen;
+    ra.nhits = row_nhits[ri.row];
+    ra.dterm = ri.dterm;
+    ra.stats = stats;
+    if (dscore_body<HK / 2, 64, false, CB, true, 0, true>(it, terms, segs, s_tbl, s_vals, s_mcnt, s_cand, s_tab, s_aux, out_hits, out_nhits,
+                                                          out_found, K, lane, ra))
+        return;
+    if (lane == 0) atomicAdd(stats, 1u);
+    wave_sync();
+    dscore_body<HK / 2, 64, false, CB, true, 0, false>(it, terms, segs, s_tbl, s_vals, s_mcnt, s_cand, s_tab, s_aux, out_hits, out_nhits,
+                                                       out_found, K, lane);
+}
+
+}
diff --git a/nextsearch-api_amd/nsbind.py b/nextsearch-api_amd/nsbind.py
--- a/nextsearch-api_amd/nsbind.py
+++ b/nextsearch-api_amd/nsbind.py
@@ -55,7 +55,7 @@
     "ns_ctx_create", "ns_ctx_destroy", "ns_ctx_set_stream", "ns_last_error", "ns_device_name",
     "ns_segment_upload", "ns_segment_release", "ns_segment_upload_begin", "ns_segment_upload_append", "ns_segment_upload_end", "ns_search_batch", "ns_batch_prepare",
     "ns_batch_bind_outputs", "ns_batch_run", "ns_batch_stream", "ns_batch_gap_ms", "ns_batch_sync", "ns_batch_fetch", "ns_batch_get_info",
-    "ns_batch_destroy", "ns_set_tuning", "ns_segment_build_impacts", "ns_ctx_use_impacts", "ns_ctx_set_host_threads", "ns_ctx_set_overlap", "ns_segment_build_packed", "ns_ctx_use_packed", "ns_segment_build_skips", "ns_ctx_use_skips", "ns_segment_build_blockmax", "ns_ctx_use_pruning", "ns_ctx_use_merge", "ns_ctx_share_scores",
+    "ns_batch_destroy", "ns_set_tuning", "ns_segment_build_impacts", "ns_ctx_use_impacts", "ns_ctx_set_host_threads", "ns_ctx_set_overlap", "ns_segment_build_packed", "ns_ctx_use_packed", "ns_segment_build_skips", "ns_ctx_use_skips", "ns_segment_build_blockmax", "ns_ctx_use_pruning", "ns_ctx_use_merge", "ns_ctx_share_scores", "ns_ctx_share_rows", "ns_batch_row_stats",
     "ns_invert_forward", "ns_segment_upload_inverted", "ns_merge_rank_rows", "ns_sem_upload", "ns_sem_release", "ns_sem_topk",
     "ns_ac_upload", "ns_ac_suggest", "ns_ac_release", "ns_ac_build_fuzzy", "ns_ac_fuzzy", "ns_ac_fuzzy_prefix",
     "ns_forward_build", "ns_forward_get_info", "ns_forward_fetch", "ns_forward_destroy",
@@ -184,6 +184,9 @@
         L.ns_ctx_use_pruning.argtypes = [vp, i32]
         L.ns_ctx_use_merge.argtypes = [vp, i32]
         L.ns_ctx_share_scores.argtypes = [vp, i32]
+        if hasattr(L, "ns_ctx_share_rows"):
+            L.ns_ctx_share_rows.argtypes = [vp, i32]
+            L.ns_batch_row_stats.argtypes = [vp, vp]
         L.ns_sem_upload.argtypes = [vp, vp, u32, u32, C.POINTER(vp)]
         L.ns_sem_release.argtypes = [vp, vp]
         L.ns_sem_topk.argtypes = [vp, vp, vp, u32, u32, C.c_float, vp, vp, vp, vp, vp, vp]
@@ -468,6 +471,13 @@
         hip_lib().ns_batch_get_info(self.h, C.byref(inf))
         return inf
 
+    def row_stats(self):
+        out = np.zeros(4, dtype=np.uint32)
+        rc = hip_lib().ns_batch_row_stats(self.h, out.ctypes.data)
+        if rc != NS_OK:
+            raise RuntimeError(f"ns_batch_row_stats failed rc={rc}")
+        return tuple(int(x) for x in out)
+
     def close(self):
         if self.h:
             hip_lib().ns_batch_destroy(self.h)
```

Result: faster. 8.887 million (median of 6 runs) (+9.1%).
